# sayands/sgaligner

Hardware: AMD Instinct MI355X
Metric: subscan-pairs/sec (fwd+bwd) + node-match Hits@1 vs reference (higher is better)
Workload: dtype f32 (fp32 operands and fp32 accumulation throughout; the anchors x negatives loss sweeps multiply them as three exact bf16 planes, six bf16 MFMAs per product...

## Files before the change

include/sgaligner_hip.h:

```cpp
#ifndef SGALIGNER_HIP_H
#define SGALIGNER_HIP_H
#include <stddef.h>
#include <stdint.h>
#ifdef __cplusplus
extern "C" {
#endif

int sga_version(void);
const char* sga_last_error(void);
int sga_device_cus(void);

int sga_pointnet_fwd(const float* x, const float* w1, const float* b1, const float* w2, const float* b2,
                     const float* w3, const float* b3, float* y, int32_t* argmax, int T, int P, int C3,
                     void* stream);
size_t sga_pointnet_fwd_ws_bytes(int T, int C3);
int sga_pointnet_fwd_ws(const float* x, const float* w1, const float* b1, const float* w2, const float* b2,
                        const float* w3, const float* b3, float* y, int32_t* argmax, int T, int P, int C3,
                        void* workspace, size_t ws_bytes, int mode, void* stream);
size_t sga_pointnet_fwd_bn_ws_bytes(int T, int C3);
int sga_pointnet_fwd_bn(const float* x, const float* w1, const float* b1, const float* w2, const float* b2,
                        const float* w3, const float* b3, float* y, int32_t* argmax, int T, int P, int C3,
                        void* workspace, size_t ws_bytes, void* bn_workspace, size_t bn_ws_bytes, double* bn_sums, int mode, void* stream);
int sga_pointnet_bwd(const float* x, const int32_t* argmax, const float* y, const float* gy, const float* w1,
                     const float* b1, const float* w2, const float* b2, const float* w3, float* gw1, float* gb1,
                     float* gw2, float* gb2, float* gw3, float* gb3, int T, int P, int C3, int mode, void* stream);

int sga_gemm(int transA, int transB, int M, int N, int K, const void* A, long lda, int a_is_f64, const float* B,
             long ldb, float* C, long ldc, const float* bias, int accumulate, void* stream);
int sga_colsum(const float* X, long ld, int M, int N, float* out, int accumulate, void* stream);
int sga_gemm_bnstats(int M, int N, int K, const float* A, long lda, const float* B, long ldb, float* C, long ldc, const float* bias,
                     double* sums, void* stream);
int sga_cast_f64_f32(const double* in, float* out, size_t n, void* stream);
enum sga_gemm_route {
    SGA_GEMM_EMPTY = 0,
    SGA_GEMM_TN_NARROW,
    SGA_GEMM_TN_SPLIT,
    SGA_GEMM_TN_BIG,
    SGA_GEMM_NN,
    SGA_GEMM_NT_128,
    SGA_GEMM_NT_64,
    SGA_GEMM_NT3_128,
    SGA_GEMM_NT3_64,
    SGA_GEMM_SMALL_F32,
    SGA_GEMM_SMALL_F64,
    SGA_GEMM_GENERIC_F32,
    SGA_GEMM_GENERIC_F64,
    SGA_GEMM_REFUSED
};
int sga_gemm_plan(int transA, int transB, int M, int N, int K, long lda, long ldb, long ldc, long ldr, int a_is_f64, int a_aligned16,
                  int b_aligned16, int has_bias, int accumulate, int act, int has_resid, int has_colstats, int ncu, int* route, int* splits,
                  int* k_per_split);

int sga_fusion_fwd(const float* const* embs, int M, const float* weight, float* joint, int T, int D, void* stream);
size_t sga_fusion_bwd_workspace_bytes(int M);
int sga_fusion_bwd(const float* const* embs, int M, const float* weight, const float* gjoint, float* const* gembs,
                   float* gweight, int T, int D, void* workspace, size_t workspace_bytes, void* stream);
int sga_fusion_var_fwd(const float* const* embs, int M, const int32_t* widths, const float* weight, float* joint, int T, void* stream);
int sga_fusion_var_bwd(const float* const* embs, int M, const int32_t* widths, const float* weight, const float* gjoint,
                       float* const* gembs, float* gweight, int T, void* workspace, size_t workspace_bytes, void* stream);

int sga_gat_complete_flags(const int64_t* edges, const int32_t* node_off, const int32_t* edge_off, int G, uint8_t* flags, void* stream);
int sga_gat_attn_fwd(const float* H, const float* att_src, const float* att_dst, const float* bias,
                     const int64_t* edges, const int32_t* node_off, const int32_t* edge_off, int G, int nmax,
                     float* out, int32_t* status, const uint8_t* complete, void* stream);
int sga_gat_attn_bwd(const float* H, const float* dO, const float* att_src, const float* att_dst, const int64_t* edges,
                     const int32_t* node_off, const int32_t* edge_off, int G, int nmax, float* dH, float* d_att_src,
                     float* d_att_dst, const uint8_t* complete, void* stream);
int sga_gat_attn_fwd_hc(const float* H, int heads, int channels, const float* att_src, const float* att_dst, const float* bias,
                        const int64_t* edges, const int32_t* node_off, const int32_t* edge_off, int G, int nmax,
                        float* out, int32_t* status, const uint8_t* complete, void* stream);
int sga_gat_attn_bwd_hc(const float* H, const float* dO, int heads, int channels, const float* att_src, const float* att_dst,
                        const int64_t* edges, const int32_t* node_off, const int32_t* edge_off, int G, int nmax, float* dH,
                        float* d_att_src, float* d_att_dst, const uint8_t* complete, void* stream);
int sga_gat_lds_nodes(int channels, int bwd);
int sga_elu_fwd(const float* x, float* y, size_t n, void* stream);
int sga_elu_bwd(const float* x, const float* gy, float* gx, size_t n, void* stream);

int sga_gcn_aggregate(const float* H, int C, const float* bias, const int64_t* edges, const int32_t* node_off, const int32_t* edge_off,
                      int G, int nmax, int transpose, int relu, float* out, int32_t* status, void* stream);
int sga_relu_bwd(const float* y, const float* gy, float* gx, size_t n, void* stream);

int sga_nca_row_group(void);
int sga_nca_block_sums(const float* S, long lds, int h, int A, int row0, float alpha, float ep, double* rsum, float* diag, double* cpart,
                       void* stream);
int sga_nca_loss(const double* rsum, const double* cpart, int ngroups, const float* diag, int A, float alpha, float beta, double* csum,
                 float* invr, float* invc, double* loss, void* stream);
int sga_nca_coef(const float* S, long lds, float* G, long ldg, float* GT, long ldt, int h, int A, int row0, float alpha, float beta, float ep,
                 const float* invr, const float* invc, const double* gout, void* stream);

int sga_loss_gather(const float* E, int T, int D, const int32_t* idx, int R, float* Z, int Dp, float* nrm, void* stream);
int sga_loss_scatter(const float* dZ, const float* Z, const float* nrm, const int32_t* idx, int R, int D, int Dp,
                     float* dE, void* stream);
int sga_loss_slots(void);
int sga_loss_neg_sums(const float* Z, int Dp, int A, int J1, int J2, float tau0, float tau1, double* sums8, void* stream);
int sga_loss_neg_grad(const float* Z, int Dp, int A, int J1, int J2, float tau0, float tau1, const double* gs8,
                      float* dZ, void* stream);
int sga_loss_neg_sums_shard(const float* Z, int Dp, int A, int J1, int J2, float tau0, float tau1, double* sums8, int a_lo, int a_hi,
                            void* stream);
int sga_loss_neg_grad_shard(const float* Z, int Dp, int A, int J1, int J2, float tau0, float tau1, const double* gs8,
                            float* dZ, int a_lo, int a_hi, void* stream);
size_t sga_loss_anchor_f16_ws_bytes(int NT, int A, int ns);
int sga_loss_anchor_fwd_f16(const float* const* Z, const void* const* Zh, const int* Dp, int NT, int A, const double* sums,
                            float alpha, float tau_icl, float tau_ial, double* out, int a_lo, int a_hi, void* ws, size_t ws_bytes,
                            void* stream);
int sga_loss_anchor_bwd_f16(const float* const* Z, const void* const* Zh, const int* Dp, int NT, int A, const double* sums,
                            float alpha, float tau_icl, float tau_ial, const float* coef, float* const* M1,
                            double* gs, int a_lo, int a_hi, void* ws, size_t ws_bytes, void* stream);

int sga_loss_stash_grad(const float* M1, const float* Z, int A, int Dp, float* dZ, int a_lo, int a_hi, void* stream);
int sga_loss_multi_sums(const float* const* Z, int M, int D, const float* beta, int A, int J1, int J2, float tau0, float tau1,
                        double* sums, int a_lo, int a_hi, void* stream);
int sga_loss_multi_grad(const float* const* Z, int M, int D, const float* beta, int A, int J1, int J2, float tau0, float tau1,
                        const double* gs, float* const* dZ, double* gamma, int a_lo, int a_hi, void* stream);
size_t sga_loss_centre_bytes(void);
int sga_loss_centre_tables(const float* Z, int A, int J1, int J2, float* Zc, void* stat_ws, void* stream);
int sga_loss_multi_sums_centred(const float* const* Zc, int M, const float* beta, int A, int J1, int J2, float tau0, float tau1,
                                double* sums, int a_lo, int a_hi, void* stream);
int sga_loss_multi_grad_centred(const float* const* Zc, int M, const float* beta, int A, int J1, int J2, float tau0, float tau1,
                                const double* gs, float* const* dZ, double* gamma, int a_lo, int a_hi, void* stream);
int sga_loss_scatter_tangent_stat(const float* dZ, const float* Z, const float* nrm, const int32_t* idx, int R, int D,
                                  const void* stat_ws, float* dE, void* stream);
int sga_loss_anchor_multi_fwd(const float* const* Z, int M, const float* beta, int A, const double* sums, float alpha,
                              float tau_icl, float tau_ial, double* out, int a_lo, int a_hi, void* stream);
int sga_loss_anchor_multi_bwd(const float* const* Z, int M, const float* beta, int A, const double* sums, float alpha,
                              float tau_icl, float tau_ial, const float* coef, float* const* M1, double* gs, double* gamma,
                              int a_lo, int a_hi, double* out_terms, void* stream);
int sga_loss_anchor_multi_bwd_sym(const float* const* Z, int M, const float* beta, int A, const double* sums, float alpha,
                                  float tau_icl, float tau_ial, const float* coef, float* const* M1, float* const* M2, double* gs,
                                  double* gamma, int a_lo, int a_hi, double* out_terms, void* stream);
int sga_loss_stash_grad_sym(const float* M1, const float* M2, const float* Z, int A, int Dp, float* dZ, int a_lo, int a_hi,
                            void* stream);
int sga_loss_anchor_multi_bwd_symx(const float* const* Z, int M, const float* beta, int A, const double* sums, float alpha,
                                   float tau_icl, float tau_ial, const float* coef, float* const* M1, float* const* M2,
                                   double* gs, double* gamma, int a_lo, int a_hi, int j_lo, int j_hi, int mir, double* out_terms, void* stream);
int sga_loss_stash_grad_symx(const float* M1, const float* M2, const float* Z, int A, int Dp, float* dZ, int a_lo, int a_hi,
                             int j_lo, int j_hi, int mir, void* stream);

int sga_loss_check_norms(const float* nrm, int n, float* poison, void* stream);

size_t sga_loss_split3_bytes(int A, int J1, int J2);
int sga_loss_split3_tables(const float* Z, int A, int J1, int J2, void* Zb, float* Zc, void* stream);
int sga_loss_multi_sums_bf16x6(const void* const* Zb, int M, const float* beta, int A, int J1, int J2, float tau0, float tau1,
                               double* sums, int a_lo, int a_hi, int lite, void* stream);
int sga_loss_multi_grad_bf16x6(const void* const* Zb, int M, const float* beta, int A, int J1, int J2, float tau0, float tau1,
                               const double* gs, float* const* dZ, double* gamma, int a_lo, int a_hi, void* stream);
int sga_loss_scatter_tangent(const float* dZ, const float* Z, const float* nrm, const int32_t* idx, int A, int J1, int J2, int D,
                             const void* Zb, float* dE, void* stream);
int sga_loss_stash_grad_symx_bf16x6(const float* M1, const float* M2, const void* Zb, int A, int J1, int J2, float* dZ,
                                    int a_lo, int a_hi, int j_lo, int j_hi, int mir, void* stream);

int sga_group_loss_fwd(const float* const* Z, int M, const float* beta, int A, int J1, const int32_t* groups, int G,
                       const int64_t* s_off, int64_t s_total, float alpha, float tau_icl, float tau_ial, float* S,
                       double* sums, double* out, int use_valu, void* stream);
int sga_group_loss_bwd(const float* const* Z, int M, const float* beta, int A, int J1, const int32_t* groups, int G,
                       const int64_t* s_off, int64_t s_total, float alpha, float tau_icl, float tau_ial, float* S,
                       const double* sums, const float* coef, float* const* dZ, double* gamma, int use_valu, void* stream);

size_t sga_simrank_workspace_bytes(int T);
size_t sga_simrank_workspace_bytes_f16(int T, int D);
int sga_simrank(const float* E, int T, int D, const int32_t* pair_off, const int32_t* blk_pair, const int32_t* blk_row, int n_blocks, int B,
                int max_pair_objects, const int32_t* q_idx, const int32_t* q_tgt, int Q, int K, int32_t* rank,
                int32_t* topk_idx, float* topk_sim, int f16, void* workspace, size_t workspace_bytes, void* stream);
int sga_pair_metrics(const int32_t* rank, const int32_t* topk_idx, const float* topk_sim, int K, const int32_t* q_tgt,
                     const int32_t* pair_off, const int32_t* pair_q_off, int B, float* out, void* stream);

int sga_gemm_ex(int transA, int transB, int M, int N, int K, const float* A, long lda, const float* B, long ldb,
                float* C, long ldc, const float* bias, int act, const float* resid, long ldr, void* stream);
int sga_pct_attention(const float* Q, long ldq, const float* V, long ldv, int T, int N, float* stats, float* Xs,
                      long ldx, void* stream);
int sga_pct_attention_bwd(const float* Q, long ldq, const float* V, long ldv, const float* dXs, long ldd, int T, int N,
                          const float* stats, float* work, float* dQ, long ldo, float* dV, long ldw, void* stream);
int sga_segment_max(const float* Y, long ldy, int T, int N, int C, float* G, int32_t* argmax, void* stream);
int sga_segment_max_bwd(const float* dG, const int32_t* argmax, int T, int N, int C, float* dY, long ldd, void* stream);
int sga_pct_head_prep(const float* dG, const float* G, const float* gamma, const float* beta, const float* fin, int T, int C, long R,
                      int training, float slope, float* coef, float* ab, void* stream);
int sga_pct_head_dw(const float* WG, const float* W, const float* ab, const float* cs, const float* coef, const int32_t* amax,
                    const float* cat, long ldc, int T, int N, int C, int K, float* dW, float* Wb, float* a0, void* stream);
int sga_pct_head_scatter(const float* coef, const int32_t* amax, const float* W, int T, int N, int C, int K, float* dcat, long ldd,
                         void* stream);
int sga_segment_max_affine(const float* Y, long ldy, int T, int N, int C, const float* scale, const float* shift, float slope, float* G,
                           int32_t* argmax, void* stream);

int sga_bn_stats(const float* X, long ldx, int R, int C, double* sums, void* stream);
int sga_bn_finalize(const double* sums, int R, int C, const float* gamma, const float* beta, float* running_mean, float* running_var,
                    long long* num_batches_tracked, float momentum, float eps, int training, float* out, void* stream);
int sga_bn_bwd_finalize(const double* sums, int R, int C, float* out, void* stream);
int sga_bn_apply(const float* X, long ldx, int R, int C, const float* scale, const float* shift, int act,
                 const float* resid, long ldr, float* Y, long ldy, void* stream);
int sga_bn_bwd_stats(const float* X, long ldx, const float* dY, long ldd, int R, int C, const float* scale,
                     const float* shift, const float* mean, const float* rstd, int act, double* sums, void* stream);
int sga_bn_bwd_apply(const float* X, long ldx, const float* dY, long ldd, int R, int C, const float* scale,
                     const float* shift, const float* mean, const float* rstd, const float* mean_g,
                     const float* mean_gx, int act, float* dX, long ldo, void* stream);

size_t sga_fps_scratch_floats(int total_points);
int sga_fps(const float* pts, const int32_t* offsets, int n_obj, const int32_t* start, int npoint,
            const int32_t* work_small, int n_small, const int32_t* work_mid, int n_mid,
            const int32_t* work_large, int n_large, int32_t* out_idx, float* scratch, void* stream);

int sga_hull_candidates(const float* pts, const int32_t* offsets, int n_obj, unsigned char* keep, int32_t* n_planes, void* stream);
int sga_hull_max_candidates(void);
int sga_hull_vertices(const double* pts, const int32_t* offsets, int n_obj, unsigned char* is_vertex, int32_t* status, void* stream);

size_t sga_nn_workspace_bytes(int total_queries, int max_support, int chunk);
int sga_nn_search(const double* pts, const int32_t* offsets, int n_clouds, int total_points, const int32_t* pairs, int n_pairs,
                  const int32_t* out_offsets, int total_queries, int max_queries, int max_support, int chunk,
                  const int32_t* offsets_host, const int32_t* pairs_host, int squared, double* out_dist, int32_t* out_idx,
                  void* workspace, size_t workspace_bytes, void* stream);

size_t sga_ransac_workspace_bytes(int n_jobs, int total_hyp, int max_rows, int chunk);
int sga_ransac_rigid(const double* corr, const int32_t* offsets, int n_jobs, int total_rows, const int32_t* samples,
                     const int32_t* hyp_offsets, int total_hyp, int max_rows, int max_hyp, int chunk, const int32_t* offsets_host,
                     const int32_t* hyp_offsets_host, double threshold, int refine_rounds, double* transform, int32_t* inlier_count,
                     int32_t* best_hyp, int32_t* status, unsigned char* inlier_mask, int32_t* hyp_count, void* workspace,
                     size_t workspace_bytes, void* stream);

int sga_subscan_lds_slots(void);
int sga_frame_visibility(const float* pts, const int32_t* pt_off, const double* w2c, const int32_t* fr_off, const double* intr,
                         const int64_t* vis_off, int n_scans, int total_points, int total_frames, int64_t total_words, int max_points,
                         int max_frames, const int32_t* pt_off_host, const int32_t* fr_off_host, const int64_t* vis_off_host,
                         uint64_t* vis, void* stream);
int sga_subscan_walk(const uint64_t* vis, uint64_t* cum, const int32_t* pt_off, const int32_t* fr_off, const int64_t* vis_off,
                     const int32_t* max_pts, int n_scans, int total_points, int total_frames, int64_t total_words,
                     const int32_t* pt_off_host, const int32_t* fr_off_host, const int64_t* vis_off_host, int32_t* seg_end,
                     int32_t* seg_count, int32_t* frame_count, int32_t* n_seg, void* stream);
int sga_subscan_object_counts(const uint64_t* bits, const int32_t* pt_off, const int32_t* fr_off, const int64_t* vis_off, int n_scans,
                              int total_points, int total_frames, int64_t total_words, int max_points, const int32_t* rows, int n_rows,
                              const int32_t* slot, int n_slots, const int32_t* pt_off_host, const int32_t* fr_off_host,
                              const int64_t* vis_off_host, const int32_t* rows_host, int32_t* counts, void* stream);

int sga_scenegraph_lds_slots(void);
int sga_scenegraph_tile(void);
int sga_graph_max_nodes(void);
int sga_object_counts(const int32_t* slot, const int32_t* pt_off, const int32_t* slot_off, int n_scans, int total_points, int total_slots,
                      int max_points, const int32_t* pt_off_host, const int32_t* slot_off_host, int32_t* counts, void* stream);
size_t sga_object_partition_ws_bytes(int n_scans, int max_points, int max_slots);
int sga_object_partition(const float* pts, const int32_t* slot, const int32_t* pt_off, const int32_t* slot_off, const int32_t* dest_off,
                         int n_scans, int total_points, int total_slots, int max_points, int max_slots, int n_kept_points,
                         const int32_t* pt_off_host, const int32_t* slot_off_host, const int32_t* dest_off_host, const int32_t* counts_host,
                         int32_t* perm, float* pts_out, void* ws, size_t ws_bytes, void* stream);
int sga_graph_complete(const int32_t* node_off, const int32_t* pair_off, const int32_t* trip_off, const int32_t* edge_off, int n_graphs,
                       const int32_t* pairs, const int32_t* rels, int none_id, int V, const int32_t* node_off_host,
                       const int32_t* pair_off_host, const int32_t* trip_off_host, const int32_t* edge_off_host, const int32_t* pairs_host,
                       const int32_t* rels_host, int64_t* edges, int32_t* n_edges, int32_t* bow, void* stream);
int sga_bow_counts(const int32_t* rows, const int32_t* cols, int n, int T, int V, const int32_t* rows_host, const int32_t* cols_host,
                   int32_t* out, void* stream);

size_t sga_loss_neg_grad_wide_floats(int A, int J1, int J2);
int sga_loss_neg_grad_wide(const float* Z, int Dp, int A, int J1, int J2, float tau0, float tau1, const double* gs8, float* dZ,
                           float* stash, size_t stash_floats, void* stream);

long sga_wide16_ldt(int A, int J1, int J2);
int sga_wide16_prepare(const float* Z, int Dp, int A, int J1, int J2, void* Zh, void* ZhT, void* stream);
int sga_loss_neg_sums_f16(const void* Zh, int Dp, int A, int J1, int J2, float tau0, float tau1, double* sums8, int a_lo, int a_hi, void* stream);
size_t sga_loss_neg_grad_f16_bytes(int A, int J1, int J2);
int sga_loss_neg_grad_f16(const void* Zh, const void* ZhT, int Dp, int A, int J1, int J2, float tau0, float tau1, const double* gs8,
                          float* dZ, void* stash, size_t stash_bytes, int a_lo, int a_hi, void* stream);
size_t sga_loss_stash_grad_f16_bytes(int A, int ns);
int sga_loss_stash_grad_f16(const float* M1, const void* ZhT, int Dp, int A, int J1, int J2, float* dZ, int a_lo, int a_hi,
                            void* ws, size_t ws_bytes, void* stream);

int sga_loss_head_fwd(const void* sums, int sums_f64, const float* lv_ial, const float* lv_icl, int M, double inv_a2,
                      double z_ial, double alpha, double zoom, double* out, void* stream);
int sga_loss_head_bwd(const double* gout, const void* sums, int sums_f64, const float* lv_ial, const float* lv_icl, int M,
                      double inv_a2, double z_ial, double alpha, double zoom, void* dsums, float* dlv_ial, float* dlv_icl,
                      void* stream);

#ifdef __cplusplus
}
#endif
#endif
```

sgaligner_amd/_build.py:

```python
from __future__ import annotations

import concurrent.futures as cf
import glob
import os
import subprocess
import sys

CSRC = os.path.join(os.path.dirname(os.path.abspath(__file__)), 'csrc')
LIB = os.path.join(CSRC, 'libsga_hip.so')
HIPCC = os.environ.get('HIPCC', '/opt/rocm/bin/hipcc')
FLAGS = ['--offload-arch=gfx950', '-O3', '-std=c++17', '-fPIC', '-ffp-contract=fast', '-munsafe-fp-atomics',
         '-Wno-unused-result', '-Wno-unused-value', '-I', CSRC]


def _newer(src_list, target):
    if not os.path.exists(target):
        return True
    t = os.path.getmtime(target)
    return any(os.path.getmtime(s) > t for s in src_list)


FILE_FLAGS = {'contrastive.hip': ['-fno-slp-vectorize'],
              'loss_pertable.hip': ['-fno-slp-vectorize'],
              'loss_anchor.hip': ['-fno-slp-vectorize'],
              'sweep3.hip': ['-fno-slp-vectorize'],
              'pointnet.hip': ['-fno-slp-vectorize'],
              'nnsearch.hip': ['-ffp-contract=off'],
              'visibility.hip': ['-ffp-contract=off']}


def _compile(src, obj, extra):
    cmd = [HIPCC] + FLAGS + FILE_FLAGS.get(os.path.basename(src), []) + extra + ['-c', src, '-o', obj]
    r = subprocess.run(cmd, capture_output=True, text=True)
    if r.returncode != 0:
        raise RuntimeError(f'hipcc failed for {src}:\n{r.stdout}\n{r.stderr}')
    return src


def build_lib(verbose: bool = True, extra_flags=()) -> str:
    srcs = sorted(glob.glob(os.path.join(CSRC, '*.hip')))
    hdrs = sorted(glob.glob(os.path.join(CSRC, '*.h'))) + sorted(glob.glob(os.path.join(CSRC, '..', '..', 'include', '*.h')))
    jobs = []
    objs = []
    for s in srcs:
        o = s[:-4] + '.o'
        objs.append(o)
        if _newer([s] + hdrs, o):
            jobs.append((s, o))
    if jobs:
        with cf.ThreadPoolExecutor(max_workers=min(8, len(jobs))) as ex:
            for done in ex.map(lambda so: _compile(so[0], so[1], list(extra_flags)), jobs):
                if verbose:
                    print('[sga build] compiled', os.path.basename(done), flush=True)
    if jobs or _newer(objs, LIB):
        r = subprocess.run([HIPCC, '--offload-arch=gfx950', '-shared', '-fPIC', '-o', LIB] + objs,
                           capture_output=True, text=True)
        if r.returncode != 0:
            raise RuntimeError(f'link failed:\n{r.stdout}\n{r.stderr}')
        if verbose:
            print('[sga build] linked', LIB, flush=True)
    return LIB


if __name__ == '__main__':
    build_lib(extra_flags=sys.argv[1:])
```

sgaligner_amd/_lib.py:

```python
from __future__ import annotations

import ctypes
import os
from ctypes import c_char_p, c_double, c_float, c_int, c_int64, c_long, c_size_t, c_void_p

_HERE = os.path.dirname(os.path.abspath(__file__))
LIB_PATH = os.environ.get('SGA_LIB_PATH') or os.path.join(_HERE, 'csrc', 'libsga_hip.so')
_lib = None

P = c_void_p
I = c_int
F = c_float

SIGNATURES = {
    'sga_version': (I, []),
    'sga_last_error': (c_char_p, []),
    'sga_device_cus': (I, []),
    'sga_pointnet_fwd': (I, [P, P, P, P, P, P, P, P, P, I, I, I, P]),
    'sga_pointnet_fwd_ws_bytes': (c_size_t, [I, I]),
    'sga_loss_neg_grad_wide_floats': (c_size_t, [I, I, I]),
    'sga_loss_neg_grad_wide': (I, [P, I, I, I, I, c_float, c_float, P, P, P, c_size_t, P]),
    'sga_wide16_ldt': (c_long, [I, I, I]),
    'sga_wide16_prepare': (I, [P, I, I, I, I, P, P, P]),
    'sga_loss_neg_sums_f16': (I, [P, I, I, I, I, c_float, c_float, P, I, I, P]),
    'sga_loss_neg_grad_f16_bytes': (c_size_t, [I, I, I]),
    'sga_loss_neg_grad_f16': (I, [P, P, I, I, I, I, c_float, c_float, P, P, P, c_size_t, I, I, P]),
    'sga_loss_head_fwd': (I, [P, I, P, P, I, c_double, c_double, c_double, c_double, P, P]),
    'sga_loss_head_bwd': (I, [P, P, I, P, P, I, c_double, c_double, c_double, c_double, P, P, P, P]),
    'sga_pointnet_fwd_ws': (I, [P, P, P, P, P, P, P, P, P, I, I, I, P, c_size_t, I, P]),
    'sga_pointnet_fwd_bn_ws_bytes': (c_size_t, [I, I]),
    'sga_pointnet_fwd_bn': (I, [P, P, P, P, P, P, P, P, P, I, I, I, P, c_size_t, P, c_size_t, P, I, P]),
    'sga_pointnet_bwd': (I, [P] * 15 + [I, I, I, I, P]),
    'sga_gat_complete_flags': (I, [P, P, P, I, P, P]),
    'sga_gat_attn_fwd': (I, [P, P, P, P, P, P, P, I, I, P, P, P, P]),
    'sga_gat_attn_bwd': (I, [P, P, P, P, P, P, P, I, I, P, P, P, P, P]),
    'sga_gat_attn_fwd_hc': (I, [P, I, I, P, P, P, P, P, P, I, I, P, P, P, P]),
    'sga_gat_attn_bwd_hc': (I, [P, P, I, I, P, P, P, P, P, I, I, P, P, P, P, P]),
    'sga_gat_lds_nodes': (I, [I, I]),
    'sga_elu_fwd': (I, [P, P, c_size_t, P]),
    'sga_elu_bwd': (I, [P, P, P, c_size_t, P]),
    'sga_simrank_workspace_bytes': (c_size_t, [I]),
    'sga_simrank_workspace_bytes_f16': (c_size_t, [I, I]),
    'sga_simrank': (I, [P, I, I, P, P, P, I, I, I, P, P, I, I, P, P, P, I, P, c_size_t, P]),
    'sga_pair_metrics': (I, [P, P, P, I, P, P, P, I, P, P]),
    'sga_gemm_ex': (I, [I, I, I, I, I, P, c_long, P, c_long, P, c_long, P, I, P, c_long, P]),
    'sga_pct_attention': (I, [P, c_long, P, c_long, I, I, P, P, c_long, P]),
    'sga_pct_attention_bwd': (I, [P, c_long, P, c_long, P, c_long, I, I, P, P, P, c_long, P, c_long, P]),
    'sga_segment_max': (I, [P, c_long, I, I, I, P, P, P]),
    'sga_segment_max_bwd': (I, [P, P, I, I, I, P, c_long, P]),
    'sga_pct_head_prep': (I, [P, P, P, P, P, I, I, c_long, I, c_float, P, P, P]),
    'sga_pct_head_dw': (I, [P, P, P, P, P, P, P, c_long, I, I, I, I, P, P, P, P]),
    'sga_pct_head_scatter': (I, [P, P, P, I, I, I, I, P, c_long, P]),
    'sga_segment_max_affine': (I, [P, c_long, I, I, I, P, P, c_float, P, P, P]),
    'sga_bn_stats': (I, [P, c_long, I, I, P, P]),
    'sga_bn_finalize': (I, [P, I, I, P, P, P, P, P, c_float, c_float, I, P, P]),
    'sga_bn_bwd_finalize': (I, [P, I, I, P, P]),
    'sga_bn_apply': (I, [P, c_long, I, I, P, P, I, P, c_long, P, c_long, P]),
    'sga_bn_bwd_stats': (I, [P, c_long, P, c_long, I, I, P, P, P, P, I, P, P]),
    'sga_bn_bwd_apply': (I, [P, c_long, P, c_long, I, I, P, P, P, P, P, P, I, P, c_long, P]),
    'sga_fps_scratch_floats': (c_size_t, [I]),
    'sga_fps': (I, [P, P, I, P, I, P, I, P, I, P, I, P, P, P]),
    'sga_hull_candidates': (I, [P, P, I, P, P, P]),
    'sga_hull_max_candidates': (I, []),
    'sga_hull_vertices': (I, [P, P, I, P, P, P]),
    'sga_nn_workspace_bytes': (c_size_t, [I, I, I]),
    'sga_nn_search': (I, [P, P, I, I, P, I, P, I, I, I, I, P, P, I, P, P, P, c_size_t, P]),
    'sga_ransac_workspace_bytes': (c_size_t, [I, I, I, I]),
    'sga_ransac_rigid': (I, [P, P, I, I, P, P, I, I, I, I, P, P, c_double, I, P, P, P, P, P, P, P, c_size_t, P]),
    'sga_subscan_lds_slots': (I, []),
    'sga_frame_visibility': (I, [P, P, P, P, P, P, I, I, I, c_int64, I, I, P, P, P, P, P]),
    'sga_subscan_walk': (I, [P, P, P, P, P, P, I, I, I, c_int64, P, P, P, P, P, P, P, P]),
    'sga_subscan_object_counts': (I, [P, P, P, P, I, I, I, c_int64, I, P, I, P, I, P, P, P, P, P, P]),
    'sga_scenegraph_lds_slots': (I, []),
    'sga_scenegraph_tile': (I, []),
    'sga_graph_max_nodes': (I, []),
    'sga_object_counts': (I, [P, P, P, I, I, I, I, P, P, P, P]),
    'sga_object_partition_ws_bytes': (c_size_t, [I, I, I]),
    'sga_object_partition': (I, [P, P, P, P, P, I, I, I, I, I, I, P, P, P, P, P, P, P, c_size_t, P]),
    'sga_graph_complete': (I, [P, P, P, P, I, P, P, I, I, P, P, P, P, P, P, P, P, P, P]),
    'sga_bow_counts': (I, [P, P, I, I, I, P, P, P, P]),
    'sga_gemm': (I, [I, I, I, I, I, P, c_long, I, P, c_long, P, c_long, P, I, P]),
    'sga_colsum': (I, [P, c_long, I, I, P, I, P]),
    'sga_gemm_bnstats': (I, [I, I, I, P, c_long, P, c_long, P, c_long, P, P, P]),
    'sga_cast_f64_f32': (I, [P, P, c_size_t, P]),
    'sga_gemm_plan': (I, [I, I, I, I, I, c_long, c_long, c_long, c_long] + [I] * 9 + [P, P, P]),
    'sga_loss_gather': (I, [P, I, I, P, I, P, I, P, P]),
    'sga_loss_scatter': (I, [P, P, P, P, I, I, I, P, P]),
    'sga_loss_neg_sums': (I, [P, I, I, I, I, F, F, P, P]),
    'sga_loss_neg_grad': (I, [P, I, I, I, I, F, F, P, P, P]),
    'sga_loss_neg_sums_shard': (I, [P, I, I, I, I, F, F, P, I, I, P]),
    'sga_loss_neg_grad_shard': (I, [P, I, I, I, I, F, F, P, P, I, I, P]),
    'sga_loss_anchor_f16_ws_bytes': (c_size_t, [I, I, I]),
    'sga_loss_anchor_fwd_f16': (I, [P, P, P, I, I, P, F, F, F, P, I, I, P, c_size_t, P]),
    'sga_loss_anchor_bwd_f16': (I, [P, P, P, I, I, P, F, F, F, P, P, P, I, I, P, c_size_t, P]),
    'sga_loss_stash_grad_f16_bytes': (c_size_t, [I, I]),
    'sga_loss_stash_grad_f16': (I, [P, P, I, I, I, I, P, I, I, P, c_size_t, P]),
    'sga_loss_multi_sums': (I, [P, I, I, P, I, I, I, F, F, P, I, I, P]),
    'sga_loss_multi_grad': (I, [P, I, I, P, I, I, I, F, F, P, P, P, I, I, P]),
    'sga_loss_centre_bytes': (c_size_t, []),
    'sga_loss_centre_tables': (I, [P, I, I, I, P, P, P]),
    'sga_loss_multi_sums_centred': (I, [P, I, P, I, I, I, F, F, P, I, I, P]),
    'sga_loss_multi_grad_centred': (I, [P, I, P, I, I, I, F, F, P, P, P, I, I, P]),
    'sga_loss_scatter_tangent_stat': (I, [P, P, P, P, I, I, P, P, P]),
    'sga_loss_check_norms': (I, [P, I, P, P]),
    'sga_loss_slots': (I, []),
    'sga_loss_anchor_multi_fwd': (I, [P, I, P, I, P, F, F, F, P, I, I, P]),
    'sga_loss_anchor_multi_bwd': (I, [P, I, P, I, P, F, F, F, P, P, P, P, I, I, P, P]),
    'sga_loss_stash_grad': (I, [P, P, I, I, P, I, I, P]),
    'sga_loss_anchor_multi_bwd_sym': (I, [P, I, P, I, P, F, F, F, P, P, P, P, P, I, I, P, P]),
    'sga_loss_stash_grad_sym': (I, [P, P, P, I, I, P, I, I, P]),
    'sga_loss_anchor_multi_bwd_symx': (I, [P, I, P, I, P, F, F, F, P, P, P, P, P, I, I, I, I, I, P, P]),
    'sga_loss_stash_grad_symx': (I, [P, P, P, I, I, P, I, I, I, I, I, P]),
    'sga_loss_split3_bytes': (c_size_t, [I, I, I]),
    'sga_loss_split3_tables': (I, [P, I, I, I, P, P, P]),
    'sga_loss_scatter_tangent': (I, [P, P, P, P, I, I, I, I, P, P, P]),
    'sga_loss_stash_grad_symx_bf16x6': (I, [P, P, P, I, I, I, P, I, I, I, I, I, P]),
    'sga_loss_multi_sums_bf16x6': (I, [P, I, P, I, I, I, F, F, P, I, I, I, P]),
    'sga_loss_multi_grad_bf16x6': (I, [P, I, P, I, I, I, F, F, P, P, P, I, I, P]),
    'sga_group_loss_fwd': (I, [P, I, P, I, I, P, I, P, c_int64, F, F, F, P, P, P, I, P]),
    'sga_group_loss_bwd': (I, [P, I, P, I, I, P, I, P, c_int64, F, F, F, P, P, P, P, P, I, P]),
    'sga_fusion_fwd': (I, [P, I, P, P, I, I, P]),
    'sga_fusion_bwd_workspace_bytes': (c_size_t, [I]),
    'sga_fusion_bwd': (I, [P, I, P, P, P, P, I, I, P, c_size_t, P]),
    'sga_fusion_var_fwd': (I, [P, I, P, P, P, I, P]),
    'sga_fusion_var_bwd': (I, [P, I, P, P, P, P, P, I, P, c_size_t, P]),
    'sga_gcn_aggregate': (I, [P, I, P, P, P, P, I, I, I, I, P, P, P]),
    'sga_relu_bwd': (I, [P, P, P, c_size_t, P]),
    'sga_nca_row_group': (I, []),
    'sga_nca_block_sums': (I, [P, c_long, I, I, I, F, F, P, P, P, P]),
    'sga_nca_loss': (I, [P, P, I, P, I, F, F, P, P, P, P, P]),
    'sga_nca_coef': (I, [P, c_long, P, c_long, P, c_long, I, I, I, F, F, F, P, P, P, P]),
}

GEMM_ROUTES = ('EMPTY', 'TN_NARROW', 'TN_SPLIT', 'TN_BIG', 'NN', 'NT_128', 'NT_64', 'NT3_128', 'NT3_64', 'SMALL_F32', 'SMALL_F64',
               'GENERIC_F32', 'GENERIC_F64', 'REFUSED')


class SgaLibraryError(RuntimeError):
    pass


def lib():
    global _lib
    if _lib is None:
        if not os.path.exists(LIB_PATH):
            raise SgaLibraryError(
                f'HIP library not built: {LIB_PATH} is missing. Run `python -c "import __graft_entry__ as g; g.build()"` '
                f'(or `python -m sgaligner_amd._build`). sgaligner_amd has no CPU fallback.')
        import torch
        try:
            l = ctypes.CDLL(LIB_PATH)
        except OSError as e:
            raise SgaLibraryError(f'cannot load {LIB_PATH}: {e}') from e
        for name, (res, args) in SIGNATURES.items():
            try:
                fn = getattr(l, name)
            except AttributeError as e:
                raise SgaLibraryError(f'{LIB_PATH} does not export {name}; rebuild the library') from e
            fn.restype = res
            fn.argtypes = args
        _lib = l
    return _lib


def check(rc: int, what: str):
    if rc != 0:
        msg = lib().sga_last_error()
        raise RuntimeError(f'{what} failed (code {rc}): {msg.decode() if msg else "?"}')
```

sgaligner_amd/csrc/loss_anchor.hip:

```cpp
#include "mfma_tiles.h"
#include <type_traits>

#include "loss_math.h"

extern "C" int sga_gemm(int transA, int transB, int M, int N, int K, const void* A, long lda, int a_is_f64, const float* B,
                        long ldb, float* C, long ldc, const float* bias, int accumulate, void* stream);

namespace {

constexpr int CT_THREADS = 256;
struct AnchorMultiArgs {
    int M, A, i_lo, i_hi, nsplit;
    const float* Z[4];
    const float* beta;
    const double* sums;
    const float* inv;
    float alpha, kc, ki, itc, iti;
    double* out;
    const float* coef;
    float* M1[4];
    double* gs;
    double* gamma;
    int j_lo;
    float* M2[4];
    int j_hi, mir;
};

template <int M>
__global__ __launch_bounds__(CT_THREADS, M <= 3 ? 2 : 1) void anchor_multi_kernel(AnchorMultiArgs a) {
    constexpr int DP = 104, NQ = 13, NT = M + 1;
    extern __shared__ __attribute__((aligned(16))) float lds[];
    float* inv_s = lds + M * 2 * 32 * DP;
    const int tid = threadIdx.x, lane = tid & 63, wave = tid >> 6, h = lane >> 5, l31 = lane & 31;
    const int A = a.A, ns = a.i_hi - a.i_lo;
    const int ib = blockIdx.x / a.nsplit, split = blockIdx.x % a.nsplit;
    const int i0 = a.i_lo + ib * 32;
    const int my_i = i0 + l31;
    const bool iv = my_i < a.i_hi;

    for (int e = tid; e < M * 2 * 32 * (DP / 4); e += CT_THREADS) {
        const int c = (e % (DP / 4)) * 4, r = (e / (DP / 4)) % 32, side = (e / (DP / 4) / 32) % 2, m = e / (DP / 4) / 64;
        const int row = min(i0 + r, a.i_hi - 1) + side * A;
        *reinterpret_cast<f32x4*>(lds + ((m * 2 + side) * 32 + r) * DP + c) = *reinterpret_cast<const f32x4*>(a.Z[m] + (size_t)row * DP + c);
    }
    for (int e = tid; e < NT * 8; e += CT_THREADS) inv_s[e] = (float)(1.0 / (a.sums[e] + 1e-9));
    __syncthreads();
    float beta[M];
#pragma unroll
    for (int m = 0; m < M; ++m) beta[m] = a.beta[m];

    double acc_d[NT + 2 * M];
#pragma unroll
    for (int e = 0; e < NT + 2 * M; ++e) acc_d[e] = 0.0;

    const int ntile = (A + 31) / 32;
    for (int jt = split * 4 + wave; jt < ntile; jt += a.nsplit * 4) {
        const int j0 = jt * 32;
        float acc_out[NT + 2 * M];
#pragma unroll
        for (int e = 0; e < NT + 2 * M; ++e) acc_out[e] = 0.f;
        const int jrow = min(j0 + l31, A - 1);
        f32x16 P[M], Q[M];
        zero_acc<M>(P);
        zero_acc<M>(Q);
#pragma unroll
        for (int m = 0; m < M; ++m) {
            const float* gp = a.Z[m] + (size_t)(A + jrow) * DP + 4 * h;
            const float* gq = a.Z[m] + (size_t)jrow * DP + 4 * h;
            const float* bp = lds + ((m * 2 + 0) * 32 + l31) * DP + 4 * h;
            const float* bq = lds + ((m * 2 + 1) * 32 + l31) * DP + 4 * h;
            f32x4 apA = *reinterpret_cast<const f32x4*>(gp), aqA = *reinterpret_cast<const f32x4*>(gq), apB = apA, aqB = aqA;
#pragma unroll
            for (int q = 0; q < NQ; ++q) {
                if (q + 1 < NQ) {
                    if (q & 1) { apA = *reinterpret_cast<const f32x4*>(gp + 8 * (q + 1)); aqA = *reinterpret_cast<const f32x4*>(gq + 8 * (q + 1)); }
                    else { apB = *reinterpret_cast<const f32x4*>(gp + 8 * (q + 1)); aqB = *reinterpret_cast<const f32x4*>(gq + 8 * (q + 1)); }
                }
                const f32x4 b1 = *reinterpret_cast<const f32x4*>(bp + 8 * q);
                const f32x4 b2 = *reinterpret_cast<const f32x4*>(bq + 8 * q);
#pragma unroll
                for (int r = 0; r < 4; ++r) {
                    P[m] = __builtin_amdgcn_mfma_f32_32x32x2f32((q & 1) ? apB[r] : apA[r], b1[r], P[m], 0, 0, 0);
                    Q[m] = __builtin_amdgcn_mfma_f32_32x32x2f32((q & 1) ? aqB[r] : aqA[r], b2[r], Q[m], 0, 0, 0);
                }
                __builtin_amdgcn_sched_barrier(0);
            }
        }
        float xs[M][16], ys[M][16];
#pragma unroll
        for (int m = 0; m < M; ++m)
#pragma unroll
            for (int r = 0; r < 16; ++r) { xs[m][r] = P[m][r]; ys[m][r] = Q[m][r]; }
        const float* js = inv_s + M * 8;
#pragma unroll
        for (int r = 0; r < 16; ++r) {
            const int j = j0 + mfma32_row(r, h);
            const bool ok = iv && j < A;
            float xj = 0.f, yj = 0.f;
#pragma unroll
            for (int m = 0; m < M; ++m) { xj = fmaf(beta[m], xs[m][r], xj); yj = fmaf(beta[m], ys[m][r], yj); }
            {
                const float dji = fexp2(xj * a.ki);
                const float qma = g_val(dji, js[1], js[3]), qmb = g_val(dji, js[5], js[7]);
                const float lqma = flog(qma), lqmb = flog(qmb);
#pragma unroll
                for (int k = 0; k < NT; ++k) {
                    const float x = k < M ? xs[k < M ? k : 0][r] : xj, y = k < M ? ys[k < M ? k : 0][r] : yj;
                    const float* is = inv_s + k * 8;
                    const float qa = g_val(fexp2(x * a.kc), is[0], is[2]);
                    const float qb = g_val(fexp2(y * a.kc), is[4], is[6]);
                    const float term = -flog(a.alpha * qa + (1.f - a.alpha) * qb);
                    acc_out[k] += ok ? term : 0.f;
                    if (k < M) {
                        const float dm = fexp2(x * a.ki);
                        const float qoa = g_val(dm, is[1], is[3]), qob = g_val(dm, is[5], is[7]);
                        const float ta = __expf(qoa) * (qoa - lqma), tb = __expf(qob) * (qob - lqmb);
                        acc_out[NT + (k < M ? k : 0)] += ok ? ta : 0.f;
                        acc_out[NT + M + (k < M ? k : 0)] += ok ? tb : 0.f;
                    }
                }
            }
#pragma unroll
            for (int e = 0; e < NT + 2 * M; ++e) asm volatile("" : "+v"(acc_out[e]));
            __builtin_amdgcn_sched_barrier(0);
        }
#pragma unroll
        for (int e = 0; e < NT + 2 * M; ++e) acc_d[e] += (double)acc_out[e];
    }
    const int slot = my_slot();
#pragma unroll
    for (int e = 0; e < NT + 2 * M; ++e) {
        const double v = wave_sum_d(acc_d[e]);
        if (lane == 0 && v != 0.0) atomicAdd(a.out + (NT + 2 * M) * (1 + slot) + e, v);
    }
}

__global__ void inv_sums_kernel(const double* __restrict__ sums, float* __restrict__ inv, int n) {
    const int i = blockIdx.x * blockDim.x + threadIdx.x;
    if (i < n) inv[i] = (float)(1.0 / (sums[i] + 1e-9));
}

template <int M, bool TERMS = false, int RB = (M <= 3 ? 32 : 16), bool SYM = false>
__global__ __launch_bounds__(CT_THREADS, 2) void anchor_multi_bwd16_kernel(AnchorMultiArgs a) {
    static_assert(!SYM || TERMS, "symmetric mode: one-pass build");
    constexpr int DP = 104, NT = M + 1, NSUB = RB / 16, TW = 4 / NSUB;
    extern __shared__ __attribute__((aligned(16))) float lds[];
    const float* __restrict__ inv_s = a.inv;
    auto CF = [&](int e) { return a.coef[e]; };
    const int tid = threadIdx.x, lane = tid & 63, wave = tid >> 6, g = lane >> 4, l15 = lane & 15;
    const int A = a.A, ns = a.i_hi - a.i_lo;
    const int JH = SYM ? a.j_hi : A;
    const int ib = blockIdx.x / a.nsplit, split = blockIdx.x % a.nsplit;
    const int i0 = a.i_lo + ib * RB;
    const int ih = wave % NSUB, tw = wave / NSUB;
    const int my_i = i0 + ih * 16 + l15;
    const bool iv = my_i < a.i_hi;

    for (int e = tid; e < M * 2 * RB * (DP / 4); e += CT_THREADS) {
        const int c = (e % (DP / 4)) * 4, r = (e / (DP / 4)) % RB, side = (e / (DP / 4) / RB) % 2, m = e / (DP / 4) / (2 * RB);
        const int row = min(i0 + r, a.i_hi - 1) + side * A;
        *reinterpret_cast<f32x4*>(lds + ((m * 2 + side) * RB + r) * DP + c) = *reinterpret_cast<const f32x4*>(a.Z[m] + (size_t)row * DP + c);
    }
    __syncthreads();
    float beta[M];
#pragma unroll
    for (int m = 0; m < M; ++m) beta[m] = a.beta[m];

    float acc_gs[NT][8], acc_gam[M];
#pragma unroll
    for (int k = 0; k < NT; ++k)
#pragma unroll
        for (int e = 0; e < 8; ++e) acc_gs[k][e] = 0.f;
#pragma unroll
    for (int m = 0; m < M; ++m) acc_gam[m] = 0.f;
    float acc_out[TERMS ? NT + 2 * M : 1];
#pragma unroll
    for (int e = 0; e < (TERMS ? NT + 2 * M : 1); ++e) acc_out[e] = 0.f;
    int tiles_done = 0;
    const int slot = my_slot();
    auto flush = [&]() {
        if (TERMS) {
#pragma unroll
            for (int e = 0; e < NT + 2 * M; ++e) {
                const float v = wave_sum(acc_out[TERMS ? e : 0]);
                if (lane == 0 && v != 0.f) atomicAdd(a.out + (NT + 2 * M) * (1 + slot) + e, (double)v);
                acc_out[TERMS ? e : 0] = 0.f;
            }
        }
#pragma unroll
        for (int k = 0; k < NT; ++k)
#pragma unroll
            for (int e = 0; e < 8; ++e) {
                const float iv2 = inv_s[k * 8 + e];
                const float v = -iv2 * iv2 * wave_sum(acc_gs[k][e]);
                if (lane == 0 && v != 0.f) atomicAdd(a.gs + NT * 8 * (1 + slot) + k * 8 + e, (double)v);
                acc_gs[k][e] = 0.f;
            }
#pragma unroll
        for (int m = 0; m < M; ++m) {
            const float v = wave_sum(acc_gam[m]);
            if (lane == 0 && v != 0.f) atomicAdd(a.gamma + M * (1 + slot) + m, (double)v);
            acc_gam[m] = 0.f;
        }
    };
    const float* js = inv_s + M * 8;

    const int ntile = (JH + 15) / 16;
#pragma unroll 1
    for (int jt = (a.j_lo >> 4) + split * TW + tw; jt < ntile; jt += a.nsplit * TW) {
        const int j0 = jt * 16;
        const int jrow = min(j0 + l15, A - 1);
        int lofs = 0;
        asm volatile("" : "+v"(lofs));
        f32x4 P[M], Q[M];
        struct JOps { f32x4 p[6], q[6]; float pt[2], qt[2]; };
        auto jload = [&](int m, JOps& o) {
            const float* gp = a.Z[m] + (size_t)(A + jrow) * DP;
            const float* gq = a.Z[m] + (size_t)jrow * DP;
#pragma unroll
            for (int q = 0; q < 6; ++q) {
                o.p[q] = *reinterpret_cast<const f32x4*>(gp + 16 * q + 4 * g);
                o.q[q] = *reinterpret_cast<const f32x4*>(gq + 16 * q + 4 * g);
            }
#pragma unroll
            for (int t = 0; t < 2; ++t) { o.pt[t] = gp[96 + 4 * t + g]; o.qt[t] = gq[96 + 4 * t + g]; }
        };
        constexpr bool JDB = true;
        JOps jb[JDB ? 2 : 1];
        jload(0, jb[0]);
#pragma unroll
        for (int m = 0; m < M; ++m) {
            if (JDB) { if (m + 1 < M) jload(m + 1, jb[JDB ? (m + 1) & 1 : 0]); }
            else if (m > 0) jload(m, jb[0]);
            __builtin_amdgcn_sched_barrier(0);
            P[m] = f32x4{0.f, 0.f, 0.f, 0.f};
            Q[m] = P[m];
            const JOps& o = jb[JDB ? m & 1 : 0];
            const float* bp = lds + lofs + ((m * 2 + 0) * RB + ih * 16 + l15) * DP;
            const float* bq = lds + lofs + ((m * 2 + 1) * RB + ih * 16 + l15) * DP;
#pragma unroll
            for (int q = 0; q < 6; ++q) {
                const f32x4 b1 = *reinterpret_cast<const f32x4*>(bp + 16 * q + 4 * g);
                const f32x4 b2 = *reinterpret_cast<const f32x4*>(bq + 16 * q + 4 * g);
#pragma unroll
                for (int r = 0; r < 4; ++r) {
                    P[m] = __builtin_amdgcn_mfma_f32_16x16x4f32(o.p[q][r], b1[r], P[m], 0, 0, 0);
                    Q[m] = __builtin_amdgcn_mfma_f32_16x16x4f32(o.q[q][r], b2[r], Q[m], 0, 0, 0);
                }
            }
#pragma unroll
            for (int t = 0; t < 2; ++t) {
                const int kk = 96 + 4 * t + g;
                P[m] = __builtin_amdgcn_mfma_f32_16x16x4f32(o.pt[t], bp[kk], P[m], 0, 0, 0);
                Q[m] = __builtin_amdgcn_mfma_f32_16x16x4f32(o.qt[t], bq[kk], Q[m], 0, 0, 0);
            }
            __builtin_amdgcn_sched_barrier(0);
        }
        const float cJ = CF(M);
        auto epilogue = [&](auto masked_c) {
        constexpr bool MASKED = decltype(masked_c)::value;
#pragma unroll
        for (int r = 0; r < 4; ++r) {
            const int j = j0 + 4 * g + r;
            const bool ok = !MASKED || (iv && (j < JH));
            const float okf = (!MASKED || ok) ? 1.f : 0.f;
            float xj = 0.f, yj = 0.f;
#pragma unroll
            for (int m = 0; m < M; ++m) { xj = fmaf(beta[m], P[m][r], xj); yj = fmaf(beta[m], Q[m][r], yj); }
            float gJ, EA = 0.f, EB = 0.f;
            {
                const float dx = fexp2(xj * a.kc), dy = fexp2(yj * a.kc);
                const GP Ax = g_parts(dx, js[0], js[2]), Bx = g_parts(dx, js[4], js[6]);
                const float qAy = g_val(dy, js[0], js[2]), qBy = g_val(dy, js[4], js[6]);
                const float denA = a.alpha * Ax.q + (1.f - a.alpha) * qBy;
                const float wA = okf * (-cJ * a.alpha) * frcp(denA) * dx;
                const float wB = okf * (-cJ * (1.f - a.alpha)) * frcp(a.alpha * qAy + (1.f - a.alpha) * Bx.q) * dx;
                if (TERMS) acc_out[TERMS ? M : 0] = fmaf(okf, -flog(denA), acc_out[TERMS ? M : 0]);
                gJ = fmaf(wA, Ax.dd, wB * Bx.dd) * a.itc;
                acc_gs[M][0] = fmaf(wA, Ax.p, acc_gs[M][0]); acc_gs[M][2] = fmaf(wA, Ax.r, acc_gs[M][2]);
                acc_gs[M][4] = fmaf(wB, Bx.p, acc_gs[M][4]); acc_gs[M][6] = fmaf(wB, Bx.r, acc_gs[M][6]);
            }
            const float dji = fexp2(xj * a.ki);
            const GP MA = g_parts(dji, js[1], js[3]), MB = g_parts(dji, js[5], js[7]);
            const float lqma = flog(MA.q), lqmb = flog(MB.q);
            float gx[M];
#pragma unroll
            for (int m = 0; m < M; ++m) {
                const float* is = inv_s + m * 8;
                const float c = CF(m), ca = CF(NT + m), cb = CF(NT + M + m);
                const float x = P[m][r], y = Q[m][r];
                const float dx = fexp2(x * a.kc), dy = fexp2(y * a.kc);
                const GP Ax = g_parts(dx, is[0], is[2]), Bx = g_parts(dx, is[4], is[6]);
                const float qAy = g_val(dy, is[0], is[2]), qBy = g_val(dy, is[4], is[6]);
                const float denA = a.alpha * Ax.q + (1.f - a.alpha) * qBy;
                const float wA = okf * (-c * a.alpha) * frcp(denA) * dx;
                const float wB = okf * (-c * (1.f - a.alpha)) * frcp(a.alpha * qAy + (1.f - a.alpha) * Bx.q) * dx;
                if (TERMS) acc_out[TERMS ? m : 0] = fmaf(okf, -flog(denA), acc_out[TERMS ? m : 0]);
                float gxm = fmaf(wA, Ax.dd, wB * Bx.dd) * a.itc;
                acc_gs[m][0] = fmaf(wA, Ax.p, acc_gs[m][0]); acc_gs[m][2] = fmaf(wA, Ax.r, acc_gs[m][2]);
                acc_gs[m][4] = fmaf(wB, Bx.p, acc_gs[m][4]); acc_gs[m][6] = fmaf(wB, Bx.r, acc_gs[m][6]);
                const float dm = fexp2(x * a.ki);
                const GP OA = g_parts(dm, is[1], is[3]), OB = g_parts(dm, is[5], is[7]);
                const float xA = okf * __expf(OA.q), xB = okf * __expf(OB.q);
                const float eA = ca * xA, eB = cb * xB;
                if (TERMS) {
                    acc_out[TERMS ? NT + m : 0] = fmaf(xA, OA.q - lqma, acc_out[TERMS ? NT + m : 0]);
                    acc_out[TERMS ? NT + M + m : 0] = fmaf(xB, OB.q - lqmb, acc_out[TERMS ? NT + M + m : 0]);
                }
                const float tA = eA * (OA.q - lqma + 1.f) * dm, tB = eB * (OB.q - lqmb + 1.f) * dm;
                gxm = fmaf(fmaf(tA, OA.dd, tB * OB.dd), a.iti, gxm);
                acc_gs[m][1] = fmaf(tA, OA.p, acc_gs[m][1]); acc_gs[m][3] = fmaf(tA, OA.r, acc_gs[m][3]);
                acc_gs[m][5] = fmaf(tB, OB.p, acc_gs[m][5]); acc_gs[m][7] = fmaf(tB, OB.r, acc_gs[m][7]);
                EA += eA; EB += eB;
                gx[m] = gxm;
            }
            {
                const float uA = -EA * frcp(MA.q) * dji, uB = -EB * frcp(MB.q) * dji;
                gJ = fmaf(fmaf(uA, MA.dd, uB * MB.dd), a.iti, gJ);
                acc_gs[M][1] = fmaf(uA, MA.p, acc_gs[M][1]); acc_gs[M][3] = fmaf(uA, MA.r, acc_gs[M][3]);
                acc_gs[M][5] = fmaf(uB, MB.p, acc_gs[M][5]); acc_gs[M][7] = fmaf(uB, MB.r, acc_gs[M][7]);
            }
#pragma unroll
            for (int m = 0; m < M; ++m) {
                acc_gam[m] = fmaf(gJ, P[m][r], acc_gam[m]);
                if (ok) a.M1[m][(size_t)(j - a.j_lo) * ns + (my_i - a.i_lo)] = fmaf(beta[m], gJ, gx[m]);
            }
#pragma unroll
            for (int k = 0; k < NT; ++k)
#pragma unroll
                for (int e = 0; e < 8; ++e) asm volatile("" : "+v"(acc_gs[k][e]));
#pragma unroll
            for (int m = 0; m < M; ++m) asm volatile("" : "+v"(acc_gam[m]));
            if (TERMS) {
#pragma unroll
                for (int e = 0; e < NT + 2 * M; ++e) asm volatile("" : "+v"(acc_out[TERMS ? e : 0]));
            }
            __builtin_amdgcn_sched_barrier(0);
        }
        };
        auto epilogue_sym = [&](auto) {
#pragma unroll
        for (int r = 0; r < 4; ++r) {
            const int j = j0 + 4 * g + r;
            const bool ok = iv && (j < JH);
            const float okf = ok ? 1.f : 0.f;
            float xj = 0.f, yj = 0.f;
#pragma unroll
            for (int m = 0; m < M; ++m) { xj = fmaf(beta[m], P[m][r], xj); yj = fmaf(beta[m], Q[m][r], yj); }
            float gci[NT][2];
#pragma unroll
            for (int k = 0; k < NT; ++k) {
                const float* is = inv_s + k * 8;
                const float x = k < M ? P[k < M ? k : 0][r] : xj, y = k < M ? Q[k < M ? k : 0][r] : yj;
                const float c = CF(k);
                const float dx = fexp2(x * a.kc), dy = fexp2(y * a.kc);
                const GP Ax = g_parts(dx, is[0], is[2]), Bx = g_parts(dx, is[4], is[6]);
                const GP Ay = g_parts(dy, is[0], is[2]), By = g_parts(dy, is[4], is[6]);
                const float den1 = a.alpha * Ax.q + (1.f - a.alpha) * By.q;
                const float den2 = a.alpha * Ay.q + (1.f - a.alpha) * Bx.q;
                const float r1 = okf * -c * frcp(den1), r2 = okf * -c * frcp(den2);
                const float wAx = a.alpha * r1 * dx, wBx = (1.f - a.alpha) * r2 * dx;
                const float wAy = a.alpha * r2 * dy, wBy = (1.f - a.alpha) * r1 * dy;
                acc_out[TERMS ? k : 0] = fmaf(okf, -(flog(den1) + flog(den2)), acc_out[TERMS ? k : 0]);
                gci[k][0] = fmaf(wAx, Ax.dd, wBx * Bx.dd) * a.itc;
                gci[k][1] = fmaf(wAy, Ay.dd, wBy * By.dd) * a.itc;
                acc_gs[k][0] = fmaf(wAx, Ax.p, fmaf(wAy, Ay.p, acc_gs[k][0])); acc_gs[k][2] = fmaf(wAx, Ax.r, fmaf(wAy, Ay.r, acc_gs[k][2]));
                acc_gs[k][4] = fmaf(wBx, Bx.p, fmaf(wBy, By.p, acc_gs[k][4])); acc_gs[k][6] = fmaf(wBx, Bx.r, fmaf(wBy, By.r, acc_gs[k][6]));
#pragma unroll
                for (int e = 0; e < 8; e += 2) asm volatile("" : "+v"(acc_gs[k][e]));
                asm volatile("" : "+v"(acc_out[TERMS ? k : 0]));
                __builtin_amdgcn_sched_barrier(0);
            }
#pragma unroll
            for (int dir = 0; dir < 2; ++dir) {
                const float vj = dir ? yj : xj;
                const float dji = fexp2(vj * a.ki);
                const GP MA = g_parts(dji, js[1], js[3]), MB = g_parts(dji, js[5], js[7]);
                const float lqma = flog(MA.q), lqmb = flog(MB.q);
                float gx[M], EA = 0.f, EB = 0.f;
#pragma unroll
                for (int m = 0; m < M; ++m) {
                    const float* is = inv_s + m * 8;
                    const float ca = CF(NT + m), cb = CF(NT + M + m);
                    const float v = dir ? Q[m][r] : P[m][r];
                    const float dm = fexp2(v * a.ki);
                    const GP OA = g_parts(dm, is[1], is[3]), OB = g_parts(dm, is[5], is[7]);
                    const float xA = okf * __expf(OA.q), xB = okf * __expf(OB.q);
                    const float eA = ca * xA, eB = cb * xB;
                    acc_out[TERMS ? NT + m : 0] = fmaf(xA, OA.q - lqma, acc_out[TERMS ? NT + m : 0]);
                    acc_out[TERMS ? NT + M + m : 0] = fmaf(xB, OB.q - lqmb, acc_out[TERMS ? NT + M + m : 0]);
                    const float tA = eA * (OA.q - lqma + 1.f) * dm, tB = eB * (OB.q - lqmb + 1.f) * dm;
                    gx[m] = fmaf(fmaf(tA, OA.dd, tB * OB.dd), a.iti, gci[m][dir]);
                    acc_gs[m][1] = fmaf(tA, OA.p, acc_gs[m][1]); acc_gs[m][3] = fmaf(tA, OA.r, acc_gs[m][3]);
                    acc_gs[m][5] = fmaf(tB, OB.p, acc_gs[m][5]); acc_gs[m][7] = fmaf(tB, OB.r, acc_gs[m][7]);
                    EA += eA; EB += eB;
                }
                const float uA = -EA * frcp(MA.q) * dji, uB = -EB * frcp(MB.q) * dji;
                const float gJ = fmaf(fmaf(uA, MA.dd, uB * MB.dd), a.iti, gci[M][dir]);
                acc_gs[M][1] = fmaf(uA, MA.p, acc_gs[M][1]); acc_gs[M][3] = fmaf(uA, MA.r, acc_gs[M][3]);
                acc_gs[M][5] = fmaf(uB, MB.p, acc_gs[M][5]); acc_gs[M][7] = fmaf(uB, MB.r, acc_gs[M][7]);
                float* const* dst = dir ? a.M2 : a.M1;
                const size_t off = (size_t)(j - (dir ? a.mir : a.j_lo)) * ns + (my_i - a.i_lo);
#pragma unroll
                for (int m = 0; m < M; ++m) {
                    acc_gam[m] = fmaf(gJ, dir ? Q[m][r] : P[m][r], acc_gam[m]);
                    if (ok) dst[m][off] = fmaf(beta[m], gJ, gx[m]);
                }
#pragma unroll
                for (int k = 0; k < NT; ++k)
#pragma unroll
                    for (int e = 1; e < 8; e += 2) asm volatile("" : "+v"(acc_gs[k][e]));
#pragma unroll
                for (int m = 0; m < M; ++m) asm volatile("" : "+v"(acc_gam[m]));
#pragma unroll
                for (int e = NT; e < NT + 2 * M; ++e) asm volatile("" : "+v"(acc_out[TERMS ? e : 0]));
                __builtin_amdgcn_sched_barrier(0);
            }
        }
        };
        if constexpr (SYM) {
            if (j0 >= a.mir) epilogue_sym(0); else epilogue(std::true_type{});
        } else {
            if (j0 + 16 <= A && i0 + RB <= a.i_hi) epilogue(std::false_type{}); else epilogue(std::true_type{});
        }
        if ((++tiles_done & (SYM ? 15 : 31)) == 0) flush();
    }
    flush();
}

}

static int fill_anchor_multi(AnchorMultiArgs& a, const float* const* Z, int M, const float* beta, int A, const double* sums,
                             float alpha, float tau_icl, float tau_ial, int a_lo, int a_hi) {
    if (M < 2 || M > 4) { sga_set_error("sga_loss_anchor_multi: M=%d not in {2,3,4} (use the per-table kernels)", M); return SGA_ERR_ARG; }
    if (a_lo < 0 || a_hi > A || a_lo > a_hi) { sga_set_error("sga_loss_anchor_multi: anchor shard [%d,%d) outside [0,%d]", a_lo, a_hi, A); return SGA_ERR_ARG; }
    a.M = M; a.A = A; a.i_lo = a_lo; a.i_hi = a_hi; a.beta = beta; a.sums = sums; a.alpha = alpha;
    a.kc = LOG2E / tau_icl; a.ki = LOG2E / tau_ial; a.itc = 1.f / tau_icl; a.iti = 1.f / tau_ial;
    for (int m = 0; m < M; ++m) { if (!Z[m]) { sga_set_error("sga_loss_anchor_multi: null table"); return SGA_ERR_ARG; } a.Z[m] = Z[m]; }
    const int nib = (a_hi - a_lo + 31) / 32, ntile = (A + 31) / 32;
    int ns = (4 * sga_num_cus() + nib - 1) / (nib > 0 ? nib : 1);
    if (ns > (ntile + 3) / 4) ns = (ntile + 3) / 4;
    if (ns < 1) ns = 1;
    a.nsplit = ns;
    return SGA_OK;
}

template <int M>
static void launch_anchor_multi(const AnchorMultiArgs& a, hipStream_t s) {
    const size_t lds = (size_t)(M * 2 * 32 * 104 + (M + 1) * 8) * sizeof(float);
    auto k = anchor_multi_kernel<M>;
    hipFuncSetAttribute(reinterpret_cast<const void*>(k), hipFuncAttributeMaxDynamicSharedMemorySize, (int)lds);
    const int nib = (a.i_hi - a.i_lo + 31) / 32;
    hipLaunchKernelGGL(k, dim3(nib * a.nsplit), dim3(CT_THREADS), lds, s, a);
}

extern "C" int sga_loss_anchor_multi_fwd(const float* const* Z, int M, const float* beta, int A, const double* sums,
                                         float alpha, float tau_icl, float tau_ial, double* out, int a_lo, int a_hi,
                                         void* stream) {
    SGA_CHECK_ARG(Z && beta && sums && out && A >= 0, "sga_loss_anchor_multi_fwd: bad argument");
    hipStream_t s = static_cast<hipStream_t>(stream);
    const int n = (M + 1) + 2 * M;
    if (int rc0 = zero_slots(out, n, s, "sga_loss_anchor_multi_fwd")) return rc0;
    if (A == 0 || a_hi <= a_lo) return SGA_OK;
    AnchorMultiArgs a{};
    int rc = fill_anchor_multi(a, Z, M, beta, A, sums, alpha, tau_icl, tau_ial, a_lo, a_hi);
    if (rc) return rc;
    a.out = out;
    if (M == 2) launch_anchor_multi<2>(a, s); else if (M == 3) launch_anchor_multi<3>(a, s); else launch_anchor_multi<4>(a, s);
    fold_slots(out, n, s);
    SGA_CHECK_LAUNCH("sga_loss_anchor_multi_fwd");
    return SGA_OK;
}

static void launch_anchor_multi_bwd(AnchorMultiArgs& a, int j_lo, int j_hi, int mir, bool sym, hipStream_t s) {
    const int M = a.M;
    a.j_lo = j_lo; a.j_hi = j_hi; a.mir = mir;
    float* inv = reinterpret_cast<float*>(a.gs + (size_t)(1 + SGA_SLOTS) * (M + 1) * 8);
    hipLaunchKernelGGL(inv_sums_kernel, dim3(1), dim3(64), 0, s, a.sums, inv, (M + 1) * 8);
    a.inv = inv;
    const int RB = M <= 3 ? 32 : 16, TW = M <= 3 ? 2 : 4;
    const size_t lds = (size_t)(M * 2 * RB * 104 + (M + 1) * 8) * sizeof(float);
    const int nib = (a.i_hi - a.i_lo + RB - 1) / RB, ntile16 = (j_hi - j_lo + 15) / 16;
    int nsp = (6 * sga_num_cus() + nib - 1) / nib;
    if (nsp > (ntile16 + TW - 1) / TW) nsp = (ntile16 + TW - 1) / TW;
    if (nsp < 1) nsp = 1;
    a.nsplit = nsp;
    auto go = [&](auto k) {
        hipFuncSetAttribute(reinterpret_cast<const void*>(k), hipFuncAttributeMaxDynamicSharedMemorySize, (int)lds);
        hipLaunchKernelGGL(k, dim3(nib * nsp), dim3(CT_THREADS), lds, s, a);
    };
    if (sym) { if (M == 2) go(anchor_multi_bwd16_kernel<2, true, 32, true>); else if (M == 3) go(anchor_multi_bwd16_kernel<3, true, 32, true>); else go(anchor_multi_bwd16_kernel<4, true, 16, true>); }
    else if (a.out) { if (M == 2) go(anchor_multi_bwd16_kernel<2, true>); else if (M == 3) go(anchor_multi_bwd16_kernel<3, true>); else go(anchor_multi_bwd16_kernel<4, true>); }
    else { if (M == 2) go(anchor_multi_bwd16_kernel<2, false>); else if (M == 3) go(anchor_multi_bwd16_kernel<3, false>); else go(anchor_multi_bwd16_kernel<4, false>); }
    if (a.out) fold_slots(a.out, (M + 1) + 2 * M, s);
    fold_slots(a.gs, (M + 1) * 8, s);
    fold_slots(a.gamma, M, s);
}

extern "C" int sga_loss_anchor_multi_bwd(const float* const* Z, int M, const float* beta, int A, const double* sums,
                                         float alpha, float tau_icl, float tau_ial, const float* coef, float* const* M1,
                                         double* gs, double* gamma, int a_lo, int a_hi, double* out_terms, void* stream) {
    SGA_CHECK_ARG(Z && beta && sums && coef && M1 && gs && gamma && A >= 0, "sga_loss_anchor_multi_bwd: bad argument");
    hipStream_t s = static_cast<hipStream_t>(stream);
    if (int rc0 = zero_slots(gs, (M + 1) * 8, s, "sga_loss_anchor_multi_bwd")) return rc0;
    if (int rc1 = zero_slots(gamma, M, s, "sga_loss_anchor_multi_bwd")) return rc1;
    if (out_terms) { if (int rc2 = zero_slots(out_terms, (M + 1) + 2 * M, s, "sga_loss_anchor_multi_bwd")) return rc2; }
    if (A == 0 || a_hi <= a_lo) return SGA_OK;
    AnchorMultiArgs a{};
    int rc = fill_anchor_multi(a, Z, M, beta, A, sums, alpha, tau_icl, tau_ial, a_lo, a_hi);
    if (rc) return rc;
    a.coef = coef; a.gs = gs; a.gamma = gamma; a.out = out_terms;
    for (int m = 0; m < M; ++m) { SGA_CHECK_ARG(M1[m], "sga_loss_anchor_multi_bwd: null stash"); a.M1[m] = M1[m]; }
    launch_anchor_multi_bwd(a, 0, A, A, false, s);
    SGA_CHECK_LAUNCH("sga_loss_anchor_multi_bwd");
    return SGA_OK;
}

extern "C" int sga_loss_anchor_multi_bwd_symx(const float* const* Z, int M, const float* beta, int A, const double* sums, float alpha,
                                              float tau_icl, float tau_ial, const float* coef, float* const* M1, float* const* M2,
                                              double* gs, double* gamma, int a_lo, int a_hi, int j_lo, int j_hi, int mir, double* out_terms,
                                              void* stream) {
    SGA_CHECK_ARG(Z && beta && sums && coef && M1 && M2 && gs && gamma && out_terms && A >= 0, "sga_loss_anchor_multi_bwd_symx: bad argument");
    SGA_CHECK_ARG(M >= 2 && M <= 4, "sga_loss_anchor_multi_bwd_symx: M=%d (2, 3 or 4)", M);
    SGA_CHECK_ARG(a_lo % 32 == 0 && (a_hi % 32 == 0 || a_hi == A), "sga_loss_anchor_multi_bwd_symx: block [%d,%d) not on 32-row boundaries", a_lo, a_hi);
    SGA_CHECK_ARG(j_lo >= 0 && j_lo % 16 == 0 && j_hi <= A && j_lo <= j_hi && (j_hi % 16 == 0 || j_hi == A) && mir >= j_lo && (mir % 16 == 0 || mir >= j_hi),
                  "sga_loss_anchor_multi_bwd_symx: columns [%d,%d) / mirror start %d not on 16-column boundaries", j_lo, j_hi, mir);
    SGA_CHECK_ARG(mir <= j_lo || (j_lo >= a_lo && (mir < j_hi ? mir : j_hi) <= a_hi), "sga_loss_anchor_multi_bwd_symx: ordered columns [%d,%d) outside the block's square [%d,%d)",
                  j_lo, mir, a_lo, a_hi);
    hipStream_t s = static_cast<hipStream_t>(stream);
    if (int rc0 = zero_slots(gs, (M + 1) * 8, s, "sga_loss_anchor_multi_bwd_symx")) return rc0;
    if (int rc1 = zero_slots(gamma, M, s, "sga_loss_anchor_multi_bwd_symx")) return rc1;
    if (int rc2 = zero_slots(out_terms, (M + 1) + 2 * M, s, "sga_loss_anchor_multi_bwd_symx")) return rc2;
    if (A == 0 || a_hi <= a_lo || j_hi <= j_lo) return SGA_OK;
    AnchorMultiArgs a{};
    int rc = fill_anchor_multi(a, Z, M, beta, A, sums, alpha, tau_icl, tau_ial, a_lo, a_hi);
    if (rc) return rc;
    a.coef = coef; a.gs = gs; a.gamma = gamma; a.out = out_terms;
    for (int m = 0; m < M; ++m) {
        SGA_CHECK_ARG(M1[m] && (M2[m] || mir >= j_hi), "sga_loss_anchor_multi_bwd_symx: null stash");
        a.M1[m] = M1[m]; a.M2[m] = M2[m];
    }
    launch_anchor_multi_bwd(a, j_lo, j_hi, mir, true, s);
    SGA_CHECK_LAUNCH("sga_loss_anchor_multi_bwd_symx");
    return SGA_OK;
}

extern "C" int sga_loss_anchor_multi_bwd_sym(const float* const* Z, int M, const float* beta, int A, const double* sums, float alpha,
                                             float tau_icl, float tau_ial, const float* coef, float* const* M1, float* const* M2,
                                             double* gs, double* gamma, int a_lo, int a_hi, double* out_terms, void* stream) {
    return sga_loss_anchor_multi_bwd_symx(Z, M, beta, A, sums, alpha, tau_icl, tau_ial, coef, M1, M2, gs, gamma, a_lo, a_hi, a_lo, A, a_hi, out_terms, stream);
}

extern "C" int sga_loss_stash_grad_symx(const float* M1, const float* M2, const float* Z, int A, int Dp, float* dZ, int a_lo, int a_hi,
                                        int j_lo, int j_hi, int mir, void* stream) {
    SGA_CHECK_ARG(M1 && Z && dZ && A >= 0 && Dp >= 8 && Dp % 8 == 0 && a_lo >= 0 && a_hi <= A && a_lo <= a_hi && j_lo >= 0 && j_lo <= j_hi && j_hi <= A &&
                  mir >= j_lo && (M2 || mir >= j_hi), "sga_loss_stash_grad_symx: bad argument");
    const int ns = a_hi - a_lo, c1 = j_hi - j_lo, c2 = mir < j_hi ? j_hi - mir : 0;
    if (A == 0 || ns == 0 || c1 == 0) return SGA_OK;
    const float* X1 = Z;
    const float* X2 = Z + (size_t)A * Dp;
    float* d1 = dZ;
    float* d2 = dZ + (size_t)A * Dp;
    int rc = sga_gemm(1, 0, ns, Dp, c1, M1, ns, 0, X2 + (size_t)j_lo * Dp, Dp, d1 + (size_t)a_lo * Dp, Dp, nullptr, 1, stream);
    if (!rc) rc = sga_gemm(0, 0, c1, Dp, ns, M1, ns, 0, X1 + (size_t)a_lo * Dp, Dp, d2 + (size_t)j_lo * Dp, Dp, nullptr, 1, stream);
    if (!rc && c2 > 0) rc = sga_gemm(0, 0, c2, Dp, ns, M2, ns, 0, X2 + (size_t)a_lo * Dp, Dp, d1 + (size_t)mir * Dp, Dp, nullptr, 1, stream);
    if (!rc && c2 > 0) rc = sga_gemm(1, 0, ns, Dp, c2, M2, ns, 0, X1 + (size_t)mir * Dp, Dp, d2 + (size_t)a_lo * Dp, Dp, nullptr, 1, stream);
    return rc;
}

extern "C" int sga_loss_stash_grad_sym(const float* M1, const float* M2, const float* Z, int A, int Dp, float* dZ, int a_lo, int a_hi,
                                       void* stream) {
    return sga_loss_stash_grad_symx(M1, M2, Z, A, Dp, dZ, a_lo, a_hi, a_lo, A, a_hi, stream);
}
```

sgaligner_amd/csrc/sweep3.hip:

```cpp
#include <type_traits>

#include "loss_math.h"

namespace {

typedef __bf16 bf16x8 __attribute__((ext_vector_type(8)));
typedef __bf16 bf16x2 __attribute__((ext_vector_type(2)));
typedef float f32x2 __attribute__((ext_vector_type(2)));
typedef unsigned int u32x4 __attribute__((ext_vector_type(4)));
typedef unsigned int u32x2 __attribute__((ext_vector_type(2)));
typedef short s16x4 __attribute__((ext_vector_type(4)));

constexpr int S3_DP = 104;
constexpr int S3_PLANE = 3 * 2 * 1024;
constexpr int S3_TAIL = 3 * S3_PLANE;
constexpr int S3_BLOCK = S3_TAIL + 2048;
constexpr int S3_NCH = S3_BLOCK / 1024;
constexpr int S3_ROWSLOTS = 3 * 12 + 4;

__device__ __forceinline__ void split3_pair(float v0, float v1, unsigned& h, unsigned& m, unsigned& l) {
    const bf16x2 H = __builtin_convertvector(f32x2{v0, v1}, bf16x2);
    const unsigned hu = __builtin_bit_cast(unsigned, H);
#ifdef S3_SPLIT_DOT2
    unsigned c0 = 0x0000BF80u, c1 = 0xBF800000u;
    asm("" : "+s"(c0), "+s"(c1));
    const bf16x2 n0 = __builtin_bit_cast(bf16x2, c0), n1 = __builtin_bit_cast(bf16x2, c1);
    const float r0 = __builtin_amdgcn_fdot2_f32_bf16(H, n0, v0, false);
    const float r1 = __builtin_amdgcn_fdot2_f32_bf16(H, n1, v1, false);
#else
    const float r0 = v0 - __builtin_bit_cast(float, hu << 16);
    const float r1 = v1 - __builtin_bit_cast(float, hu & 0xffff0000u);
#endif
    const bf16x2 Mi = __builtin_convertvector(f32x2{r0, r1}, bf16x2);
    const unsigned mu = __builtin_bit_cast(unsigned, Mi);
#ifdef S3_SPLIT_DOT2
    const float s0 = __builtin_amdgcn_fdot2_f32_bf16(Mi, n0, r0, false);
    const float s1 = __builtin_amdgcn_fdot2_f32_bf16(Mi, n1, r1, false);
#else
    const float s0 = r0 - __builtin_bit_cast(float, mu << 16);
    const float s1 = r1 - __builtin_bit_cast(float, mu & 0xffff0000u);
#endif
    const bf16x2 Lo = __builtin_convertvector(f32x2{s0, s1}, bf16x2);
    h = hu; m = mu; l = __builtin_bit_cast(unsigned, Lo);
}
__device__ __forceinline__ f32x4 mfma_b(u32x4 a, u32x4 b, f32x4 c) {
    return __builtin_amdgcn_mfma_f32_16x16x32_bf16(__builtin_bit_cast(bf16x8, a), __builtin_bit_cast(bf16x8, b), c, 0, 0, 0);
}
__device__ __forceinline__ u32x2 tr_read16(const unsigned char* p) {
    return __builtin_bit_cast(u32x2, __builtin_amdgcn_ds_read_tr16_b64_v4i16((__attribute__((address_space(3))) s16x4*)(p)));
}
__device__ __forceinline__ unsigned long long sreg64(unsigned long long v) {
    const unsigned lo = __builtin_amdgcn_readfirstlane((unsigned)v), hi = __builtin_amdgcn_readfirstlane((unsigned)(v >> 32));
    return ((unsigned long long)hi << 32) | lo;
}
template <int X, int END, int NR, bool VALU_ALL> __device__ __forceinline__ void sgb_seq() {
    if constexpr (X < END) {
        __builtin_amdgcn_sched_group_barrier(0x008, 1, 0);
        if constexpr (X < NR) __builtin_amdgcn_sched_group_barrier(0x100, 1, 0);
        if constexpr (VALU_ALL || X < 2) __builtin_amdgcn_sched_group_barrier(0x002, 2, 0);
        sgb_seq<X + 1, END, NR, VALU_ALL>();
    }
}
__host__ __device__ constexpr int s3_slot(int g, int i) { return 16 * g + (i ^ (12 * (g & 1))); }

struct TLayout { int nbA, nb1, nb2; };
__host__ __device__ inline TLayout make_tlayout(int A, int J1, int J2) { return TLayout{(A + 31) / 32, (J1 + 31) / 32, (J2 + 31) / 32}; }

constexpr int S3_STAT_BYTES = 2048;
constexpr int S3_DREAL = 100;

constexpr int S3_CS_BLOCKS = 256;
__global__ __launch_bounds__(128) void split3_colsum_kernel(const float* __restrict__ Z, int R, double* __restrict__ part) {
    const int c = threadIdx.x;
    const int per = (R + gridDim.x - 1) / gridDim.x, r0 = blockIdx.x * per, r1 = min(R, r0 + per);
    if (c >= S3_DP) return;
    double acc = 0.0;
    for (int r = r0; r < r1; ++r) acc += (double)Z[(size_t)r * S3_DP + c];
    part[(size_t)blockIdx.x * S3_DP + c] = acc;
}
__global__ __launch_bounds__(128) void split3_stats_kernel(const double* __restrict__ part, int nblocks, int R, float* __restrict__ stat) {
    __shared__ double sq[128];
    const int c = threadIdx.x;
    double cs = 0.0;
    if (c < S3_DP) for (int b = 0; b < nblocks; ++b) cs += part[(size_t)b * S3_DP + c];
    float zb = (c < S3_DREAL && R > 0) ? (float)(cs / (double)R) : 0.f;
    sq[c] = (double)zb * (double)zb;
    __syncthreads();
    __shared__ double tot;
    if (c == 0) {
        double t = 0.0;
        for (int i = 0; i < 128; ++i) t += sq[i];
        tot = t;
    }
    __syncthreads();
    const bool centre = tot >= 0.25;
    if (!centre) zb = 0.f;
    if (c < S3_DP) stat[c] = zb;
    if (c == 0) { stat[S3_DP] = centre ? (float)(0.5 * tot) : 0.f; stat[S3_DP + 1] = centre ? 1.f : 0.f; }
}

__global__ __launch_bounds__(256) void split3_tables_kernel(const float* __restrict__ Z, int A, int J1, int J2, unsigned char* __restrict__ Zb,
                                                            const float* __restrict__ stat, float* __restrict__ Zc) {
    __shared__ float tile[32 * S3_DP];
    __shared__ float zbar[S3_DP];
    const TLayout L = make_tlayout(A, J1, J2);
    int b = blockIdx.x, old0, len;
    if (b < L.nbA) { old0 = 0; len = A; }
    else if (b < 2 * L.nbA) { b -= L.nbA; old0 = A; len = A; }
    else if (b < 2 * L.nbA + L.nb1) { b -= 2 * L.nbA; old0 = 2 * A; len = J1; }
    else { b -= 2 * L.nbA + L.nb1; old0 = 2 * A + J1; len = J2; }
    const int nvalid = min(32, len - 32 * b);
    const float* src = Z + (size_t)(old0 + 32 * b) * S3_DP;
    if (threadIdx.x < S3_DP) zbar[threadIdx.x] = stat[threadIdx.x];
    __syncthreads();
    for (int e = threadIdx.x; e < 32 * S3_DP; e += 256) {
        const int r = e / S3_DP, c = e - r * S3_DP;
        tile[e] = (r < nvalid && c < S3_DREAL) ? src[e] - zbar[c] : 0.f;
        if (Zc && old0 < 2 * A && r < nvalid) Zc[(size_t)(old0 + 32 * b) * S3_DP + e] = c == S3_DREAL + 1 ? 1.f : tile[e];
    }
    __syncthreads();
    if (threadIdx.x < 32) {
        const int r = threadIdx.x;
        if (r < nvalid) {
            double a = 0.0;
            for (int c = 0; c < S3_DREAL; ++c) a += (double)zbar[c] * (double)tile[r * S3_DP + c];
            tile[r * S3_DP + S3_DREAL] = (float)(a + (double)stat[S3_DP]);
            tile[r * S3_DP + S3_DREAL + 1] = 1.f;
        }
    }
    __syncthreads();
    unsigned* out = reinterpret_cast<unsigned*>(Zb + (size_t)blockIdx.x * S3_BLOCK);
    for (int e = threadIdx.x; e < 3 * 2 * 64 * 4; e += 256) {
        const int p = e & 3, st = (e >> 2) & 63, jh = (e >> 8) & 1, q = e >> 9;
        const int g = st >> 4, i = (st & 15) ^ (12 * (g & 1));
        const int row = 8 * (i >> 2) + 4 * jh + (i & 3), col = 32 * q + 8 * g + 2 * p;
        unsigned h, m, l;
        split3_pair(tile[row * S3_DP + col], tile[row * S3_DP + col + 1], h, m, l);
        out[e] = h; out[S3_PLANE / 4 + e] = m; out[2 * S3_PLANE / 4 + e] = l;
    }
    for (int e = threadIdx.x; e < 2 * 64 * 4; e += 256) {
        const int p = e & 3, st = (e >> 2) & 63, jh = (e >> 8) & 1;
        const int g = st >> 4, i = (st & 15) ^ (12 * (g & 1));
        const int row = 8 * (i >> 2) + 4 * jh + (i & 3), col = 96 + 2 * p;
        unsigned h, m, l;
        split3_pair(tile[row * S3_DP + col], tile[row * S3_DP + col + 1], h, m, l);
        out[S3_TAIL / 4 + e] = g < 2 ? h : (g == 2 ? m : l);
    }
}


__global__ __launch_bounds__(256) void centre_tables_kernel(const float* __restrict__ Z, int R, const float* __restrict__ stat, float* __restrict__ Zc) {
    const int lane = threadIdx.x & 63, wpb = blockDim.x >> 6;
    for (int r = blockIdx.x * wpb + (threadIdx.x >> 6); r < R; r += gridDim.x * wpb) {
        const float* z = Z + (size_t)r * S3_DP;
        float* o = Zc + (size_t)r * S3_DP;
        double acc = 0.0;
        float v[2];
#pragma unroll
        for (int t = 0; t < 2; ++t) {
            const int d = lane + 64 * t;
            const float zb = d < S3_DREAL ? stat[d] : 0.f;
            v[t] = d < S3_DREAL ? z[d] - zb : 0.f;
            acc += (double)zb * (double)v[t];
        }
        acc = wave_sum_d(acc);
        o[lane] = v[0];
        const int d1 = lane + 64;
        if (d1 < S3_DP) o[d1] = d1 < S3_DREAL ? v[1] : (d1 == S3_DREAL ? (float)(acc + (double)stat[S3_DP]) : (d1 == S3_DREAL + 1 ? 1.f : 0.f));
    }
}

#ifdef S3_DBG_TIMING
__device__ unsigned long long g_s3_dbg[16];
#define S3_T(i) { const unsigned long long t_ = __builtin_readcyclecounter(); tacc[i] += t_ - tprev; tprev = t_; }
#else
#define S3_T(i)
#endif
struct TSeg { int blk0, jt_lo, jt_hi, old0, lo, hi, fam; };
struct TGroup { int own0, nown, own_old0, own_blk0, blk0, nsplit, nseg; TSeg seg[2]; };
struct TArgs {
    int M; const unsigned char* Zb[4]; int perm[4]; int ngroups; TGroup grp[4];
    float k0, k1, it0, it1, ka;
    const float* beta;
    double* sums;
    const double* gs;
    float* dZ[4];
    double* gamma;
};

#ifndef S3_PAIR
#define S3_PAIR 1
#endif
template <int M, int PER> struct S3PairGaps {
    int slot[M][40];
    constexpr S3PairGaps() : slot{} {
        for (int p = 0; p < M; ++p) {
            int n = 0;
            for (int P = 0; P < 40; ++P) {
                const bool copy = p < M - 1 && P % (20 / PER) == 1 && P / (20 / PER) < 2 * PER;
                slot[p][P] = (P >= 3 && !copy) ? n++ : -1;
            }
        }
    }
};

template <int M, bool GRAD, int WV, int MG, bool GAM, bool LITE, bool FOLD>
__device__ __forceinline__ void sweep3_body(const TArgs& a, const int g) {
    static_assert(!LITE || !GRAD, "LITE: the forward sums only");
    static_assert(!FOLD || (GRAD && WV == 4), "FOLD: the one-wave-per-SIMD gradient sweep only");
    constexpr int NCT = 7;
    constexpr int WAVES = WV, THREADS = WAVES * 64;
    constexpr int OWN = WV * 16;
    constexpr int NCH = LITE ? S3_NCH - S3_PLANE / 1024 : S3_NCH;
    constexpr int KMAX = (NCH + WAVES - 1) / WAVES;
    constexpr int BUF = M * S3_BLOCK;
    constexpr bool PIPE = WV == 4;
#ifndef S3_OWN_IN_S
#define S3_OWN_IN_S 1
#endif
    constexpr bool OWN_IN_S = GRAD && PIPE && S3_OWN_IN_S;
#ifndef S3_SPREAD
#define S3_SPREAD 1
#endif
    constexpr bool SPREAD = OWN_IN_S && S3_SPREAD && !FOLD;
    constexpr bool PAIR_FITS = !(!GRAD && WV == 8 && M == 3 && !LITE);
    constexpr bool PAIR_DEFAULT = !(GRAD && M == 2) && !(!GRAD && M == 4 && !LITE);
    constexpr bool PAIR = PAIR_FITS && (S3_PAIR == 2 || (S3_PAIR == 1 && PAIR_DEFAULT));
    extern __shared__ __attribute__((aligned(16))) unsigned char lds3[];

    const int tid = threadIdx.x, lane = tid & 63, wave = tid >> 6, g4 = lane >> 4, l15 = lane & 15;
    const TGroup& grp = a.grp[g];
    const int wg_in_grp = (int)blockIdx.x - grp.blk0;
    const int nsplit = grp.nsplit, n_ob = (grp.nown + OWN - 1) / OWN, n_units = n_ob * nsplit;
    const int unit = (wg_in_grp & 7) * ((n_units + 7) >> 3) + (wg_in_grp >> 3);
    if ((wg_in_grp >> 3) >= ((n_units + 7) >> 3) || unit >= n_units) return;
    const int split = unit / n_ob;
    const int own0 = grp.own0 + (unit - split * n_ob) * OWN;
    const int own_end = grp.own0 + grp.nown;
    const int wrow0 = own0 + wave * 16;
#ifdef S3_DBG_TIMING
    unsigned long long tacc[8] = {0, 0, 0, 0, 0, 0, 0, 0}, tprev = __builtin_readcyclecounter();
#endif

    u32x4 opl[M][3][3], otl[M][2];
    float beta[M];
    const bool iv = wrow0 + l15 < own_end;
    {
        const int my_i = wrow0 + l15;
        const int rel = (iv ? my_i : own0) - grp.own_old0;
        const int o = rel & 31, oi = 4 * (o >> 3) + (o & 3), ojh = (o >> 2) & 1;
        const size_t off = (size_t)(grp.own_blk0 + (rel >> 5)) * S3_BLOCK;
#pragma unroll
        for (int m = 0; m < M; ++m) {
            const unsigned char* base = a.Zb[m] + off;
#pragma unroll
            for (int p = 0; p < 3; ++p)
#pragma unroll
                for (int q = 0; q < 3; ++q) {
                    const int so = ((q * 2 + ojh) * 64 + s3_slot(g4, oi)) * 16;
                    opl[m][p][q] = iv ? *reinterpret_cast<const u32x4*>(base + p * S3_PLANE + so) : u32x4{0, 0, 0, 0};
                }
            u32x4 th = iv ? *reinterpret_cast<const u32x4*>(base + S3_TAIL + (ojh * 64 + s3_slot(0, oi)) * 16) : u32x4{0, 0, 0, 0};
            u32x4 tm = iv ? *reinterpret_cast<const u32x4*>(base + S3_TAIL + (ojh * 64 + s3_slot(2, oi)) * 16) : u32x4{0, 0, 0, 0};
            u32x4 tl = iv ? *reinterpret_cast<const u32x4*>(base + S3_TAIL + (ojh * 64 + s3_slot(3, oi)) * 16) : u32x4{0, 0, 0, 0};
            const float ksc = a.k1;
            auto rescale = [&](u32x4& ph, u32x4& pm, u32x4& pl) {
#pragma unroll
                for (int d = 0; d < 4; ++d) {
                    const float x0 = (__builtin_bit_cast(float, ph[d] << 16) + __builtin_bit_cast(float, pm[d] << 16)) + __builtin_bit_cast(float, pl[d] << 16);
                    const float x1 = (__builtin_bit_cast(float, ph[d] & 0xffff0000u) + __builtin_bit_cast(float, pm[d] & 0xffff0000u)) + __builtin_bit_cast(float, pl[d] & 0xffff0000u);
                    unsigned nh, nm, nl;
                    split3_pair(x0 * ksc, x1 * ksc, nh, nm, nl);
                    ph[d] = nh; pm[d] = nm; pl[d] = nl;
                }
            };
#pragma unroll
            for (int q = 0; q < 3; ++q) rescale(opl[m][0][q], opl[m][1][q], opl[m][2][q]);
            rescale(th, tm, tl);
            otl[m][0] = g4 == 1 ? tm : th;
            otl[m][1] = g4 == 0 ? tl : (g4 == 2 ? tm : u32x4{0, 0, 0, 0});
#pragma unroll
            for (int t = 0; t < 2; ++t)
                otl[m][t][2] = (otl[m][t][2] >> 16) | (otl[m][t][2] << 16);
        }
    }
#pragma unroll
    for (int m = 0; m < M; ++m) beta[m] = a.beta[a.perm[m]];

    constexpr int NSM = GRAD ? (FOLD ? 1 : MG) : 1;
    f32x4 gacc[GRAD ? MG : 1][NCT], gsm[NSM][NCT];
#pragma unroll
    for (int m = 0; m < (GRAD ? MG : 1); ++m)
#pragma unroll
        for (int ct = 0; ct < NCT; ++ct) gacc[m][ct] = f32x4{0.f, 0.f, 0.f, 0.f};
#pragma unroll
    for (int m = 0; m < NSM; ++m)
#pragma unroll
        for (int ct = 0; ct < NCT; ++ct) gsm[m][ct] = f32x4{0.f, 0.f, 0.f, 0.f};
    float gam[M];
#pragma unroll
    for (int m = 0; m < M; ++m) gam[m] = 0.f;

    const int wave_u = __builtin_amdgcn_readfirstlane(wave);
    const unsigned l16 = (threadIdx.x & 63u) * 16u;
    __amdgpu_buffer_rsrc_t rs[M];
    typedef __attribute__((address_space(3))) unsigned char* lds_ptr;
    constexpr bool LAST_ODD = KMAX * WAVES > NCH || (LITE && KMAX * WAVES > 2 * (S3_PLANE / 1024));
    unsigned crot[M], clast[M], trot[M], brot[M];
    unsigned tile_off = 0, buf_off = 0;
#pragma unroll
    for (int m = 0; m < M; ++m) {
        const int rot = (wave_u + m) & (WAVES - 1);
        int c = rot + (KMAX - 1) * WAVES;
        c = c >= NCH ? c - WAVES : c;
        if (LITE) c = c >= 2 * (S3_PLANE / 1024) ? c + S3_PLANE / 1024 : c;
        crot[m] = (unsigned)rot * 1024u; clast[m] = (unsigned)c * 1024u;
        trot[m] = 0; brot[m] = 0;
    }
    auto set_seg = [&](const TSeg& sgm) {
#pragma unroll
        for (int m = 0; m < M; ++m)
            rs[m] = __builtin_amdgcn_make_buffer_rsrc(const_cast<unsigned char*>(a.Zb[m]) + (size_t)sgm.blk0 * S3_BLOCK, (short)0,
                                                      (int)((unsigned)sgm.jt_hi * (unsigned)S3_BLOCK), 0x00020000);
    };
    auto set_tile = [&](int jt, unsigned char* buf) {
        tile_off = (unsigned)jt * (unsigned)S3_BLOCK;
        buf_off = (unsigned)(buf - lds3);
#pragma unroll
        for (int m = 0; m < M; ++m) {
            trot[m] = tile_off + crot[m]; brot[m] = buf_off + (unsigned)(m * S3_BLOCK) + crot[m];
            asm("" : "+s"(trot[m]), "+s"(brot[m]));
        }
    };
    auto issue_slots = [&](int f_lo, int f_hi) {
#ifdef S3_DBG_NODMA
        return;
#endif
#ifdef S3_DBG_DMA_WAVES
        unsigned dma_mask = S3_DBG_DMA_WAVES;
        asm volatile("" : "+s"(dma_mask));
        if (!((dma_mask >> wave_u) & 1u)) return;
#endif
#pragma unroll
        for (int f = f_lo; f < f_hi; ++f) {
            if (f >= M * KMAX) break;
            const int m = f / KMAX, k = f % KMAX;
            unsigned so, lo;
            if (LAST_ODD && k == KMAX - 1) { so = tile_off + clast[m]; lo = buf_off + (unsigned)(m * S3_BLOCK) + clast[m]; }
            else { so = trot[m] + (unsigned)(k * WAVES * 1024); lo = brot[m] + (unsigned)(k * WAVES * 1024); }
            __builtin_amdgcn_raw_ptr_buffer_load_lds(rs[m], (lds_ptr)lds3 + lo, 16, l16, so, 0, 0);
        }
    };
    auto issue = [&](int jt, unsigned char* buf) { set_tile(jt, buf); issue_slots(0, M * KMAX); };

    const int aoff = s3_slot(g4, l15) * 16;
    const int tr_io = 4 * g4 + (l15 >> 2), tr_cs = l15 & 3;
    const int tr_main = s3_slot(tr_cs >> 1, tr_io) * 16 + (tr_cs & 1) * 8;
    const int tr_tail = S3_TAIL + tr_io * 16 + (tr_cs & 1) * 8;
    const int tr_tail_l = S3_TAIL + (48 + (tr_io ^ 12)) * 16 + (tr_cs & 1) * 8;

#pragma unroll 1
    for (int sg = 0; sg < 2; ++sg) {
        if (sg >= grp.nseg) break;
        const TSeg seg = grp.seg[sg];
        set_seg(seg);
        float c0[M + 1], c1[M + 1];
#pragma unroll
        for (int m = 0; m <= M; ++m) {
            const int mo = m < M ? a.perm[m] : M;
            c0[m] = GRAD ? (float)(a.gs[mo * 8 + seg.fam * 2 + 0] * (double)a.it0) : 0.f;
            c1[m] = GRAD ? (float)(a.gs[mo * 8 + seg.fam * 2 + 1] * (double)a.it1) : 0.f;
        }
        const float ka = a.ka;
        double dsum[M + 1][2];
#pragma unroll
        for (int m = 0; m <= M; ++m) { dsum[m][0] = 0.0; dsum[m][1] = 0.0; }
        float pl0[LITE ? M + 1 : 1], pl1[LITE ? M + 1 : 1];
#pragma unroll
        for (int m = 0; m < (LITE ? M + 1 : 1); ++m) { pl0[m] = 0.f; pl1[m] = 0.f; }

        __syncthreads();
        if (seg.jt_lo + split < seg.jt_hi) issue(seg.jt_lo + split, lds3);
        int it = 0;
#pragma unroll 1
        for (int jt = seg.jt_lo + split; jt < seg.jt_hi; jt += nsplit, ++it) {
            unsigned char* buf = lds3 + (it & 1) * BUF;
            const int j0 = seg.old0 + 32 * jt;
            S3_T(5)
            __syncthreads();
            S3_T(0)
            const int next_jt = jt + nsplit < seg.jt_hi ? jt + nsplit : jt;
            unsigned char* next_buf = lds3 + ((it + 1) & 1) * BUF;
            set_tile(next_jt, next_buf);
            S3_T(1)
            if (GRAD) {
                const int vlo = max(seg.lo - j0, 0), vhi = min(seg.hi - j0, 32);
                if (vlo > 0 || vhi < 32) {
                    for (int x = tid; x < M * 32 * S3_ROWSLOTS; x += THREADS) {
                        const int pc = x % S3_ROWSLOTS, w = (x / S3_ROWSLOTS) % 32, m = x / (S3_ROWSLOTS * 32);
                        if (w >= vlo && w < vhi) continue;
                        const int wjh = (w >> 2) & 1, wi = 4 * (w >> 3) + (w & 3);
                        unsigned char* base = buf + m * S3_BLOCK;
                        if (pc < 36) {
                            const int pl = pc / 12, q = (pc % 12) >> 2, gq = pc & 3;
                            *reinterpret_cast<u32x4*>(base + pl * S3_PLANE + ((q * 2 + wjh) * 64 + s3_slot(gq, wi)) * 16) = u32x4{0, 0, 0, 0};
                        } else {
                            const int gq = pc - 36;
                            *reinterpret_cast<u32x4*>(base + S3_TAIL + (wjh * 64 + s3_slot(gq, wi)) * 16) = u32x4{0, 0, 0, 0};
                        }
                    }
                    __syncthreads();
                }
            }

            f32x4 sacc[M][2];
            float own[M][2][4];
            float cj[2][4];
            auto substep_wait = [&](int ss) {
                if (ss > 0) { __builtin_amdgcn_s_waitcnt(0xc07f); __builtin_amdgcn_sched_barrier(0); }
            };
            constexpr int NSET = (PIPE || PAIR) ? 2 : 1;
            u32x4 at[NSET], ap[NSET][3][3];
            auto ld_one = [&](int ss, int idx) {
                const int e = ss % NSET;
                const unsigned char* ar = buf + (SPREAD ? ss % M : ss >> 1) * S3_BLOCK + (SPREAD ? ss / M : ss & 1) * 1024 + aoff;
                if (idx < 1) at[e] = *reinterpret_cast<const u32x4*>(ar + S3_TAIL);
                else ap[e][2 - (idx - 1) / 3][(idx - 1) % 3] = *reinterpret_cast<const u32x4*>(ar + (2 - (idx - 1) / 3) * S3_PLANE + ((idx - 1) % 3) * 2048);
            };
            auto ld_set = [&](int ss) {
#pragma unroll
                for (int idx = 0; idx < 10; ++idx) if (!(LITE && idx >= 1 && idx <= 3)) ld_one(ss, idx);
            };
            if (PIPE) {
                ld_set(0);
                if (PAIR) ld_set(1);
                __builtin_amdgcn_s_waitcnt(0xc07f);
                __builtin_amdgcn_sched_barrier(0);
            }
            auto lgkm_wait = [&](int n) {
                if (n == 0) __builtin_amdgcn_s_waitcnt(0xc07f);
                else if (n == 6) __builtin_amdgcn_s_waitcnt(0xc67f);
                else if (n == 8) __builtin_amdgcn_s_waitcnt(0xc87f);
                else __builtin_amdgcn_s_waitcnt(0xce7f);
                __builtin_amdgcn_sched_barrier(0);
            };
            if constexpr (SPREAD && PAIR) {
                constexpr int NDS = 2 * M - 2, PER = (M * KMAX + NDS - 1) / NDS, CS = 20 / PER;
                static_assert(2 * PER * CS <= 40 && (M - 1) * 2 * PER >= M * KMAX, "paired S stream: the copies' gaps");
                constexpr int PA[6] = {2, 1, 1, 0, 0, 0}, PB[6] = {0, 1, 0, 2, 1, 0};
                constexpr S3PairGaps<M, PER> GAPS{};
                f32x4 accq[2][2];
                float ot0 = 0.f, ot1 = 0.f, sjt = 0.f, ce0 = 0.f, ce1 = 0.f;
                auto own_step = [&](int ss, int r, int k) {
                    const int mm = ss % M, hh = ss / M;
                    if (mm >= MG) return;
                    const float sv = sacc[mm][hh][r];
                    if (k == 0) ot0 = fexp2(sv * ka);
                    else if (k == 1) ot1 = fexp2(sv);
                    else own[mm][hh][r] = fmaf(c0[mm], ot0, c1[mm] * ot1);
                };
                auto cj_step = [&](int hh, int r, int k) {
                    if (k == 0) {
                        sjt = 0.f;
#pragma unroll
                        for (int mm = 0; mm < M; ++mm) sjt = fmaf(beta[mm], sacc[mm][hh][r], sjt);
                    } else if (k == 1) ce0 = fexp2(sjt * ka);
                    else if (k == 2) ce1 = fexp2(sjt);
                    else cj[hh][r] = c0[M] * ce0 + c1[M] * ce1;
                };
                auto read_s = [&](int ss, const f32x4& acc) {
#pragma unroll
                    for (int r = 0; r < 4; ++r) {
                        float v = acc[r];
                        asm volatile("" : "+v"(v));
                        sacc[ss % M][ss / M][r] = v;
                    }
                };
#pragma unroll
                for (int p = 0; p < M; ++p) {
                    const int pp = p & 1;
                    const bool nxt = p + 1 < M;
                    accq[pp][0] = f32x4{0.f, 0.f, 0.f, 0.f}; accq[pp][1] = f32x4{0.f, 0.f, 0.f, 0.f};
                    if (p > 0) lgkm_wait(6);
#pragma unroll
                    for (int P = 0; P < 40; ++P) {
                        const int x = P >> 1, s = P & 1, m = (2 * p + s) % M;
                        if (x == 0) accq[pp][s] = mfma_b(at[s], otl[m][1], accq[pp][s]);
                        else if (x == 1) accq[pp][s] = mfma_b(at[s], otl[m][0], accq[pp][s]);
                        else accq[pp][s] = mfma_b(ap[s][PA[(x - 2) / 3]][(x - 2) % 3], opl[m][PB[(x - 2) / 3]][(x - 2) % 3], accq[pp][s]);
                        __builtin_amdgcn_sched_barrier(0);
                        if (nxt) {
                            const int sn = 2 * p + 2 + s;
                            if (P >= 2 && P < 4) ld_one(sn, 0);
                            else if (P >= 4 && P < 10) ld_one(sn, 1 + (P - 4) / 2);
                            else if (P >= 16 && P < 22) ld_one(sn, 4 + (P - 16) / 2);
                            else if (P >= 34) ld_one(sn, 7 + (P - 34) / 2);
                        }
                        if (p < M - 1 && (P % CS) == 1 && P / CS < 2 * PER) issue_slots(p * 2 * PER + P / CS, p * 2 * PER + P / CS + 1);
                        if (p > 0) {
                            if (P == 0) read_s(2 * p - 2, accq[pp ^ 1][0]);
                            if (P == 2) read_s(2 * p - 1, accq[pp ^ 1][1]);
                            const int fs = GAPS.slot[p][P];
                            if (fs >= 0) {
                                const int t = nxt ? fs : (fs % 3 < 2 ? 2 * (fs / 3) + fs % 3 : -1);
                                const int qq = (!nxt && fs % 3 == 2) ? fs / 3 : -1;
                                if (t >= 0 && t < 24) own_step(2 * p - 2 + ((t / 3) & 1), t / 6, t % 3);
                                if (qq >= 0 && qq < 12) {
                                    const int r = qq / 3, k = qq % 3;
                                    if (k == 0) { if (r > 0) cj_step(0, r - 1, 3); cj_step(0, r, 0); }
                                    else cj_step(0, r, k);
                                }
                            }
                            if (P == 21) lgkm_wait(nxt ? 14 : 0);
                        }
                        __builtin_amdgcn_sched_barrier(0);
                    }
                }
                read_s(2 * M - 2, accq[(M - 1) & 1][0]);
                read_s(2 * M - 1, accq[(M - 1) & 1][1]);
                cj_step(0, 3, 3);
            } else if constexpr (SPREAD) {
                constexpr int NDS = 2 * M - 2, PER = (M * KMAX + NDS - 1) / NDS;
                constexpr int PA[6] = {2, 1, 1, 0, 0, 0}, PB[6] = {0, 1, 0, 2, 1, 0};
                f32x4 accp[2][2];
                float ot0 = 0.f, ot1 = 0.f, sjt = 0.f, ce0 = 0.f, ce1 = 0.f;
                auto own_step = [&](int mm, int hh, int r, int k) {
                    const float sv = sacc[mm][hh][r];
                    if (k == 0) ot0 = fexp2(sv * ka);
                    else if (k == 1) ot1 = fexp2(sv);
                    else own[mm][hh][r] = fmaf(c0[mm], ot0, c1[mm] * ot1);
                };
                auto cj_step = [&](int hh, int r, int k) {
                    if (k == 0) {
                        sjt = 0.f;
#pragma unroll
                        for (int mm = 0; mm < M; ++mm) sjt = fmaf(beta[mm], sacc[mm][hh][r], sjt);
                    } else if (k == 1) ce0 = fexp2(sjt * ka);
                    else if (k == 2) ce1 = fexp2(sjt);
                    else cj[hh][r] = c0[M] * ce0 + c1[M] * ce1;
                };
#pragma unroll
                for (int ss = 0; ss < 2 * M; ++ss) {
                    const int m = ss % M, jh = ss / M, e = ss % NSET, pa = ss & 1;
                    const int pm = ss > 0 ? (ss - 1) % M : 0, pjh = ss > 0 ? (ss - 1) / M : 0;
                    accp[pa][0] = f32x4{0.f, 0.f, 0.f, 0.f}; accp[pa][1] = f32x4{0.f, 0.f, 0.f, 0.f};
                    substep_wait(ss);
#pragma unroll
                    for (int x = 0; x < 20; ++x) {
                        if (x == 0) accp[pa][0] = mfma_b(at[e], otl[m][1], accp[pa][0]);
                        else if (x == 1) accp[pa][1] = mfma_b(at[e], otl[m][0], accp[pa][1]);
                        else accp[pa][x & 1] = mfma_b(ap[e][PA[(x - 2) / 3]][(x - 2) % 3], opl[m][PB[(x - 2) / 3]][(x - 2) % 3], accp[pa][x & 1]);
                        __builtin_amdgcn_sched_barrier(0);
                        if (ss + 1 < 2 * M && x < 10) ld_one(ss + 1, x);
                        if (ss < NDS && (x % 3) == 1 && (x / 3) < PER) issue_slots(ss * PER + (x / 3), ss * PER + (x / 3) + 1);
                        if (ss > 0) {
                            if (x == 0) { sacc[pm][pjh][0] = accp[pa ^ 1][0][0] + accp[pa ^ 1][1][0]; sacc[pm][pjh][1] = accp[pa ^ 1][0][1] + accp[pa ^ 1][1][1]; }
                            if (x == 2) { sacc[pm][pjh][2] = accp[pa ^ 1][0][2] + accp[pa ^ 1][1][2]; sacc[pm][pjh][3] = accp[pa ^ 1][0][3] + accp[pa ^ 1][1][3]; }
                            if (pm < MG) {
                                constexpr int G0[4] = {3, 8, 12, 16}, G1[4] = {5, 9, 14, 17}, G2[4] = {6, 11, 15, 18};
#pragma unroll
                                for (int r = 0; r < 4; ++r) {
                                    if (x == G0[r]) own_step(pm, pjh, r, 0);
                                    if (x == G1[r]) own_step(pm, pjh, r, 1);
                                    if (x == G2[r]) own_step(pm, pjh, r, 2);
                                }
                            }
                        }
                        if (ss >= NDS) {
                            const int q = (x == 19 ? 5 : (x % 3) == 1 && x <= 13 ? x / 3 : -1);
                            if (q >= 0) {
                                const int qq = (ss - NDS) * 6 + q, r = qq / 3, k = qq % 3;
                                if (k == 0) { if (r > 0) cj_step(0, r - 1, 3); cj_step(0, r, 0); }
                                else cj_step(0, r, k);
                            }
                        }
                        __builtin_amdgcn_sched_barrier(0);
                    }
                }
#pragma unroll
                for (int r = 0; r < 4; ++r) sacc[M - 1][1][r] = accp[(2 * M - 1) & 1][0][r] + accp[(2 * M - 1) & 1][1][r];
                cj_step(0, 3, 3);
            } else if constexpr (PAIR) {
                constexpr int NDS = GRAD ? (2 * M - 2) : 2 * M, PER = (M * KMAX + NDS - 1) / NDS, CS = 20 / PER;
                static_assert(!PIPE || (2 * PER * CS <= 40 && (NDS / 2) * 2 * PER >= M * KMAX), "paired S stream: the copies' gaps");
                constexpr int PA[6] = {2, 1, 1, 0, 0, 0}, PB[6] = {0, 1, 0, 2, 1, 0};
#pragma unroll
// ... 750 lines not shown
```

sgaligner_amd/loss_ops.py:

```python
from __future__ import annotations

import ctypes as _ct

import numpy as _np
import torch

from . import _lib
from . import ops as _o
from .ops import (_SmallCache, _ev_start, _ev_stop, _fingerprint, _h2d, _p, _ptr_array, _req, _stream, get_mfma_mode, DEFERRED_CHECKS, IndexSets,
                  _POINTNET_MODE, _stash_bytes, cast_f32, colsum, gemm)

def _anchor_chunks(a_lo, a_hi, A, n_tables):
    ns = a_hi - a_lo
    if ns <= 0 or A <= 0:
        return []
    rows = max(32, (_stash_bytes() // (4 * A * max(1, n_tables))) // 32 * 32)
    return [(c, min(c + rows, a_hi)) for c in range(a_lo, a_hi, rows)]


def _sym_chunks(A, n_tables):
    return [(lo, hi) for lo, hi, _, _, _ in _sym_jobs([0, A], 0, n_tables)]


def _sym_jobs(cuts, rank, n_tables):
# ... 119 lines not shown
        coef = gout.contiguous().float()
        A = s.A
        slots = 1 + L.sga_loss_slots()
        dparr = (_ct.c_int * nt)(*dps)
        dzs = [torch.zeros((s.R, dp), device=dev, dtype=torch.float32) for dp in dps]
        gs = torch.zeros((nt, 8), device=dev, dtype=torch.float64)
        a_lo, a_hi = ctx.shard
        all16 = nt > 0 and all(dp > 128 for dp in dps)
        chunks = _anchor_chunks(a_lo, a_hi, A, 3 * nt if all16 else nt)
        if chunks:
            cmax = max(hi - lo for lo, hi in chunks)
            m1 = [torch.empty((A * cmax,), device=dev, dtype=torch.float32) for _ in range(nt)]
            gsc = torch.empty((slots, nt, 8), device=dev, dtype=torch.float64)
            ws = ws16 = None
            evb = _ev_start() if all(zh is not None for zh in zhs) else None
            if all16:
                ws = torch.empty((int(L.sga_loss_anchor_f16_ws_bytes(nt, A, cmax)),), device=dev, dtype=torch.uint8)
                if any(zh is not None for zh in zhs):
                    ws16 = torch.empty((int(L.sga_loss_stash_grad_f16_bytes(A, cmax)),), device=dev, dtype=torch.uint8)
            for lo, hi in chunks:
                _lib.check(L.sga_loss_anchor_bwd_f16(_ptr_array(zs), _ptr_array(zhs), dparr, nt, A, _p(sums), ctx.alpha, TAU_ICL, TAU_IAL, _p(coef),
                                                     _ptr_array(m1), _p(gsc), lo, hi, _p(ws) if all16 else None, ws.numel() if all16 else 0, st),
                           'sga_loss_anchor_bwd_f16')
                gs += gsc[0]
                for k in range(nt):
                    if zhs[k] is not None and lo % 8 == 0:
                        _lib.check(L.sga_loss_stash_grad_f16(_p(m1[k]), _p(zts[k]), dps[k], A, s.J1, s.J2, _p(dzs[k]), lo, hi, _p(ws16) if ws16 is not None else None,
                                                             ws16.numel() if ws16 is not None else 0, st), 'sga_loss_stash_grad_f16')
                    else:
                        _lib.check(L.sga_loss_stash_grad(_p(m1[k]), _p(zs[k]), A, dps[k], _p(dzs[k]), lo, hi, st), 'sga_loss_stash_grad')
            del m1, ws, ws16
            _ev_stop(evb, 'wide16_aa_bwd', (A, sum(dps)))
        gs = _allreduce_sum(gs, ctx.reduce)
        grads = []
        for k in range(nt):
            z, dp, dz = zs[k], dps[k], dzs[k]
            ev = _ev_start() if dp <= 128 else None
            if zhs[k] is not None:
                need = int(L.sga_loss_neg_grad_f16_bytes(A, s.J1, s.J2))
                have = max(min(need, _stash_bytes()), int(L.sga_loss_neg_grad_f16_bytes(min(A, 128), s.J1, s.J2)))
                stash = torch.empty((have,), device=dev, dtype=torch.uint8)
                ev16 = _ev_start()
                _lib.check(L.sga_loss_neg_grad_f16(_p(zhs[k]), _p(zts[k]), dp, A, s.J1, s.J2, TAU_ICL, TAU_IAL, gs[k].data_ptr(), _p(dz),
                                                   _p(stash), have, a_lo, a_hi, st), 'sga_loss_neg_grad_f16')
                _ev_stop(ev16, 'wide16_grad', (A, s.J1, s.J2, dp))
                del stash
            elif dp > 128 and _o.WIDE_STASH and a_lo == 0 and a_hi == A:
                need = int(L.sga_loss_neg_grad_wide_floats(A, s.J1, s.J2))
                have = max(min(need, _stash_bytes() // 4), 2 * (s.J1 + s.J2) * min(A, 32))
                stash = torch.empty((have,), device=dev, dtype=torch.float32)
                _lib.check(L.sga_loss_neg_grad_wide(_p(z), dp, A, s.J1, s.J2, TAU_ICL, TAU_IAL, gs[k].data_ptr(), _p(dz), _p(stash), have, st),
                           'sga_loss_neg_grad_wide')
                del stash
            else:
                _lib.check(L.sga_loss_neg_grad_shard(_p(z), dp, A, s.J1, s.J2, TAU_ICL, TAU_IAL, gs[k].data_ptr(), _p(dz), a_lo, a_hi, st),
                           'sga_loss_neg_grad')
            _ev_stop(ev, 'sweep_kernel<4,4,grad>', (A, s.J1, s.J2, dp))
            t, d = ctx.shapes[k]
            de = torch.zeros((t, d), device=dev, dtype=torch.float32)
            _lib.check(L.sga_loss_scatter(_p(dz), _p(z), _p(nrms[k]), _p(s.idx), s.R, d, dp, _p(de), st), 'sga_loss_scatter')
            grads.append(de)
            dzs[k] = None
        return (None, None, None, None, *grads)


def contrastive_terms(tables, data_dict, alpha=ALPHA, shard=None, reduce=None):
    s = IndexSets.of(data_dict, tables[0].device, int(tables[0].shape[0]))
    return ContrastiveTermsFn.apply(s, alpha, shard, reduce, *tables), s


class LossHeadFn(torch.autograd.Function):

    @staticmethod
    def forward(ctx, sums, lv_ial, lv_icl, n_anchors, z_ial, alpha_ial, zoom):
        M = int(lv_ial.numel())
        if sums.dtype not in (torch.float32, torch.float64) or sums.numel() != 3 * M + 1 or lv_icl.numel() != M:
            raise RuntimeError('sgaligner_amd: LossHeadFn takes the 3M+1 loss terms (float32/float64) and two [M] log_vars vectors')
        sums = sums.contiguous()
        la, lc = _req(lv_ial.detach(), 'log_vars (ial)'), _req(lv_icl.detach(), 'log_vars (icl)')
        out = torch.empty((4,), device=sums.device, dtype=torch.float64)
        inv_aa = 1.0 / float(n_anchors * n_anchors) if n_anchors else float('nan')
        ctx.consts = (M, inv_aa, float(z_ial), float(alpha_ial), float(zoom))
        ctx.f64 = int(sums.dtype == torch.float64)
        _lib.check(_lib.lib().sga_loss_head_fwd(_p(sums), ctx.f64, _p(la), _p(lc), *ctx.consts, _p(out), _stream()), 'sga_loss_head_fwd')
        ctx.save_for_backward(sums, la, lc)
        return out

    @staticmethod
    def coef_hint(lv_ial, lv_icl, n_anchors, z_ial, alpha_ial, zoom):
        M = int(lv_ial.numel())
        la, lc = _req(lv_ial.detach(), 'log_vars (ial)'), _req(lv_icl.detach(), 'log_vars (icl)')
        dev = la.device
        key = (str(dev), M)
        cst = LossHeadFn._hint_const.get(key)
        if cst is None:
            cst = LossHeadFn._hint_const[key] = (torch.tensor([1.0, 0.0, 0.0, 0.0], device=dev, dtype=torch.float64),
                                                 torch.zeros((3 * M + 1,), device=dev, dtype=torch.float32))
        inv_aa = 1.0 / float(n_anchors * n_anchors) if n_anchors else float('nan')
        d = torch.empty((3 * M + 1,), device=dev, dtype=torch.float32)
        junk = torch.empty((2, M), device=dev, dtype=torch.float32)
        _lib.check(_lib.lib().sga_loss_head_bwd(_p(cst[0]), _p(cst[1]), 0, _p(la), _p(lc), M, inv_aa, float(z_ial), float(alpha_ial), float(zoom),
                                                _p(d), _p(junk[0]), _p(junk[1]), _stream()), 'sga_loss_head_bwd')
        return d

    _hint_const = {}

    @staticmethod
    def backward(ctx, gout):
        sums, la, lc = ctx.saved_tensors
        M = ctx.consts[0]
        gout = gout.to(torch.float64).contiguous()
        dsums = torch.empty_like(sums)
        dla, dlc = torch.empty_like(la), torch.empty_like(lc)
        _lib.check(_lib.lib().sga_loss_head_bwd(_p(gout), _p(sums), ctx.f64, _p(la), _p(lc), *ctx.consts, _p(dsums), _p(dla), _p(dlc),
                                                _stream()), 'sga_loss_head_bwd')
        return dsums, dla, dlc, None, None, None, None


class LossGroups:

    def __init__(self, data_dict, b, device):
        ca = _np.asarray(data_dict['e1i_count']).reshape(-1).astype(_np.int64)
        c1 = _np.asarray(data_dict['e1j_count']).reshape(-1).astype(_np.int64)
        c2 = _np.asarray(data_dict['e2j_count']).reshape(-1).astype(_np.int64)
        if not (len(ca) == len(c1) == len(c2)):
            raise RuntimeError('sgaligner_amd: e1i_count / e1j_count / e2j_count disagree')
        if int(b) < 1:
            raise RuntimeError(f'sgaligner_amd: loss_group must be a positive number of pairs (got {b})')
        B = len(ca)
        cuts = list(range(0, B, int(b))) + [B]
        oa, o1, o2 = (_np.concatenate([[0], _np.cumsum(c)]) for c in (ca, c1, c2))
        g = _np.zeros((len(cuts) - 1, 8), dtype=_np.int32)
        for k, (lo, hi) in enumerate(zip(cuts[:-1], cuts[1:])):
            g[k, :6] = (oa[lo], oa[hi] - oa[lo], o1[lo], o1[hi] - o1[lo], o2[lo], o2[hi] - o2[lo])
        size = 2 * g[:, 1].astype(_np.int64) * (g[:, 1].astype(_np.int64) + g[:, 3] + g[:, 5])
        soff = _np.concatenate([[0], _np.cumsum(size)]).astype(_np.int64)
        self.G, self.b = int(g.shape[0]), int(b)
        self.host = g
        self.s_total = int(soff[-1])
        self.groups = torch.from_numpy(g).to(device)
        self.soff = torch.from_numpy(soff).to(device)
        self.na = torch.from_numpy(g[:, 1].astype(_np.float32)).to(device)
        self.totals = (int(oa[-1]), int(o1[-1]), int(o2[-1]))

    _cache = _SmallCache()

    @staticmethod
    def of(data_dict, b, device):
        device = torch.device(device)
        key = _fingerprint([_np.asarray(data_dict[k]) for k in ('e1i_count', 'e1j_count', 'e2j_count')], (str(device), int(b)))
        return LossGroups._cache.get(key, lambda: LossGroups(data_dict, b, device))


class GroupedContrastiveFn(torch.autograd.Function):

    @staticmethod
    def forward(ctx, index_sets, groups, alpha, beta, *tables):
        L = _lib.lib()
        M = len(tables)
        nt = M + 1 if M > 1 else 1
        no = nt + (2 * M if M > 1 else 0)
        tables = [_req(t.contiguous(), f'table[{i}]') for i, t in enumerate(tables)]
        dev = tables[0].device
        s, gr = index_sets, groups
        if (s.A, s.J1, s.J2) != gr.totals:
            raise RuntimeError('sgaligner_amd: per-pair counts (e1i_count/e1j_count/e2j_count) do not add up to the index sets')
        st = _stream()
        dp = 104
        T = tables[0].shape[0]
        zs, nrms = [], []
        poison = torch.zeros((1,), device=dev, dtype=torch.float32)
        for e in tables:
            d = e.shape[1]
            if d > dp:
                raise RuntimeError('sgaligner_amd: loss_group needs emb_dim <= 104')
            z = torch.empty((max(s.R, 1), dp), device=dev, dtype=torch.float32)
            nrm = torch.empty((max(s.R, 1),), device=dev, dtype=torch.float32)
            _lib.check(L.sga_loss_gather(_p(e), T, d, _p(s.idx), s.R, _p(z), dp, _p(nrm), st), 'sga_loss_gather')
            _lib.check(L.sga_loss_check_norms(_p(nrm), s.R, _p(poison), st), 'sga_loss_check_norms')
            zs.append(z); nrms.append(nrm)
        if beta is not None:
            beta = _req(beta.contiguous(), 'beta')
        S = torch.empty((M * max(gr.s_total, 1),), device=dev, dtype=torch.float32)
        sums = torch.empty((max(gr.G, 1), nt, 8), device=dev, dtype=torch.float64)
        out = torch.zeros((max(gr.G, 1), no), device=dev, dtype=torch.float64)
        _lib.check(L.sga_group_loss_fwd(_ptr_array(zs), M, _p(beta), s.A, s.J1, _p(gr.groups), gr.G, _p(gr.soff), gr.s_total,
                                        float(alpha), TAU_ICL, TAU_IAL, _p(S), _p(sums), _p(out), int(_o.GROUP_LOSS_VALU), st), 'sga_group_loss_fwd')
        ctx.s, ctx.gr, ctx.alpha, ctx.M = s, gr, float(alpha), M
        ctx.shapes = [tuple(t.shape) for t in tables]
        ctx.has_beta = beta is not None
        ctx.save_for_backward(S, sums, *( [beta] if beta is not None else []), *zs, *nrms)
        return out[:gr.G].float() + poison

    @staticmethod
    def backward(ctx, gout):
        L = _lib.lib()
        s, gr, M = ctx.s, ctx.gr, ctx.M
        saved = list(ctx.saved_tensors)
        S, sums = saved[0], saved[1]
        beta = saved[2] if ctx.has_beta else None
        rest = saved[3:] if ctx.has_beta else saved[2:]
        zs, nrms = rest[:M], rest[M:]
        dev = S.device
        st = _stream()
        dp = 104
        coef = gout.contiguous().float()
        C = S.clone()
        dzs = [torch.zeros((max(s.R, 1), dp), device=dev, dtype=torch.float32) for _ in range(M)]
        gamma = torch.zeros((max(gr.G, 1), M), device=dev, dtype=torch.float64)
        _lib.check(L.sga_group_loss_bwd(_ptr_array(zs), M, _p(beta), s.A, s.J1, _p(gr.groups), gr.G, _p(gr.soff), gr.s_total,
                                        ctx.alpha, TAU_ICL, TAU_IAL, _p(C), _p(sums), _p(coef), _ptr_array(dzs), _p(gamma), int(_o.GROUP_LOSS_VALU), st),
                   'sga_group_loss_bwd')
        grads = []
        for k in range(M):
            t, d = ctx.shapes[k]
            de = torch.zeros((t, d), device=dev, dtype=torch.float32)
            _lib.check(L.sga_loss_scatter(_p(dzs[k]), _p(zs[k]), _p(nrms[k]), _p(s.idx), s.R, d, dp, _p(de), st), 'sga_loss_scatter')
            grads.append(de)
        gbeta = gamma[:gr.G].sum(0).float() if ctx.has_beta else None
        return (None, None, None, gbeta, *grads)


def grouped_contrastive_terms(tables, fusion_weight, data_dict, b, alpha=ALPHA):
    dev = tables[0].device
    s = IndexSets.of(data_dict, dev, int(tables[0].shape[0]))
    gr = LossGroups.of(data_dict, b, dev)
    beta = None
    if len(tables) > 1:
        w = torch.softmax(fusion_weight.reshape(-1), dim=0)
        beta = (w * w) / (w * w).sum()
    return GroupedContrastiveFn.apply(s, gr, alpha, beta, *tables), gr


def group_data_dicts(data_dict, b):
    ca, c1, c2 = (_np.asarray(data_dict[k]).reshape(-1) for k in ('e1i_count', 'e1j_count', 'e2j_count'))
    oa, o1, o2 = (_np.concatenate([[0], _np.cumsum(c)]) for c in (ca, c1, c2))
    B = len(ca)
    out = []
    for lo in range(0, B, int(b)):
        hi = min(B, lo + int(b))
        out.append({'e1i': _np.asarray(data_dict['e1i'])[oa[lo]:oa[hi]], 'e2i': _np.asarray(data_dict['e2i'])[oa[lo]:oa[hi]],
                    'e1j': _np.asarray(data_dict['e1j'])[o1[lo]:o1[hi]], 'e2j': _np.asarray(data_dict['e2j'])[o2[lo]:o2[hi]]})
    return out


def _sums_lite(ns, J1, J2):
    if _o.BF16X6_SUMS_LITE is not None:
        return bool(_o.BF16X6_SUMS_LITE)
    return ns * min(J1, J2) >= _o.BF16X6_SUMS_LITE_MIN_TERMS


def _allreduce_sum(t, group_reduce):
    if group_reduce is not None:
        group_reduce(t)
    return t


def _call(name, *args):
    _lib.check(getattr(_lib.lib(), name)(*args, _stream()), name)


class PlainTier:
    images, FILL = (), None
    sweep_on, stash_on = 'zs', 'zs'
    SUMS, GRAD = ('sga_loss_multi_sums', 'loss_multi_sums'), ('sga_loss_multi_grad', 'loss_multi_grad')

    def __init__(self, s, zs, dmax, saved=None):
        self.s, self.zs, self.dmax, self.M, self.geom = s, list(zs), dmax, len(zs), (s.A, s.J1, s.J2)
        if saved is None:
            self.alloc()
        else:
            for i, name in enumerate(self.images):
                setattr(self, name, list(saved[i * self.M:(i + 1) * self.M]))

    def saved(self):
        return [t for name in self.images for t in getattr(self, name)]

    def alloc(self):
        """The image buffers, their slack rows zeroed."""

    def prepare(self):
        for k, z in enumerate(self.zs if self.FILL else ()):
            _call(self.FILL, _p(z), *self.geom, *(_p(getattr(self, name)[k]) for name in self.images))

    def _sweep(self, entry, event, beta, io, a_lo, a_hi, *tail):
        width = (self.dmax,) if self.sweep_on == 'zs' else ()
        ev = _ev_start()
        _call(entry, _ptr_array(getattr(self, self.sweep_on)), self.M, *width, _p(beta), *self.geom, TAU_ICL, TAU_IAL, *io, a_lo, a_hi, *tail)
        _ev_stop(ev, event, (a_hi - a_lo, *self.geom, self.M, *map(bool, tail)))

    def sums(self, beta, sums, a_lo, a_hi):
        self._sweep(*self.SUMS, beta, (_p(sums),), a_lo, a_hi)

    def grad(self, beta, gs, dzs, gam_neg, a_lo, a_hi):
        self._sweep(*self.GRAD, beta, (_p(gs), _ptr_array(dzs), _p(gam_neg)), a_lo, a_hi)

    def stash(self, k, m1, m2, dz, job, sym):
        b = _p(getattr(self, self.stash_on)[k])
        if sym:
            _call('sga_loss_stash_grad_symx', _p(m1), _p(m2), b, self.s.A, 104, _p(dz), *job)
        else:
            _call('sga_loss_stash_grad', _p(m1), b, self.s.A, 104, _p(dz), *job[:2])

    def scatter(self, k, dz, nrm, d, de):
        _call('sga_loss_scatter', _p(dz), _p(self.zs[k]), _p(nrm), _p(self.s.idx), self.s.R, d, 104, _p(de))


class CentredTier(PlainTier):
    images, FILL, sweep_on, stash_on = ('zc', 'stat'), 'sga_loss_centre_tables', 'zc', 'zc'
    SUMS, GRAD = ('sga_loss_multi_sums_centred', 'loss_multi_sums'), ('sga_loss_multi_grad_centred', 'loss_multi_grad')

    def alloc(self):
        dev, nst = self.zs[0].device, int(_lib.lib().sga_loss_centre_bytes())
        self.stat = [torch.empty((nst,), device=dev, dtype=torch.uint8) for _ in self.zs]
        self.zc = [torch.empty((self.s.R + 32, 104), device=dev, dtype=torch.float32) for _ in self.zs]
        for zc in self.zc:
            zc[self.s.R:].zero_()

    def scatter(self, k, dz, nrm, d, de):
        _call('sga_loss_scatter_tangent_stat', _p(dz), _p(self.zs[k]), _p(nrm), _p(self.s.idx), self.s.R, d, _p(self.stat[k]), _p(de))


class PlanesTier(PlainTier):
    images, FILL, sweep_on, stash_on = ('planes', 'zc'), 'sga_loss_split3_tables', 'planes', 'zc'
    SUMS, GRAD = ('sga_loss_multi_sums_bf16x6', 'loss_multi_sums_bf16x6'), ('sga_loss_multi_grad_bf16x6', 'loss_multi_grad_bf16x6')

    def alloc(self):
        dev, nb = self.zs[0].device, _lib.lib().sga_loss_split3_bytes(*self.geom)
        self.planes = [torch.empty((nb,), device=dev, dtype=torch.uint8) for _ in self.zs]
        self.zc = [torch.empty((2 * self.s.A + 32, 104), device=dev, dtype=torch.float32) for _ in self.zs]
        for zc in self.zc:
            zc[2 * self.s.A:].zero_()

    def sums(self, beta, sums, a_lo, a_hi):
        self._sweep(*self.SUMS, beta, (_p(sums),), a_lo, a_hi, 1 if _sums_lite(a_hi - a_lo, *self.geom[1:]) else 0)

    def stash(self, k, m1, m2, dz, job, sym):
        if not _o.BF16X6_STASH:
            return super().stash(k, m1, m2, dz, job, sym)
        _call('sga_loss_stash_grad_symx_bf16x6', _p(m1), _p(m2), _p(self.planes[k]), *self.geom, _p(dz), *job)

    def scatter(self, k, dz, nrm, d, de):
        _call('sga_loss_scatter_tangent', _p(dz), _p(self.zs[k]), _p(nrm), _p(self.s.idx), *self.geom, d, _p(self.planes[k]), _p(de))


TIERS = {'plain': PlainTier, 'centred': CentredTier, 'planes': PlanesTier}


def _aa_walk(s, tier, beta, sums, alpha, coef, dzs, walk, sym, out=None):
    L = _lib.lib()
    M, A, nt = tier.M, s.A, tier.M + 1
    dev = sums.device
    slots = 1 + L.sga_loss_slots()
    n_terms = nt + 2 * M if out is not None else 0
    zz = torch.zeros((n_terms + nt * 8 + M,), device=dev, dtype=torch.float64)
    terms, gs, gam = zz[:n_terms], zz[n_terms:n_terms + nt * 8].view(nt, 8), zz[n_terms + nt * 8:]
    if not walk:
        return terms, gs, gam
    jobs = walk if sym else [(lo, hi, 0, A, A) for lo, hi in walk]
    gsc = torch.empty((slots + 1, nt, 8), device=dev, dtype=torch.float64)
    gam2 = torch.empty((slots, M), device=dev, dtype=torch.float64)
    fl = max(((jh - jl) + max(0, jh - mir)) * (hi - lo) for lo, hi, jl, jh, mir in jobs)
    buf = [torch.empty((fl,), device=dev, dtype=torch.float32) for _ in range(M)]
    zarr = _ptr_array(tier.zs)
    for lo, hi, jl, jh, mir in jobs:
        n1 = (jh - jl) * (hi - lo)
        m1, m2 = [b[:n1] for b in buf], [b[n1:] for b in buf]
        has2 = mir < jh
        if sym:
            _call('sga_loss_anchor_multi_bwd_symx', zarr, M, _p(beta), A, _p(sums), alpha, TAU_ICL, TAU_IAL, _p(coef), _ptr_array(m1),
                  _ptr_array(m2) if has2 else (_ct.c_void_p * M)(), _p(gsc), _p(gam2), lo, hi, jl, jh, mir, _p(out))
        else:
            _call('sga_loss_anchor_multi_bwd', zarr, M, _p(beta), A, _p(sums), alpha, TAU_ICL, TAU_IAL, _p(coef), _ptr_array(m1), _p(gsc), _p(gam2),
                  lo, hi, _p(out))
        if out is not None:
            terms += out[:n_terms]
        gs += gsc[0]
        gam += gam2[0]
        for k in range(M):
            tier.stash(k, m1[k], m2[k] if has2 else None, dzs[k], (lo, hi, jl, jh, mir), sym)
    return terms, gs, gam


class FusedContrastiveFn(torch.autograd.Function):

    @staticmethod
    def forward(ctx, index_sets, alpha, shard, reduce, coef_hint, beta, *tables):
        L = _lib.lib()
        M = len(tables)
        nt = M + 1
        tables = [_req(t.contiguous(), f'table[{i}]') for i, t in enumerate(tables)]
        beta = _req(beta.contiguous(), 'beta')
        dev = tables[0].device
        s = index_sets
        a_lo, a_hi = (0, s.A) if shard is None else (int(shard[0]), int(shard[1]))
        T = tables[0].shape[0]
        st = _stream()
        dp = 104
        dmax = max(e.shape[1] for e in tables)
        zs, nrms = [], []
        poison = torch.zeros((1,), device=dev, dtype=torch.float32)
        for k, e in enumerate(tables):
            d = e.shape[1]
            if d > dp:
                raise RuntimeError('sgaligner_amd: the fused loss path needs emb_dim <= 104')
            z = torch.empty((s.R + 32, dp), device=dev, dtype=torch.float32)
            z[s.R:].zero_()
            nrm = torch.empty((s.R,), device=dev, dtype=torch.float32)
            _lib.check(L.sga_loss_gather(_p(e), T, d, _p(s.idx), s.R, _p(z), dp, _p(nrm), st), 'sga_loss_gather')
            _lib.check(L.sga_loss_check_norms(_p(nrm), s.R, _p(poison), st), 'sga_loss_check_norms')
            zs.append(z); nrms.append(nrm)
        slots = 1 + L.sga_loss_slots()
        sums = torch.empty((slots, nt, 8), device=dev, dtype=torch.float64)
        tier = TIERS['plain' if dmax > 100 else 'centred' if get_mfma_mode() == 'f32' else 'planes'](s, zs, dmax)
        tier.prepare()
        tier.sums(beta, sums, a_lo, a_hi)
        sums = _allreduce_sum(sums[0].contiguous(), reduce)
        out = torch.empty((slots * (nt + 2 * M),), device=dev, dtype=torch.float64)
        onepass = coef_hint is not None and _o.FUSED_AA_ONEPASS and s.A >= _o.ONEPASS_MIN_ANCHORS
        extra = []
        if onepass:
            coef = _req(coef_hint.contiguous(), 'coef_hint')
            dz_all = torch.zeros((M, s.R, dp), device=dev, dtype=torch.float32)
            cuts, crank = (shard[2], shard[3]) if (shard is not None and len(shard) >= 4) else (([0, s.A], 0) if (a_lo == 0 and a_hi == s.A) else (None, 0))
            sym = _o.AA_SYMMETRIC and cuts is not None and all(c % 32 == 0 for c in cuts[:-1]) and cuts[-1] == s.A \
                and cuts[crank] == a_lo and cuts[crank + 1] == a_hi
            walk = _sym_jobs(list(cuts), crank, M) if sym else []
            if sym and len(cuts) == 2 and len(walk) < 2:
                sym = False
            if not sym:
                walk = _anchor_chunks(a_lo, a_hi, s.A, M)
            terms, gs_aa, gam_aa = _aa_walk(s, tier, beta, sums, float(alpha), coef, dz_all, walk, sym, out=out)
            out = _allreduce_sum(terms.clone(), reduce)
            extra = [dz_all, gs_aa.clone(), gam_aa.clone(), coef]
        else:
            _call('sga_loss_anchor_multi_fwd', _ptr_array(zs), M, _p(beta), s.A, _p(sums), float(alpha), TAU_ICL, TAU_IAL, _p(out), a_lo, a_hi)
            out = _allreduce_sum(out[:nt + 2 * M].contiguous(), reduce)
        ctx.s, ctx.alpha, ctx.M, ctx.shard, ctx.reduce = s, float(alpha), M, (a_lo, a_hi), reduce
        ctx.shapes = [tuple(t.shape) for t in tables]
        ctx.tier, ctx.dmax, ctx.onepass = type(tier), dmax, onepass
        ctx.save_for_backward(sums, beta, *zs, *nrms, *tier.saved(), *extra)
        return out.float() + poison

    @staticmethod
    def backward(ctx, gout):
        L = _lib.lib()
        s, M = ctx.s, ctx.M
        a_lo, a_hi = ctx.shard
        sums, beta, *rest = ctx.saved_tensors
        zs, nrms = rest[:M], rest[M:2 * M]
        tier = ctx.tier(s, zs, ctx.dmax, saved=rest[2 * M:])
        dev = sums.device
        dp = 104
        A = s.A
        coef = gout.contiguous().float()
        slots = 1 + L.sga_loss_slots()
        gam_neg = torch.empty((slots, M), device=dev, dtype=torch.float64)
        if ctx.onepass:
            dz_aa, gs_aa, gam_aa, hint = rest[-4:]
            hh = torch.dot(hint, hint)
            u = torch.dot(coef, hint) / hh
            mismatch = (coef - u * hint).abs().max() > 1e-4 * hh.sqrt()
            u = torch.where(mismatch, torch.full_like(u, float('nan')), u)
            if _o.VALIDATE:
                bad = mismatch.to(torch.int32).reshape(1)
                DEFERRED_CHECKS.submit_fn(bad, lambda v: None if v[0] == 0 else (
                    'sgaligner_amd: the gradient that reached the loss terms is not a multiple of the one OverallLoss announced at forward time '
                    "(backward through something other than loss_dict['loss'] up to a factor); set sgaligner_amd.ops.FUSED_AA_ONEPASS = False"))
            dz_all = dz_aa * u.float()
            dzs = [dz_all[k] for k in range(M)]
            gs = _allreduce_sum(gs_aa * u, ctx.reduce)
            gam_anc = gam_aa * u
        else:
            dz_all = torch.zeros((M, s.R, dp), device=dev, dtype=torch.float32)
            dzs = [dz_all[k] for k in range(M)]
            _, gs, gam_anc = _aa_walk(s, tier, beta, sums, ctx.alpha, coef, dzs, _anchor_chunks(a_lo, a_hi, A, M), False)
            gs = _allreduce_sum(gs, ctx.reduce)
        tier.grad(beta, gs, dzs, gam_neg, a_lo, a_hi)
        grads = []
        same = all(sh == ctx.shapes[0] for sh in ctx.shapes)
        de_all = torch.zeros((M,) + tuple(ctx.shapes[0]), device=dev, dtype=torch.float32) if same else None
        for k in range(M):
            t, d = ctx.shapes[k]
            de = de_all[k] if same else torch.zeros((t, d), device=dev, dtype=torch.float32)
            tier.scatter(k, dzs[k], nrms[k], d, de)
            grads.append(de)
        gbeta = (gam_neg[0] + gam_anc).float()
        return (None, None, None, None, None, gbeta, *grads)


def fused_contrastive_terms(tables, fusion_weight, data_dict, alpha=ALPHA, shard=None, reduce=None, coef_hint=None):
    s = IndexSets.of(data_dict, tables[0].device, int(tables[0].shape[0]))
    w = torch.softmax(fusion_weight.reshape(-1), dim=0)
    beta = (w * w) / (w * w).sum()
    if coef_hint is not None and not (torch.is_grad_enabled() and (beta.requires_grad or any(t.requires_grad for t in tables))):
        coef_hint = None
    return FusedContrastiveFn.apply(s, alpha, shard, reduce, coef_hint, beta, *tables), s
```

sgaligner_amd/ops.py:

```python
from __future__ import annotations

import torch

from . import _lib


_raw_stream = getattr(torch._C, '_cuda_getCurrentRawStream', None)


def _stream():
    if _raw_stream is not None:
        return _raw_stream(torch.cuda.current_device())
    return torch.cuda.current_stream().cuda_stream


def _req(t: torch.Tensor, name: str, dtype=torch.float32):
    if not isinstance(t, torch.Tensor) or not t.is_cuda:
        raise RuntimeError(f'sgaligner_amd: `{name}` must be a HIP device tensor (got '
                           f'{t.device if isinstance(t, torch.Tensor) else type(t)}); there is no CPU path')
    if t.dtype != dtype:
        raise RuntimeError(f'sgaligner_amd: `{name}` must be {dtype} (got {t.dtype})')
    if not t.is_contiguous():
        raise RuntimeError(f'sgaligner_amd: `{name}` must be contiguous')
    if t.data_ptr() % 16:
# ... 72 lines not shown
        raise RuntimeError(f'sgaligner_amd: unsupported feature dtype {x.dtype}')
    x = x.contiguous()
    out = torch.empty(x.shape, device=x.device, dtype=torch.float32)
    _lib.check(_lib.lib().sga_cast_f64_f32(_p(x), _p(out), x.numel(), _stream()), 'sga_cast_f64_f32')
    return out


class LinearFn(torch.autograd.Function):

    @staticmethod
    def forward(ctx, x, weight, bias):
        if not x.is_cuda:
            raise RuntimeError('sgaligner_amd.LinearFn: HIP device tensor required; there is no CPU path')
        if x.dtype not in (torch.float32, torch.float64):
            raise RuntimeError(f'sgaligner_amd.LinearFn: features must be float32 or float64 (the collated bag-of-words '
                               f'tables), got {x.dtype}')
        x = x.contiguous()
        _req(weight, 'weight'); _req(bias, 'bias')
        t, k = x.shape
        if x.dim() != 2 or k != weight.shape[1]:
            raise RuntimeError(f'sgaligner_amd.LinearFn: x is {tuple(x.shape)} but weight is {tuple(weight.shape)}')
        y = gemm(x, weight, False, True, t, weight.shape[0], k, bias=bias)
        ctx.save_for_backward(x, weight)
        return y

    @staticmethod
    def backward(ctx, gy):
        x, weight = ctx.saved_tensors
        gy = gy.contiguous()
        t, k = x.shape
        n = weight.shape[0]
        gx = gw = gb = None
        if ctx.needs_input_grad[0]:
            gx = gemm(gy, weight.t().contiguous(), False, True, t, k, n)
        if ctx.needs_input_grad[1]:
            if k % 4 and t >= 4096:
                kp = (k + 3) // 4 * 4
                xp = torch.zeros((t, kp), device=x.device, dtype=torch.float32)
                xp[:, :k] = x
                gw = gemm(gy, xp, True, False, n, kp, t)[:, :k].contiguous()
            else:
                gw = gemm(gy, cast_f32(x), True, False, n, k, t)
        if ctx.needs_input_grad[2]:
            gb = colsum(gy)
        return gx, gw, gb


def linear(x, weight, bias):
    return LinearFn.apply(x, weight, bias)


import ctypes as _ct


def _ptr_array(tensors):
    arr = (_ct.c_void_p * len(tensors))(*[(t.data_ptr() if t is not None else None) for t in tensors])
    return arr


def _ev_start():
    if KERNEL_EVENTS is None:
        return None
    ev = (torch.cuda.Event(enable_timing=True), torch.cuda.Event(enable_timing=True))
    ev[0].record()
    return ev


def _ev_stop(ev, key, shape):
    if ev is not None:
        ev[1].record()
        KERNEL_EVENTS.setdefault(key, []).append(ev + (shape,))


class FusionFn(torch.autograd.Function):

    @staticmethod
    def forward(ctx, weight, *embs):
        m = len(embs)
        embs = [_req(e.contiguous(), f'embs[{i}]') for i, e in enumerate(embs)]
        w = _req(weight.contiguous(), 'fusion.weight')
        t, d = embs[0].shape
        for e in embs:
            if tuple(e.shape) != (t, d):
                raise RuntimeError('sgaligner_amd.FusionFn: all modality tables must share one shape')
        joint = torch.empty((t, m * d), device=w.device, dtype=torch.float32)
        arr = _ptr_array(embs)
        ev = _ev_start()
        _lib.check(_lib.lib().sga_fusion_fwd(arr, m, _p(w), _p(joint), t, d, _stream()), 'sga_fusion_fwd')
        _ev_stop(ev, 'fusion_fwd', (t, d, m))
        ctx.save_for_backward(w, *embs)
        return joint

    @staticmethod
    def backward(ctx, gj):
        w, *embs = ctx.saved_tensors
        m = len(embs)
        t, d = embs[0].shape
        gj = gj.contiguous()
        gembs = [torch.empty_like(e) for e in embs]
        gw = torch.empty_like(w)
        nb = _lib.lib().sga_fusion_bwd_workspace_bytes(m)
        ws = torch.empty((nb,), device=w.device, dtype=torch.uint8)
        ev = _ev_start()
        _lib.check(_lib.lib().sga_fusion_bwd(_ptr_array(embs), m, _p(w), _p(gj), _ptr_array(gembs), _p(gw), t, d,
                                             _p(ws), nb, _stream()), 'sga_fusion_bwd')
        _ev_stop(ev, 'fusion_bwd', (t, d, m))
        return (gw, *gembs)


class FusionVarFn(torch.autograd.Function):

    @staticmethod
    def forward(ctx, weight, *embs):
        m = len(embs)
        embs = [_req(e.contiguous(), f'embs[{i}]') for i, e in enumerate(embs)]
        w = _req(weight.contiguous(), 'fusion.weight')
        t = embs[0].shape[0]
        for e in embs:
            if e.dim() != 2 or e.shape[0] != t:
                raise RuntimeError('sgaligner_amd.FusionVarFn: all modality tables must have the same number of rows')
        widths = (_ct.c_int32 * m)(*[int(e.shape[1]) for e in embs])
        joint = torch.empty((t, sum(widths)), device=w.device, dtype=torch.float32)
        ev = _ev_start()
        _lib.check(_lib.lib().sga_fusion_var_fwd(_ptr_array(embs), m, widths, _p(w), _p(joint), t, _stream()), 'sga_fusion_var_fwd')
        _ev_stop(ev, 'fusion_var_fwd', (t, tuple(widths), m))
        ctx.save_for_backward(w, *embs)
        return joint

    @staticmethod
    def backward(ctx, gj):
        w, *embs = ctx.saved_tensors
        m = len(embs)
        t = embs[0].shape[0]
        gj = gj.contiguous()
        widths = (_ct.c_int32 * m)(*[int(e.shape[1]) for e in embs])
        gembs = [torch.empty_like(e) for e in embs]
        gw = torch.empty_like(w)
        nb = _lib.lib().sga_fusion_bwd_workspace_bytes(m)
        ws = torch.empty((nb,), device=w.device, dtype=torch.uint8)
        ev = _ev_start()
        _lib.check(_lib.lib().sga_fusion_var_bwd(_ptr_array(embs), m, widths, _p(w), _p(gj), _ptr_array(gembs), _p(gw), t,
                                                 _p(ws), nb, _stream()), 'sga_fusion_var_bwd')
        _ev_stop(ev, 'fusion_var_bwd', (t, tuple(widths), m))
        return (gw, *gembs)


def fusion(weight, embs):
    if len({int(e.shape[-1]) for e in embs}) > 1:
        return FusionVarFn.apply(weight, *embs)
    return FusionFn.apply(weight, *embs)


import hashlib as _hashlib
import os as _os
from collections import OrderedDict as _OrderedDict

import numpy as _np


def _fingerprint(arrays, extra=()):
    h = _hashlib.blake2b(digest_size=16)
    shapes = []
    for a in arrays:
        a = _np.ascontiguousarray(a)
        shapes.append((a.shape, a.dtype.str))
        h.update(a.reshape(-1).view(_np.uint8))
    return (h.digest(), tuple(shapes), tuple(extra))


class _SmallCache:

    def __init__(self, n=4):
        self.n, self.d = n, _OrderedDict()

    def get(self, key, make):
        v = self.d.get(key)
        if v is None:
            v = make()
            self.d[key] = v
            while len(self.d) > self.n:
                self.d.popitem(last=False)
        else:
            self.d.move_to_end(key)
        return v

    def clear(self):
        self.d.clear()


_H2D_RING = {'n': 0, 'bufs': [None] * 8, 'evs': [None] * 8}


def _h2d(host_array, device):
    arr = _np.ascontiguousarray(host_array)
    t = torch.from_numpy(arr)
    device = torch.device(device)
    if device.type != 'cuda':
        return t.to(device)
    slot = _H2D_RING['n'] % len(_H2D_RING['bufs'])
    _H2D_RING['n'] += 1
    buf, ev = _H2D_RING['bufs'][slot], _H2D_RING['evs'][slot]
    if ev is not None:
        ev.synchronize()
    nbytes = arr.nbytes
    if buf is None or buf.numel() < nbytes:
        buf = torch.empty((max(nbytes * 2, 4096),), dtype=torch.uint8).pin_memory()
        _H2D_RING['bufs'][slot] = buf
    if nbytes:
        _np.copyto(buf.numpy()[:nbytes], arr.reshape(-1).view(_np.uint8))
    out = buf[:nbytes].view(t.dtype).view(t.shape).to(device, non_blocking=True)
    ev = torch.cuda.Event()
    ev.record()
    _H2D_RING['evs'][slot] = ev
    return out


VALIDATE = _os.environ.get('SGA_VALIDATE', '1') != '0'


class _DeferredChecks:

    def __init__(self):
        self.pending = []
        self.free = []

    def submit_fn(self, dev_tensor, verdict):
        n = int(dev_tensor.numel())
        host = self.free.pop() if self.free else torch.empty((2,), dtype=torch.int64).pin_memory()
        view = host[:n] if dev_tensor.dtype == torch.int64 else host.view(torch.int32)[:n]
        view.copy_(dev_tensor.reshape(-1), non_blocking=True)
        ev = torch.cuda.Event()
        ev.record()
        self.pending.append((ev, host, view, verdict))

    def submit(self, minmax_dev, upper, what):
        upper = int(upper)
        self.submit_fn(minmax_dev, lambda v: (what % (v[0], v[1], upper)) if (v[0] < 0 or v[1] >= upper) else None)

    def poll(self, wait=False):
        keep = []
        err = None
        for ev, host, view, verdict in self.pending:
            if wait:
                ev.synchronize()
            if wait or ev.query():
                msg = verdict([int(x) for x in view])
                self.free.append(host)
                if msg is not None and err is None:
                    err = msg
            else:
                keep.append((ev, host, view, verdict))
        self.pending = keep
        if err is not None:
            raise RuntimeError(err)

    def flush(self):
        self.poll(wait=True)


DEFERRED_CHECKS = _DeferredChecks()


class IndexSets:

    def __init__(self, data_dict, device, n_rows=None):
        arrs = [_np.ascontiguousarray(_np.asarray(data_dict[k]).astype(_np.int32)) for k in ('e1i', 'e2i', 'e1j', 'e2j')]
        if arrs[0].shape != arrs[1].shape:
            raise RuntimeError('sgaligner_amd: e1i and e2i must have the same length')
        self.A, self.J1, self.J2 = int(arrs[0].shape[0]), int(arrs[2].shape[0]), int(arrs[3].shape[0])
        self.R = 2 * self.A + self.J1 + self.J2
        host = _np.concatenate(arrs)
        if VALIDATE and host.size:
            lo, hi = int(host.min()), int(host.max())
            if lo < 0 or (n_rows is not None and hi >= n_rows):
                raise RuntimeError(f'sgaligner_amd: e1i/e2i/e1j/e2j hold object indices in [{lo}, {hi}] but the embedding '
                                   f'tables have {n_rows} rows')
        self.idx = _h2d(host, device)

    _cache = _SmallCache()

    @staticmethod
    def from_device(idx, A, J1, J2):
        s = IndexSets.__new__(IndexSets)
        s.A, s.J1, s.J2 = int(A), int(J1), int(J2)
        s.R = 2 * s.A + s.J1 + s.J2
        if idx.dtype != torch.int32 or idx.numel() != s.R:
            raise RuntimeError('sgaligner_amd: packed index array must be int32 of length 2A+J1+J2')
        s.idx = idx.contiguous()
        return s

    @staticmethod
    def of(data_dict, device, n_rows=None):
        pre = data_dict.get('_sga_index_sets') if isinstance(data_dict, dict) else None
        if pre is not None:
            return pre
        device = torch.device(device)
        key = _fingerprint([_np.asarray(data_dict[k]) for k in ('e1i', 'e2i', 'e1j', 'e2j')], (str(device), n_rows))
        return IndexSets._cache.get(key, lambda: IndexSets(data_dict, device, n_rows))


FUSED_AA_ONEPASS = True
AA_SYMMETRIC = True
ONEPASS_MIN_ANCHORS = 256
WIDE_STASH = True
KERNEL_EVENTS = None

def _default_stash_bytes():
    env = _os.environ.get('SGA_STASH_BYTES')
    if env:
        return int(env)
    try:
        if torch.cuda.is_available() and torch.cuda.get_device_properties(torch.cuda.current_device()).total_memory >= (128 << 30):
            return 16 << 30
    except Exception:
        pass
    return 4 << 30


STASH_BYTES = None
_stash_default = []


def _stash_bytes():
    if STASH_BYTES is not None:
        return int(STASH_BYTES)
    if not _stash_default:
        _stash_default.append(_default_stash_bytes())
    return _stash_default[0]


POINTNET_SPLIT_MAX_OBJECTS = 1023
BF16X6_SUMS_LITE = {'1': True, '0': False}.get(_os.environ.get('SGA_BF16X6_SUMS_LITE', ''), None)
BF16X6_SUMS_LITE_MIN_TERMS = 1 << 24
BF16X6_STASH = _os.environ.get('SGA_BF16X6_STASH', '1') != '0'
GAT_COMPLETE_FAST_PATH = _os.environ.get('SGA_GAT_COMPLETE', '1') != '0'
SIMRANK_F16 = False


_REEXPORT = {
    'pointnet_ops': ('pointnet_bn_fusable', 'pointnet_forward', 'PointNetFn', 'pointnet'),
    'loss_ops': ('_anchor_chunks', '_sym_chunks', '_sym_jobs', 'SWEEP_GRAD_INFO', 'SWEEP_SUMS_INFO', 'TAU_ICL', 'TAU_IAL', 'ALPHA', 'ContrastiveTermsFn',
                 'contrastive_terms', 'LossHeadFn', 'LossGroups', 'GroupedContrastiveFn', 'grouped_contrastive_terms', 'group_data_dicts',
                 '_allreduce_sum', 'FusedContrastiveFn', 'fused_contrastive_terms'),
    'gat_ops': ('GraphBatch', '_attn_fwd', '_attn_bwd', '_elu', 'MultiGATFn', 'multi_gat', 'gat_lds_nodes', '_attn_fwd_hc', '_attn_bwd_hc',
                'GATLayerFn', 'EluFn', 'multi_gat_layers'),
    'gcn_ops': ('gcn_aggregate', 'MultiGCNFn', 'multi_gcn'),
    'nca_ops': ('NCAFn', 'nca_loss'),
    'rank_ops': ('PairLayout', 'QueryBlocks', 'simrank', 'pair_metrics'),
}
_WHERE = {name: mod for mod, names in _REEXPORT.items() for name in names}


def __getattr__(name):
    mod = _WHERE.get(name)
    if mod is None:
        raise AttributeError(f"module 'sgaligner_amd.ops' has no attribute {name!r}")
    import importlib
    value = getattr(importlib.import_module('.' + mod, __package__), name)
    globals()[name] = value
    return value
```

Baseline: 990.2.

## Add bf16x6 split-plane anchor-anchor backward kernel with shared epilogue

Adds a new anchor-anchor backward kernel that reads the precomputed three-plane bf16 tables and forms the anchor-by-anchor similarities with bf16 MFMAs, six per product, instead of the fp32 path. The epilogue and the split-plane layout helpers move into shared headers so both kernels use them. The Python tier class sends aligned jobs to the new kernel when at least 1024 anchors and at most three tables are present, and falls back otherwise. The aim is to speed up the anchor similarity matmul by reusing the split planes already built for the sweeps, at the cost of extra code paths and alignment conditions.

```diff
diff --git a/include/sgaligner_hip.h b/include/sgaligner_hip.h
--- a/include/sgaligner_hip.h
+++ b/include/sgaligner_hip.h
@@ -148,6 +148,10 @@
                              const void* Zb, float* dE, void* stream);
 int sga_loss_stash_grad_symx_bf16x6(const float* M1, const float* M2, const void* Zb, int A, int J1, int J2, float* dZ,
                                     int a_lo, int a_hi, int j_lo, int j_hi, int mir, void* stream);
+int sga_loss_anchor_multi_bwd_symx_bf16x6(const void* const* Zb, int M, const float* beta, int A, int J1, int J2, const double* sums,
+                                          float alpha, float tau_icl, float tau_ial, const float* coef, float* const* M1, float* const* M2,
+                                          double* gs, double* gamma, int a_lo, int a_hi, int j_lo, int j_hi, int mir, double* out_terms,
+                                          void* stream);
 
 int sga_group_loss_fwd(const float* const* Z, int M, const float* beta, int A, int J1, const int32_t* groups, int G,
                        const int64_t* s_off, int64_t s_total, float alpha, float tau_icl, float tau_ial, float* S,
diff --git a/sgaligner_amd/_build.py b/sgaligner_amd/_build.py
--- a/sgaligner_amd/_build.py
+++ b/sgaligner_amd/_build.py
@@ -24,6 +24,7 @@
               'loss_pertable.hip': ['-fno-slp-vectorize'],
               'loss_anchor.hip': ['-fno-slp-vectorize'],
               'sweep3.hip': ['-fno-slp-vectorize'],
+              'anchor3.hip': ['-fno-slp-vectorize'],
               'pointnet.hip': ['-fno-slp-vectorize'],
               'nnsearch.hip': ['-ffp-contract=off'],
               'visibility.hip': ['-ffp-contract=off']}
diff --git a/sgaligner_amd/_lib.py b/sgaligner_amd/_lib.py
--- a/sgaligner_amd/_lib.py
+++ b/sgaligner_amd/_lib.py
@@ -115,6 +115,7 @@
     'sga_loss_split3_tables': (I, [P, I, I, I, P, P, P]),
     'sga_loss_scatter_tangent': (I, [P, P, P, P, I, I, I, I, P, P, P]),
     'sga_loss_stash_grad_symx_bf16x6': (I, [P, P, P, I, I, I, P, I, I, I, I, I, P]),
+    'sga_loss_anchor_multi_bwd_symx_bf16x6': (I, [P, I, P, I, I, I, P, F, F, F, P, P, P, P, P, I, I, I, I, I, P, P]),
     'sga_loss_multi_sums_bf16x6': (I, [P, I, P, I, I, I, F, F, P, I, I, I, P]),
     'sga_loss_multi_grad_bf16x6': (I, [P, I, P, I, I, I, F, F, P, P, P, I, I, P]),
     'sga_group_loss_fwd': (I, [P, I, P, I, I, P, I, P, c_int64, F, F, F, P, P, P, I, P]),
diff --git a/sgaligner_amd/csrc/aa_epilogue.h b/sgaligner_amd/csrc/aa_epilogue.h
--- /dev/null
+++ b/sgaligner_amd/csrc/aa_epilogue.h
@@ -0,0 +1,233 @@
+#pragma once
+#include "loss_math.h"
+
+namespace {
+
+struct AnchorMultiArgs {
+    int M, A, i_lo, i_hi, nsplit;
+    const float* Z[4];
+    const float* beta;
+    const double* sums;
+    const float* inv;
+    float alpha, kc, ki, itc, iti;
+    double* out;
+    const float* coef;
+    float* M1[4];
+    double* gs;
+    double* gamma;
+    int j_lo;
+    float* M2[4];
+    int j_hi, mir;
+};
+
+__global__ void inv_sums_kernel(const double* __restrict__ sums, float* __restrict__ inv, int n) {
+    const int i = blockIdx.x * blockDim.x + threadIdx.x;
+    if (i < n) inv[i] = (float)(1.0 / (sums[i] + 1e-9));
+}
+
+template <int M, bool TERMS>
+__device__ __forceinline__ void aa_flush(const AnchorMultiArgs& a, const float* inv_s, const int lane, const int slot,
+                                         float (&acc_gs)[M + 1][8], float (&acc_gam)[M], float (&acc_out)[TERMS ? 3 * M + 1 : 1]) {
+    constexpr int NT = M + 1;
+    if (TERMS) {
+#pragma unroll
+        for (int e = 0; e < NT + 2 * M; ++e) {
+            const float v = wave_sum(acc_out[TERMS ? e : 0]);
+            if (lane == 0 && v != 0.f) atomicAdd(a.out + (NT + 2 * M) * (1 + slot) + e, (double)v);
+            acc_out[TERMS ? e : 0] = 0.f;
+        }
+    }
+#pragma unroll
+    for (int k = 0; k < NT; ++k)
+#pragma unroll
+        for (int e = 0; e < 8; ++e) {
+            const float iv2 = inv_s[k * 8 + e];
+            const float v = -iv2 * iv2 * wave_sum(acc_gs[k][e]);
+            if (lane == 0 && v != 0.f) atomicAdd(a.gs + NT * 8 * (1 + slot) + k * 8 + e, (double)v);
+            acc_gs[k][e] = 0.f;
+        }
+#pragma unroll
+    for (int m = 0; m < M; ++m) {
+        const float v = wave_sum(acc_gam[m]);
+        if (lane == 0 && v != 0.f) atomicAdd(a.gamma + M * (1 + slot) + m, (double)v);
+        acc_gam[m] = 0.f;
+    }
+}
+
+template <int M, bool TERMS, bool MASKED>
+__device__ __forceinline__ void aa_epilogue(const AnchorMultiArgs& a, const float* inv_s, const float (&beta)[M], const f32x4 (&P)[M],
+                                            const f32x4 (&Q)[M], float (&acc_gs)[M + 1][8], float (&acc_gam)[M], float (&acc_out)[TERMS ? 3 * M + 1 : 1],
+                                            const int jg, const int JH, const bool iv, const int my_i, const int ns) {
+    constexpr int NT = M + 1;
+    auto CF = [&](int e) { return a.coef[e]; };
+    const float* js = inv_s + M * 8;
+    const float cJ = CF(M);
+#pragma unroll
+    for (int r = 0; r < 4; ++r) {
+        const int j = jg + r;
+        const bool ok = !MASKED || (iv && (j < JH));
+        const float okf = (!MASKED || ok) ? 1.f : 0.f;
+        float xj = 0.f, yj = 0.f;
+#pragma unroll
+        for (int m = 0; m < M; ++m) { xj = fmaf(beta[m], P[m][r], xj); yj = fmaf(beta[m], Q[m][r], yj); }
+        float gJ, EA = 0.f, EB = 0.f;
+        {
+            const float dx = fexp2(xj * a.kc), dy = fexp2(yj * a.kc);
+            const GP Ax = g_parts(dx, js[0], js[2]), Bx = g_parts(dx, js[4], js[6]);
+            const float qAy = g_val(dy, js[0], js[2]), qBy = g_val(dy, js[4], js[6]);
+            const float denA = a.alpha * Ax.q + (1.f - a.alpha) * qBy;
+            const float wA = okf * (-cJ * a.alpha) * frcp(denA) * dx;
+            const float wB = okf * (-cJ * (1.f - a.alpha)) * frcp(a.alpha * qAy + (1.f - a.alpha) * Bx.q) * dx;
+            if (TERMS) acc_out[TERMS ? M : 0] = fmaf(okf, -flog(denA), acc_out[TERMS ? M : 0]);
+            gJ = fmaf(wA, Ax.dd, wB * Bx.dd) * a.itc;
+            acc_gs[M][0] = fmaf(wA, Ax.p, acc_gs[M][0]); acc_gs[M][2] = fmaf(wA, Ax.r, acc_gs[M][2]);
+            acc_gs[M][4] = fmaf(wB, Bx.p, acc_gs[M][4]); acc_gs[M][6] = fmaf(wB, Bx.r, acc_gs[M][6]);
+        }
+        const float dji = fexp2(xj * a.ki);
+        const GP MA = g_parts(dji, js[1], js[3]), MB = g_parts(dji, js[5], js[7]);
+        const float lqma = flog(MA.q), lqmb = flog(MB.q);
+        float gx[M];
+#pragma unroll
+        for (int m = 0; m < M; ++m) {
+            const float* is = inv_s + m * 8;
+            const float c = CF(m), ca = CF(NT + m), cb = CF(NT + M + m);
+            const float x = P[m][r], y = Q[m][r];
+            const float dx = fexp2(x * a.kc), dy = fexp2(y * a.kc);
+            const GP Ax = g_parts(dx, is[0], is[2]), Bx = g_parts(dx, is[4], is[6]);
+            const float qAy = g_val(dy, is[0], is[2]), qBy = g_val(dy, is[4], is[6]);
+            const float denA = a.alpha * Ax.q + (1.f - a.alpha) * qBy;
+            const float wA = okf * (-c * a.alpha) * frcp(denA) * dx;
+            const float wB = okf * (-c * (1.f - a.alpha)) * frcp(a.alpha * qAy + (1.f - a.alpha) * Bx.q) * dx;
+            if (TERMS) acc_out[TERMS ? m : 0] = fmaf(okf, -flog(denA), acc_out[TERMS ? m : 0]);
+            float gxm = fmaf(wA, Ax.dd, wB * Bx.dd) * a.itc;
+            acc_gs[m][0] = fmaf(wA, Ax.p, acc_gs[m][0]); acc_gs[m][2] = fmaf(wA, Ax.r, acc_gs[m][2]);
+            acc_gs[m][4] = fmaf(wB, Bx.p, acc_gs[m][4]); acc_gs[m][6] = fmaf(wB, Bx.r, acc_gs[m][6]);
+            const float dm = fexp2(x * a.ki);
+            const GP OA = g_parts(dm, is[1], is[3]), OB = g_parts(dm, is[5], is[7]);
+            const float xA = okf * __expf(OA.q), xB = okf * __expf(OB.q);
+            const float eA = ca * xA, eB = cb * xB;
+            if (TERMS) {
+                acc_out[TERMS ? NT + m : 0] = fmaf(xA, OA.q - lqma, acc_out[TERMS ? NT + m : 0]);
+                acc_out[TERMS ? NT + M + m : 0] = fmaf(xB, OB.q - lqmb, acc_out[TERMS ? NT + M + m : 0]);
+            }
+            const float tA = eA * (OA.q - lqma + 1.f) * dm, tB = eB * (OB.q - lqmb + 1.f) * dm;
+            gxm = fmaf(fmaf(tA, OA.dd, tB * OB.dd), a.iti, gxm);
+            acc_gs[m][1] = fmaf(tA, OA.p, acc_gs[m][1]); acc_gs[m][3] = fmaf(tA, OA.r, acc_gs[m][3]);
+            acc_gs[m][5] = fmaf(tB, OB.p, acc_gs[m][5]); acc_gs[m][7] = fmaf(tB, OB.r, acc_gs[m][7]);
+            EA += eA; EB += eB;
+            gx[m] = gxm;
+        }
+        {
+            const float uA = -EA * frcp(MA.q) * dji, uB = -EB * frcp(MB.q) * dji;
+            gJ = fmaf(fmaf(uA, MA.dd, uB * MB.dd), a.iti, gJ);
+            acc_gs[M][1] = fmaf(uA, MA.p, acc_gs[M][1]); acc_gs[M][3] = fmaf(uA, MA.r, acc_gs[M][3]);
+            acc_gs[M][5] = fmaf(uB, MB.p, acc_gs[M][5]); acc_gs[M][7] = fmaf(uB, MB.r, acc_gs[M][7]);
+        }
+#pragma unroll
+        for (int m = 0; m < M; ++m) {
+            acc_gam[m] = fmaf(gJ, P[m][r], acc_gam[m]);
+            if (ok) a.M1[m][(size_t)(j - a.j_lo) * ns + (my_i - a.i_lo)] = fmaf(beta[m], gJ, gx[m]);
+        }
+#pragma unroll
+        for (int k = 0; k < NT; ++k)
+#pragma unroll
+            for (int e = 0; e < 8; ++e) asm volatile("" : "+v"(acc_gs[k][e]));
+#pragma unroll
+        for (int m = 0; m < M; ++m) asm volatile("" : "+v"(acc_gam[m]));
+        if (TERMS) {
+#pragma unroll
+            for (int e = 0; e < NT + 2 * M; ++e) asm volatile("" : "+v"(acc_out[TERMS ? e : 0]));
+        }
+        __builtin_amdgcn_sched_barrier(0);
+    }
+}
+
+template <int M>
+__device__ __forceinline__ void aa_epilogue_sym(const AnchorMultiArgs& a, const float* inv_s, const float (&beta)[M], const f32x4 (&P)[M],
+                                                const f32x4 (&Q)[M], float (&acc_gs)[M + 1][8], float (&acc_gam)[M], float (&acc_out)[3 * M + 1],
+                                                const int jg, const int JH, const bool iv, const int my_i, const int ns) {
+    constexpr int NT = M + 1;
+    constexpr bool TERMS = true;
+    auto CF = [&](int e) { return a.coef[e]; };
+    const float* js = inv_s + M * 8;
+#pragma unroll
+    for (int r = 0; r < 4; ++r) {
+        const int j = jg + r;
+        const bool ok = iv && (j < JH);
+        const float okf = ok ? 1.f : 0.f;
+        float xj = 0.f, yj = 0.f;
+#pragma unroll
+        for (int m = 0; m < M; ++m) { xj = fmaf(beta[m], P[m][r], xj); yj = fmaf(beta[m], Q[m][r], yj); }
+        float gci[NT][2];
+#pragma unroll
+        for (int k = 0; k < NT; ++k) {
+            const float* is = inv_s + k * 8;
+            const float x = k < M ? P[k < M ? k : 0][r] : xj, y = k < M ? Q[k < M ? k : 0][r] : yj;
+            const float c = CF(k);
+            const float dx = fexp2(x * a.kc), dy = fexp2(y * a.kc);
+            const GP Ax = g_parts(dx, is[0], is[2]), Bx = g_parts(dx, is[4], is[6]);
+            const GP Ay = g_parts(dy, is[0], is[2]), By = g_parts(dy, is[4], is[6]);
+            const float den1 = a.alpha * Ax.q + (1.f - a.alpha) * By.q;
+            const float den2 = a.alpha * Ay.q + (1.f - a.alpha) * Bx.q;
+            const float r1 = okf * -c * frcp(den1), r2 = okf * -c * frcp(den2);
+            const float wAx = a.alpha * r1 * dx, wBx = (1.f - a.alpha) * r2 * dx;
+            const float wAy = a.alpha * r2 * dy, wBy = (1.f - a.alpha) * r1 * dy;
+            acc_out[TERMS ? k : 0] = fmaf(okf, -(flog(den1) + flog(den2)), acc_out[TERMS ? k : 0]);
+            gci[k][0] = fmaf(wAx, Ax.dd, wBx * Bx.dd) * a.itc;
+            gci[k][1] = fmaf(wAy, Ay.dd, wBy * By.dd) * a.itc;
+            acc_gs[k][0] = fmaf(wAx, Ax.p, fmaf(wAy, Ay.p, acc_gs[k][0])); acc_gs[k][2] = fmaf(wAx, Ax.r, fmaf(wAy, Ay.r, acc_gs[k][2]));
+            acc_gs[k][4] = fmaf(wBx, Bx.p, fmaf(wBy, By.p, acc_gs[k][4])); acc_gs[k][6] = fmaf(wBx, Bx.r, fmaf(wBy, By.r, acc_gs[k][6]));
+#pragma unroll
+            for (int e = 0; e < 8; e += 2) asm volatile("" : "+v"(acc_gs[k][e]));
+            asm volatile("" : "+v"(acc_out[TERMS ? k : 0]));
+            __builtin_amdgcn_sched_barrier(0);
+        }
+#pragma unroll
+        for (int dir = 0; dir < 2; ++dir) {
+            const float vj = dir ? yj : xj;
+            const float dji = fexp2(vj * a.ki);
+            const GP MA = g_parts(dji, js[1], js[3]), MB = g_parts(dji, js[5], js[7]);
+            const float lqma = flog(MA.q), lqmb = flog(MB.q);
+            float gx[M], EA = 0.f, EB = 0.f;
+#pragma unroll
+            for (int m = 0; m < M; ++m) {
+                const float* is = inv_s + m * 8;
+                const float ca = CF(NT + m), cb = CF(NT + M + m);
+                const float v = dir ? Q[m][r] : P[m][r];
+                const float dm = fexp2(v * a.ki);
+                const GP OA = g_parts(dm, is[1], is[3]), OB = g_parts(dm, is[5], is[7]);
+                const float xA = okf * __expf(OA.q), xB = okf * __expf(OB.q);
+                const float eA = ca * xA, eB = cb * xB;
+                acc_out[TERMS ? NT + m : 0] = fmaf(xA, OA.q - lqma, acc_out[TERMS ? NT + m : 0]);
+                acc_out[TERMS ? NT + M + m : 0] = fmaf(xB, OB.q - lqmb, acc_out[TERMS ? NT + M + m : 0]);
+                const float tA = eA * (OA.q - lqma + 1.f) * dm, tB = eB * (OB.q - lqmb + 1.f) * dm;
+                gx[m] = fmaf(fmaf(tA, OA.dd, tB * OB.dd), a.iti, gci[m][dir]);
+                acc_gs[m][1] = fmaf(tA, OA.p, acc_gs[m][1]); acc_gs[m][3] = fmaf(tA, OA.r, acc_gs[m][3]);
+                acc_gs[m][5] = fmaf(tB, OB.p, acc_gs[m][5]); acc_gs[m][7] = fmaf(tB, OB.r, acc_gs[m][7]);
+                EA += eA; EB += eB;
+            }
+            const float uA = -EA * frcp(MA.q) * dji, uB = -EB * frcp(MB.q) * dji;
+            const float gJ = fmaf(fmaf(uA, MA.dd, uB * MB.dd), a.iti, gci[M][dir]);
+            acc_gs[M][1] = fmaf(uA, MA.p, acc_gs[M][1]); acc_gs[M][3] = fmaf(uA, MA.r, acc_gs[M][3]);
+            acc_gs[M][5] = fmaf(uB, MB.p, acc_gs[M][5]); acc_gs[M][7] = fmaf(uB, MB.r, acc_gs[M][7]);
+            float* const* dst = dir ? a.M2 : a.M1;
+            const size_t off = (size_t)(j - (dir ? a.mir : a.j_lo)) * ns + (my_i - a.i_lo);
+#pragma unroll
+            for (int m = 0; m < M; ++m) {
+                acc_gam[m] = fmaf(gJ, dir ? Q[m][r] : P[m][r], acc_gam[m]);
+                if (ok) dst[m][off] = fmaf(beta[m], gJ, gx[m]);
+            }
+#pragma unroll
+            for (int k = 0; k < NT; ++k)
+#pragma unroll
+                for (int e = 1; e < 8; e += 2) asm volatile("" : "+v"(acc_gs[k][e]));
+#pragma unroll
+            for (int m = 0; m < M; ++m) asm volatile("" : "+v"(acc_gam[m]));
+#pragma unroll
+            for (int e = NT; e < NT + 2 * M; ++e) asm volatile("" : "+v"(acc_out[TERMS ? e : 0]));
+            __builtin_amdgcn_sched_barrier(0);
+        }
+    }
+}
+
+}
diff --git a/sgaligner_amd/csrc/anchor3.hip b/sgaligner_amd/csrc/anchor3.hip
--- /dev/null
+++ b/sgaligner_amd/csrc/anchor3.hip
@@ -0,0 +1,184 @@
+#include "mfma_tiles.h"
+#include <type_traits>
+
+#include "s3_layout.h"
+#include "aa_epilogue.h"
+
+namespace {
+
+constexpr int A3_THREADS = 512;
+constexpr int A3_TW = 4;
+constexpr int A3_NOP = 11;
+
+struct Anchor3Args {
+    AnchorMultiArgs a;
+    const unsigned char* Zb[4];
+    int nbA;
+};
+
+__device__ __forceinline__ u32x4 a3_ld(const unsigned char* p) { return *reinterpret_cast<const u32x4*>(p); }
+
+template <int M, bool TERMS, bool SYM>
+__global__ __launch_bounds__(A3_THREADS) void anchor3_bwd_kernel(Anchor3Args A3) {
+    static_assert(!SYM || TERMS, "symmetric mode: one-pass build");
+    static_assert(M == 2 || M == 3, "two or three tables");
+    const AnchorMultiArgs& a = A3.a;
+    extern __shared__ __attribute__((aligned(16))) u32x4 own3[];
+    const float* __restrict__ inv_s = a.inv;
+    const int tid = threadIdx.x, lane = tid & 63, wave = tid >> 6, g = lane >> 4, l15 = lane & 15;
+    const int A = a.A, ns = a.i_hi - a.i_lo;
+    const int JH = SYM ? a.j_hi : A;
+    const int ib = blockIdx.x / a.nsplit, split = blockIdx.x % a.nsplit;
+    const int i0 = a.i_lo + ib * 32;
+    const int ih = wave & 1, tw = wave >> 1;
+    const int my_i = i0 + ih * 16 + l15;
+    const bool iv = my_i < a.i_hi;
+
+    if (tid < 256) {
+        const int ln = tid & 63, hh = (tid >> 6) & 1, side = tid >> 7;
+        const int gg = ln >> 4, o = hh * 16 + (ln & 15);
+        const int ojh = (o >> 2) & 1, oi = 4 * (o >> 3) + (o & 3);
+        const int so = (ojh * 64 + s3_slot(gg, oi)) * 16;
+#pragma unroll
+        for (int m = 0; m < M; ++m) {
+            const unsigned char* base = A3.Zb[m] + (size_t)(side * A3.nbA + (i0 >> 5)) * S3_BLOCK;
+            u32x4* dst = own3 + (((m * 2 + side) * 2 + hh) * A3_NOP) * 64 + ln;
+            const unsigned char* tb = base + S3_TAIL + ojh * 1024;
+            const u32x4 th = a3_ld(tb + s3_slot(0, oi) * 16), tm = a3_ld(tb + s3_slot(2, oi) * 16), tl = a3_ld(tb + s3_slot(3, oi) * 16);
+            u32x4 ot[2];
+            s3_own_tails(th, tm, tl, gg, ot);
+            dst[0] = ot[1];
+            dst[64] = ot[0];
+#pragma unroll
+            for (int p = 0; p < 3; ++p)
+#pragma unroll
+                for (int q = 0; q < 3; ++q) dst[(2 + p * 3 + q) * 64] = a3_ld(base + p * S3_PLANE + q * 2048 + so);
+        }
+    }
+    __syncthreads();
+    float beta[M];
+#pragma unroll
+    for (int m = 0; m < M; ++m) beta[m] = a.beta[m];
+
+    constexpr int NT = M + 1;
+    float acc_gs[NT][8], acc_gam[M];
+#pragma unroll
+    for (int k = 0; k < NT; ++k)
+#pragma unroll
+        for (int e = 0; e < 8; ++e) acc_gs[k][e] = 0.f;
+#pragma unroll
+    for (int m = 0; m < M; ++m) acc_gam[m] = 0.f;
+    float acc_out[TERMS ? NT + 2 * M : 1];
+#pragma unroll
+    for (int e = 0; e < (TERMS ? NT + 2 * M : 1); ++e) acc_out[e] = 0.f;
+    int tiles_done = 0;
+    const int slot = my_slot();
+
+    const int aoff = s3_slot(g, l15) * 16;
+    const int jt_end = 2 * ((JH + 31) >> 5);
+#pragma unroll 1
+    for (int jt = (a.j_lo >> 4) + split * A3_TW + tw; jt < jt_end; jt += a.nsplit * A3_TW) {
+        const int jb = jt >> 1, jh = jt & 1, j0 = 32 * jb;
+        int lofs = 0;
+        asm volatile("" : "+v"(lofs));
+        f32x4 P[M], Q[M];
+        struct JF { u32x4 t, p[3][3]; };
+        auto jload = [&](int ss, JF& o) {
+            const unsigned char* ar = A3.Zb[ss >> 1] + (size_t)(((ss & 1) ? 0 : A3.nbA) + jb) * S3_BLOCK + jh * 1024 + aoff;
+            o.t = a3_ld(ar + S3_TAIL);
+#pragma unroll
+            for (int p = 0; p < 3; ++p)
+#pragma unroll
+                for (int q = 0; q < 3; ++q) o.p[p][q] = a3_ld(ar + p * S3_PLANE + q * 2048);
+        };
+        JF jf[2];
+        jload(0, jf[0]);
+#pragma unroll
+        for (int ss = 0; ss < 2 * M; ++ss) {
+            if (ss + 1 < 2 * M) jload(ss + 1, jf[(ss + 1) & 1]);
+            __builtin_amdgcn_sched_barrier(0);
+            const JF& o = jf[ss & 1];
+            const u32x4* bo = own3 + lofs + ((ss * 2 + ih) * A3_NOP) * 64 + lane;
+            u32x4 ow[A3_NOP];
+#pragma unroll
+            for (int k = 0; k < A3_NOP; ++k) ow[k] = bo[k * 64];
+            constexpr int PA[6] = {2, 1, 1, 0, 0, 0}, PB[6] = {0, 1, 0, 2, 1, 0};
+            f32x4 acc = f32x4{0.f, 0.f, 0.f, 0.f};
+            acc = mfma_b(o.t, ow[0], acc);
+            acc = mfma_b(o.t, ow[1], acc);
+#pragma unroll
+            for (int x = 0; x < 6; ++x)
+#pragma unroll
+                for (int q = 0; q < 3; ++q) acc = mfma_b(o.p[PA[x]][q], ow[2 + PB[x] * 3 + q], acc);
+            if (ss & 1) Q[ss >> 1] = acc; else P[ss >> 1] = acc;
+            __builtin_amdgcn_sched_barrier(0);
+        }
+        const int jg = j0 + 8 * g + 4 * jh;
+        if constexpr (SYM) {
+            if (j0 >= a.mir) aa_epilogue_sym<M>(a, inv_s, beta, P, Q, acc_gs, acc_gam, acc_out, jg, JH, iv, my_i, ns);
+            else aa_epilogue<M, TERMS, true>(a, inv_s, beta, P, Q, acc_gs, acc_gam, acc_out, jg, JH, iv, my_i, ns);
+        } else {
+            if (j0 + 32 <= A && i0 + 32 <= a.i_hi) aa_epilogue<M, TERMS, false>(a, inv_s, beta, P, Q, acc_gs, acc_gam, acc_out, jg, JH, iv, my_i, ns);
+            else aa_epilogue<M, TERMS, true>(a, inv_s, beta, P, Q, acc_gs, acc_gam, acc_out, jg, JH, iv, my_i, ns);
+        }
+        if ((++tiles_done & (SYM ? 15 : 31)) == 0) aa_flush<M, TERMS>(a, inv_s, lane, slot, acc_gs, acc_gam, acc_out);
+    }
+    aa_flush<M, TERMS>(a, inv_s, lane, slot, acc_gs, acc_gam, acc_out);
+}
+
+}
+
+extern "C" int sga_loss_anchor_multi_bwd_symx_bf16x6(const void* const* Zb, int M, const float* beta, int A, int J1, int J2, const double* sums,
+                                                     float alpha, float tau_icl, float tau_ial, const float* coef, float* const* M1, float* const* M2,
+                                                     double* gs, double* gamma, int a_lo, int a_hi, int j_lo, int j_hi, int mir, double* out_terms,
+                                                     void* stream) {
+    SGA_CHECK_ARG(Zb && beta && sums && coef && M1 && gs && gamma && A >= 0 && J1 >= 0 && J2 >= 0, "sga_loss_anchor_multi_bwd_symx_bf16x6: bad argument");
+    SGA_CHECK_ARG(M == 2 || M == 3, "sga_loss_anchor_multi_bwd_symx_bf16x6: M=%d (2 or 3; four tables take sga_loss_anchor_multi_bwd_symx)", M);
+    SGA_CHECK_ARG(a_lo >= 0 && a_lo <= a_hi && a_hi <= A && a_lo % 32 == 0 && (a_hi % 32 == 0 || a_hi == A),
+                  "sga_loss_anchor_multi_bwd_symx_bf16x6: block [%d,%d) not on 32-row boundaries of [0,%d]", a_lo, a_hi, A);
+    SGA_CHECK_ARG(j_lo >= 0 && j_lo % 32 == 0 && j_hi <= A && j_lo <= j_hi && (j_hi % 32 == 0 || j_hi == A) && mir >= j_lo && (mir % 32 == 0 || mir >= j_hi),
+                  "sga_loss_anchor_multi_bwd_symx_bf16x6: columns [%d,%d) / mirror start %d not on 32-column boundaries", j_lo, j_hi, mir);
+    const bool ordered = j_lo == 0 && j_hi == A && mir >= j_hi;
+    SGA_CHECK_ARG(ordered || mir <= j_lo || (j_lo >= a_lo && (mir < j_hi ? mir : j_hi) <= a_hi),
+                  "sga_loss_anchor_multi_bwd_symx_bf16x6: ordered columns [%d,%d) outside the block's square [%d,%d)", j_lo, mir, a_lo, a_hi);
+    SGA_CHECK_ARG(ordered || out_terms, "sga_loss_anchor_multi_bwd_symx_bf16x6: a symmetric launch returns its terms (out_terms == NULL)");
+    for (int m = 0; m < M; ++m)
+        SGA_CHECK_ARG(Zb[m] && M1[m] && (mir >= j_hi || (M2 && M2[m])), "sga_loss_anchor_multi_bwd_symx_bf16x6: null table or stash");
+    hipStream_t s = static_cast<hipStream_t>(stream);
+    if (int rc0 = zero_slots(gs, (M + 1) * 8, s, "sga_loss_anchor_multi_bwd_symx_bf16x6")) return rc0;
+    if (int rc1 = zero_slots(gamma, M, s, "sga_loss_anchor_multi_bwd_symx_bf16x6")) return rc1;
+    if (out_terms) { if (int rc2 = zero_slots(out_terms, (M + 1) + 2 * M, s, "sga_loss_anchor_multi_bwd_symx_bf16x6")) return rc2; }
+    if (A == 0 || a_hi <= a_lo || j_hi <= j_lo) return SGA_OK;
+    Anchor3Args k{};
+    AnchorMultiArgs& a = k.a;
+    a.M = M; a.A = A; a.i_lo = a_lo; a.i_hi = a_hi; a.beta = beta; a.sums = sums; a.alpha = alpha;
+    a.kc = LOG2E / tau_icl; a.ki = LOG2E / tau_ial; a.itc = 1.f / tau_icl; a.iti = 1.f / tau_ial;
+    a.coef = coef; a.gs = gs; a.gamma = gamma; a.out = out_terms;
+    a.j_lo = j_lo; a.j_hi = j_hi; a.mir = mir;
+    k.nbA = make_tlayout(A, J1, J2).nbA;
+    for (int m = 0; m < M; ++m) {
+        k.Zb[m] = static_cast<const unsigned char*>(Zb[m]);
+        a.M1[m] = M1[m]; a.M2[m] = M2 ? M2[m] : nullptr;
+    }
+    float* inv = reinterpret_cast<float*>(gs + (size_t)(1 + SGA_SLOTS) * (M + 1) * 8);
+    hipLaunchKernelGGL(inv_sums_kernel, dim3(1), dim3(64), 0, s, sums, inv, (M + 1) * 8);
+    a.inv = inv;
+    const size_t lds = (size_t)M * 2 * 2 * A3_NOP * 1024;
+    const int nib = (a_hi - a_lo + 31) / 32, ntile16 = 2 * ((j_hi + 31) / 32) - (j_lo >> 4);
+    int nsp = (3 * sga_num_cus() + nib - 1) / nib;
+    if (nsp > (ntile16 + A3_TW - 1) / A3_TW) nsp = (ntile16 + A3_TW - 1) / A3_TW;
+    if (nsp < 1) nsp = 1;
+    a.nsplit = nsp;
+    auto go = [&](auto kern) {
+        hipFuncSetAttribute(reinterpret_cast<const void*>(kern), hipFuncAttributeMaxDynamicSharedMemorySize, (int)lds);
+        hipLaunchKernelGGL(kern, dim3(nib * nsp), dim3(A3_THREADS), lds, s, k);
+    };
+    if (!ordered) { if (M == 2) go(anchor3_bwd_kernel<2, true, true>); else go(anchor3_bwd_kernel<3, true, true>); }
+    else if (out_terms) { if (M == 2) go(anchor3_bwd_kernel<2, true, false>); else go(anchor3_bwd_kernel<3, true, false>); }
+    else { if (M == 2) go(anchor3_bwd_kernel<2, false, false>); else go(anchor3_bwd_kernel<3, false, false>); }
+    if (out_terms) fold_slots(out_terms, (M + 1) + 2 * M, s);
+    fold_slots(gs, (M + 1) * 8, s);
+    fold_slots(gamma, M, s);
+    SGA_CHECK_LAUNCH("sga_loss_anchor_multi_bwd_symx_bf16x6");
+    return SGA_OK;
+}
diff --git a/sgaligner_amd/csrc/loss_anchor.hip b/sgaligner_amd/csrc/loss_anchor.hip
--- a/sgaligner_amd/csrc/loss_anchor.hip
+++ b/sgaligner_amd/csrc/loss_anchor.hip
@@ -2,6 +2,7 @@
 #include <type_traits>
 
 #include "loss_math.h"
+#include "aa_epilogue.h"
 
 extern "C" int sga_gemm(int transA, int transB, int M, int N, int K, const void* A, long lda, int a_is_f64, const float* B,
                         long ldb, float* C, long ldc, const float* bias, int accumulate, void* stream);
@@ -9,23 +10,6 @@
 namespace {
 
 constexpr int CT_THREADS = 256;
-struct AnchorMultiArgs {
-    int M, A, i_lo, i_hi, nsplit;
-    const float* Z[4];
-    const float* beta;
-    const double* sums;
-    const float* inv;
-    float alpha, kc, ki, itc, iti;
-    double* out;
-    const float* coef;
-    float* M1[4];
-    double* gs;
-    double* gamma;
-    int j_lo;
-    float* M2[4];
-    int j_hi, mir;
-};
-
 template <int M>
 __global__ __launch_bounds__(CT_THREADS, M <= 3 ? 2 : 1) void anchor_multi_kernel(AnchorMultiArgs a) {
     constexpr int DP = 104, NQ = 13, NT = M + 1;
@@ -135,18 +119,12 @@
     }
 }
 
-__global__ void inv_sums_kernel(const double* __restrict__ sums, float* __restrict__ inv, int n) {
-    const int i = blockIdx.x * blockDim.x + threadIdx.x;
-    if (i < n) inv[i] = (float)(1.0 / (sums[i] + 1e-9));
-}
-
 template <int M, bool TERMS = false, int RB = (M <= 3 ? 32 : 16), bool SYM = false>
 __global__ __launch_bounds__(CT_THREADS, 2) void anchor_multi_bwd16_kernel(AnchorMultiArgs a) {
     static_assert(!SYM || TERMS, "symmetric mode: one-pass build");
     constexpr int DP = 104, NT = M + 1, NSUB = RB / 16, TW = 4 / NSUB;
     extern __shared__ __attribute__((aligned(16))) float lds[];
     const float* __restrict__ inv_s = a.inv;
-    auto CF = [&](int e) { return a.coef[e]; };
     const int tid = threadIdx.x, lane = tid & 63, wave = tid >> 6, g = lane >> 4, l15 = lane & 15;
     const int A = a.A, ns = a.i_hi - a.i_lo;
     const int JH = SYM ? a.j_hi : A;
@@ -178,32 +156,7 @@
     for (int e = 0; e < (TERMS ? NT + 2 * M : 1); ++e) acc_out[e] = 0.f;
     int tiles_done = 0;
     const int slot = my_slot();
-    auto flush = [&]() {
-        if (TERMS) {
-#pragma unroll
-            for (int e = 0; e < NT + 2 * M; ++e) {
-                const float v = wave_sum(acc_out[TERMS ? e : 0]);
-                if (lane == 0 && v != 0.f) atomicAdd(a.out + (NT + 2 * M) * (1 + slot) + e, (double)v);
-                acc_out[TERMS ? e : 0] = 0.f;
-            }
-        }
-#pragma unroll
-        for (int k = 0; k < NT; ++k)
-#pragma unroll
-            for (int e = 0; e < 8; ++e) {
-                const float iv2 = inv_s[k * 8 + e];
-                const float v = -iv2 * iv2 * wave_sum(acc_gs[k][e]);
-                if (lane == 0 && v != 0.f) atomicAdd(a.gs + NT * 8 * (1 + slot) + k * 8 + e, (double)v);
-                acc_gs[k][e] = 0.f;
-            }
-#pragma unroll
-        for (int m = 0; m < M; ++m) {
-            const float v = wave_sum(acc_gam[m]);
-            if (lane == 0 && v != 0.f) atomicAdd(a.gamma + M * (1 + slot) + m, (double)v);
-            acc_gam[m] = 0.f;
-        }
-    };
-    const float* js = inv_s + M * 8;
+    auto flush = [&]() { aa_flush<M, TERMS>(a, inv_s, lane, slot, acc_gs, acc_gam, acc_out); };
 
     const int ntile = (JH + 15) / 16;
 #pragma unroll 1
@@ -256,172 +209,13 @@
             }
             __builtin_amdgcn_sched_barrier(0);
         }
-        const float cJ = CF(M);
-        auto epilogue = [&](auto masked_c) {
-        constexpr bool MASKED = decltype(masked_c)::value;
-#pragma unroll
-        for (int r = 0; r < 4; ++r) {
-            const int j = j0 + 4 * g + r;
-            const bool ok = !MASKED || (iv && (j < JH));
-            const float okf = (!MASKED || ok) ? 1.f : 0.f;
-            float xj = 0.f, yj = 0.f;
-#pragma unroll
-            for (int m = 0; m < M; ++m) { xj = fmaf(beta[m], P[m][r], xj); yj = fmaf(beta[m], Q[m][r], yj); }
-            float gJ, EA = 0.f, EB = 0.f;
-            {
-                const float dx = fexp2(xj * a.kc), dy = fexp2(yj * a.kc);
-                const GP Ax = g_parts(dx, js[0], js[2]), Bx = g_parts(dx, js[4], js[6]);
-                const float qAy = g_val(dy, js[0], js[2]), qBy = g_val(dy, js[4], js[6]);
-                const float denA = a.alpha * Ax.q + (1.f - a.alpha) * qBy;
-                const float wA = okf * (-cJ * a.alpha) * frcp(denA) * dx;
-                const float wB = okf * (-cJ * (1.f - a.alpha)) * frcp(a.alpha * qAy + (1.f - a.alpha) * Bx.q) * dx;
-                if (TERMS) acc_out[TERMS ? M : 0] = fmaf(okf, -flog(denA), acc_out[TERMS ? M : 0]);
-                gJ = fmaf(wA, Ax.dd, wB * Bx.dd) * a.itc;
-                acc_gs[M][0] = fmaf(wA, Ax.p, acc_gs[M][0]); acc_gs[M][2] = fmaf(wA, Ax.r, acc_gs[M][2]);
-                acc_gs[M][4] = fmaf(wB, Bx.p, acc_gs[M][4]); acc_gs[M][6] = fmaf(wB, Bx.r, acc_gs[M][6]);
-            }
-            const float dji = fexp2(xj * a.ki);
-            const GP MA = g_parts(dji, js[1], js[3]), MB = g_parts(dji, js[5], js[7]);
-            const float lqma = flog(MA.q), lqmb = flog(MB.q);
-            float gx[M];
-#pragma unroll
-            for (int m = 0; m < M; ++m) {
-                const float* is = inv_s + m * 8;
-                const float c = CF(m), ca = CF(NT + m), cb = CF(NT + M + m);
-                const float x = P[m][r], y = Q[m][r];
-                const float dx = fexp2(x * a.kc), dy = fexp2(y * a.kc);
-                const GP Ax = g_parts(dx, is[0], is[2]), Bx = g_parts(dx, is[4], is[6]);
-                const float qAy = g_val(dy, is[0], is[2]), qBy = g_val(dy, is[4], is[6]);
-                const float denA = a.alpha * Ax.q + (1.f - a.alpha) * qBy;
-                const float wA = okf * (-c * a.alpha) * frcp(denA) * dx;
-                const float wB = okf * (-c * (1.f - a.alpha)) * frcp(a.alpha * qAy + (1.f - a.alpha) * Bx.q) * dx;
-                if (TERMS) acc_out[TERMS ? m : 0] = fmaf(okf, -flog(denA), acc_out[TERMS ? m : 0]);
-                float gxm = fmaf(wA, Ax.dd, wB * Bx.dd) * a.itc;
-                acc_gs[m][0] = fmaf(wA, Ax.p, acc_gs[m][0]); acc_gs[m][2] = fmaf(wA, Ax.r, acc_gs[m][2]);
-                acc_gs[m][4] = fmaf(wB, Bx.p, acc_gs[m][4]); acc_gs[m][6] = fmaf(wB, Bx.r, acc_gs[m][6]);
-                const float dm = fexp2(x * a.ki);
-                const GP OA = g_parts(dm, is[1], is[3]), OB = g_parts(dm, is[5], is[7]);
-                const float xA = okf * __expf(OA.q), xB = okf * __expf(OB.q);
-                const float eA = ca * xA, eB = cb * xB;
-                if (TERMS) {
-                    acc_out[TERMS ? NT + m : 0] = fmaf(xA, OA.q - lqma, acc_out[TERMS ? NT + m : 0]);
-                    acc_out[TERMS ? NT + M + m : 0] = fmaf(xB, OB.q - lqmb, acc_out[TERMS ? NT + M + m : 0]);
-                }
-                const float tA = eA * (OA.q - lqma + 1.f) * dm, tB = eB * (OB.q - lqmb + 1.f) * dm;
-                gxm = fmaf(fmaf(tA, OA.dd, tB * OB.dd), a.iti, gxm);
-                acc_gs[m][1] = fmaf(tA, OA.p, acc_gs[m][1]); acc_gs[m][3] = fmaf(tA, OA.r, acc_gs[m][3]);
-                acc_gs[m][5] = fmaf(tB, OB.p, acc_gs[m][5]); acc_gs[m][7] = fmaf(tB, OB.r, acc_gs[m][7]);
-                EA += eA; EB += eB;
-                gx[m] = gxm;
-            }
-            {
-                const float uA = -EA * frcp(MA.q) * dji, uB = -EB * frcp(MB.q) * dji;
-                gJ = fmaf(fmaf(uA, MA.dd, uB * MB.dd), a.iti, gJ);
-                acc_gs[M][1] = fmaf(uA, MA.p, acc_gs[M][1]); acc_gs[M][3] = fmaf(uA, MA.r, acc_gs[M][3]);
-                acc_gs[M][5] = fmaf(uB, MB.p, acc_gs[M][5]); acc_gs[M][7] = fmaf(uB, MB.r, acc_gs[M][7]);
-            }
-#pragma unroll
-            for (int m = 0; m < M; ++m) {
-                acc_gam[m] = fmaf(gJ, P[m][r], acc_gam[m]);
-                if (ok) a.M1[m][(size_t)(j - a.j_lo) * ns + (my_i - a.i_lo)] = fmaf(beta[m], gJ, gx[m]);
-            }
-#pragma unroll
-            for (int k = 0; k < NT; ++k)
-#pragma unroll
-                for (int e = 0; e < 8; ++e) asm volatile("" : "+v"(acc_gs[k][e]));
-#pragma unroll
-            for (int m = 0; m < M; ++m) asm volatile("" : "+v"(acc_gam[m]));
-            if (TERMS) {
-#pragma unroll
-                for (int e = 0; e < NT + 2 * M; ++e) asm volatile("" : "+v"(acc_out[TERMS ? e : 0]));
-            }
-            __builtin_amdgcn_sched_barrier(0);
-        }
-        };
-        auto epilogue_sym = [&](auto) {
-#pragma unroll
-        for (int r = 0; r < 4; ++r) {
-            const int j = j0 + 4 * g + r;
-            const bool ok = iv && (j < JH);
-            const float okf = ok ? 1.f : 0.f;
-            float xj = 0.f, yj = 0.f;
-#pragma unroll
-            for (int m = 0; m < M; ++m) { xj = fmaf(beta[m], P[m][r], xj); yj = fmaf(beta[m], Q[m][r], yj); }
-            float gci[NT][2];
-#pragma unroll
-            for (int k = 0; k < NT; ++k) {
-                const float* is = inv_s + k * 8;
-                const float x = k < M ? P[k < M ? k : 0][r] : xj, y = k < M ? Q[k < M ? k : 0][r] : yj;
-                const float c = CF(k);
-                const float dx = fexp2(x * a.kc), dy = fexp2(y * a.kc);
-                const GP Ax = g_parts(dx, is[0], is[2]), Bx = g_parts(dx, is[4], is[6]);
-                const GP Ay = g_parts(dy, is[0], is[2]), By = g_parts(dy, is[4], is[6]);
-                const float den1 = a.alpha * Ax.q + (1.f - a.alpha) * By.q;
-                const float den2 = a.alpha * Ay.q + (1.f - a.alpha) * Bx.q;
-                const float r1 = okf * -c * frcp(den1), r2 = okf * -c * frcp(den2);
-                const float wAx = a.alpha * r1 * dx, wBx = (1.f - a.alpha) * r2 * dx;
-                const float wAy = a.alpha * r2 * dy, wBy = (1.f - a.alpha) * r1 * dy;
-                acc_out[TERMS ? k : 0] = fmaf(okf, -(flog(den1) + flog(den2)), acc_out[TERMS ? k : 0]);
-                gci[k][0] = fmaf(wAx, Ax.dd, wBx * Bx.dd) * a.itc;
-                gci[k][1] = fmaf(wAy, Ay.dd, wBy * By.dd) * a.itc;
-                acc_gs[k][0] = fmaf(wAx, Ax.p, fmaf(wAy, Ay.p, acc_gs[k][0])); acc_gs[k][2] = fmaf(wAx, Ax.r, fmaf(wAy, Ay.r, acc_gs[k][2]));
-                acc_gs[k][4] = fmaf(wBx, Bx.p, fmaf(wBy, By.p, acc_gs[k][4])); acc_gs[k][6] = fmaf(wBx, Bx.r, fmaf(wBy, By.r, acc_gs[k][6]));
-#pragma unroll
-                for (int e = 0; e < 8; e += 2) asm volatile("" : "+v"(acc_gs[k][e]));
-                asm volatile("" : "+v"(acc_out[TERMS ? k : 0]));
-                __builtin_amdgcn_sched_barrier(0);
-            }
-#pragma unroll
-            for (int dir = 0; dir < 2; ++dir) {
-                const float vj = dir ? yj : xj;
-                const float dji = fexp2(vj * a.ki);
-                const GP MA = g_parts(dji, js[1], js[3]), MB = g_parts(dji, js[5], js[7]);
-                const float lqma = flog(MA.q), lqmb = flog(MB.q);
-                float gx[M], EA = 0.f, EB = 0.f;
-#pragma unroll
-                for (int m = 0; m < M; ++m) {
-                    const float* is = inv_s + m * 8;
-                    const float ca = CF(NT + m), cb = CF(NT + M + m);
-                    const float v = dir ? Q[m][r] : P[m][r];
-                    const float dm = fexp2(v * a.ki);
-                    const GP OA = g_parts(dm, is[1], is[3]), OB = g_parts(dm, is[5], is[7]);
-                    const float xA = okf * __expf(OA.q), xB = okf * __expf(OB.q);
-                    const float eA = ca * xA, eB = cb * xB;
-                    acc_out[TERMS ? NT + m : 0] = fmaf(xA, OA.q - lqma, acc_out[TERMS ? NT + m : 0]);
-                    acc_out[TERMS ? NT + M + m : 0] = fmaf(xB, OB.q - lqmb, acc_out[TERMS ? NT + M + m : 0]);
-                    const float tA = eA * (OA.q - lqma + 1.f) * dm, tB = eB * (OB.q - lqmb + 1.f) * dm;
-                    gx[m] = fmaf(fmaf(tA, OA.dd, tB * OB.dd), a.iti, gci[m][dir]);
-                    acc_gs[m][1] = fmaf(tA, OA.p, acc_gs[m][1]); acc_gs[m][3] = fmaf(tA, OA.r, acc_gs[m][3]);
-                    acc_gs[m][5] = fmaf(tB, OB.p, acc_gs[m][5]); acc_gs[m][7] = fmaf(tB, OB.r, acc_gs[m][7]);
-                    EA += eA; EB += eB;
-                }
-                const float uA = -EA * frcp(MA.q) * dji, uB = -EB * frcp(MB.q) * dji;
-                const float gJ = fmaf(fmaf(uA, MA.dd, uB * MB.dd), a.iti, gci[M][dir]);
-                acc_gs[M][1] = fmaf(uA, MA.p, acc_gs[M][1]); acc_gs[M][3] = fmaf(uA, MA.r, acc_gs[M][3]);
-                acc_gs[M][5] = fmaf(uB, MB.p, acc_gs[M][5]); acc_gs[M][7] = fmaf(uB, MB.r, acc_gs[M][7]);
-                float* const* dst = dir ? a.M2 : a.M1;
-                const size_t off = (size_t)(j - (dir ? a.mir : a.j_lo)) * ns + (my_i - a.i_lo);
-#pragma unroll
-                for (int m = 0; m < M; ++m) {
-                    acc_gam[m] = fmaf(gJ, dir ? Q[m][r] : P[m][r], acc_gam[m]);
-                    if (ok) dst[m][off] = fmaf(beta[m], gJ, gx[m]);
-                }
-#pragma unroll
-                for (int k = 0; k < NT; ++k)
-#pragma unroll
-                    for (int e = 1; e < 8; e += 2) asm volatile("" : "+v"(acc_gs[k][e]));
-#pragma unroll
-                for (int m = 0; m < M; ++m) asm volatile("" : "+v"(acc_gam[m]));
-#pragma unroll
-                for (int e = NT; e < NT + 2 * M; ++e) asm volatile("" : "+v"(acc_out[TERMS ? e : 0]));
-                __builtin_amdgcn_sched_barrier(0);
-            }
-        }
-        };
+        const int jg = j0 + 4 * g;
         if constexpr (SYM) {
-            if (j0 >= a.mir) epilogue_sym(0); else epilogue(std::true_type{});
+            if (j0 >= a.mir) aa_epilogue_sym<M>(a, inv_s, beta, P, Q, acc_gs, acc_gam, acc_out, jg, JH, iv, my_i, ns);
+            else aa_epilogue<M, TERMS, true>(a, inv_s, beta, P, Q, acc_gs, acc_gam, acc_out, jg, JH, iv, my_i, ns);
         } else {
-            if (j0 + 16 <= A && i0 + RB <= a.i_hi) epilogue(std::false_type{}); else epilogue(std::true_type{});
+            if (j0 + 16 <= A && i0 + RB <= a.i_hi) aa_epilogue<M, TERMS, false>(a, inv_s, beta, P, Q, acc_gs, acc_gam, acc_out, jg, JH, iv, my_i, ns);
+            else aa_epilogue<M, TERMS, true>(a, inv_s, beta, P, Q, acc_gs, acc_gam, acc_out, jg, JH, iv, my_i, ns);
         }
         if ((++tiles_done & (SYM ? 15 : 31)) == 0) flush();
     }
diff --git a/sgaligner_amd/csrc/s3_layout.h b/sgaligner_amd/csrc/s3_layout.h
--- /dev/null
+++ b/sgaligner_amd/csrc/s3_layout.h
@@ -0,0 +1,35 @@
+#pragma once
+#include "loss_math.h"
+
+namespace {
+
+typedef __bf16 bf16x8 __attribute__((ext_vector_type(8)));
+typedef __bf16 bf16x2 __attribute__((ext_vector_type(2)));
+typedef float f32x2 __attribute__((ext_vector_type(2)));
+typedef unsigned int u32x4 __attribute__((ext_vector_type(4)));
+typedef unsigned int u32x2 __attribute__((ext_vector_type(2)));
+typedef short s16x4 __attribute__((ext_vector_type(4)));
+
+constexpr int S3_DP = 104;
+constexpr int S3_PLANE = 3 * 2 * 1024;
+constexpr int S3_TAIL = 3 * S3_PLANE;
+constexpr int S3_BLOCK = S3_TAIL + 2048;
+constexpr int S3_NCH = S3_BLOCK / 1024;
+constexpr int S3_ROWSLOTS = 3 * 12 + 4;
+
+__device__ __forceinline__ f32x4 mfma_b(u32x4 a, u32x4 b, f32x4 c) {
+    return __builtin_amdgcn_mfma_f32_16x16x32_bf16(__builtin_bit_cast(bf16x8, a), __builtin_bit_cast(bf16x8, b), c, 0, 0, 0);
+}
+__host__ __device__ constexpr int s3_slot(int g, int i) { return 16 * g + (i ^ (12 * (g & 1))); }
+
+struct TLayout { int nbA, nb1, nb2; };
+__host__ __device__ inline TLayout make_tlayout(int A, int J1, int J2) { return TLayout{(A + 31) / 32, (J1 + 31) / 32, (J2 + 31) / 32}; }
+
+__device__ __forceinline__ void s3_own_tails(const u32x4 th, const u32x4 tm, const u32x4 tl, const int g4, u32x4 (&otl)[2]) {
+    otl[0] = g4 == 1 ? tm : th;
+    otl[1] = g4 == 0 ? tl : (g4 == 2 ? tm : u32x4{0, 0, 0, 0});
+#pragma unroll
+    for (int t = 0; t < 2; ++t) otl[t][2] = (otl[t][2] >> 16) | (otl[t][2] << 16);
+}
+
+}
diff --git a/sgaligner_amd/csrc/sweep3.hip b/sgaligner_amd/csrc/sweep3.hip
--- a/sgaligner_amd/csrc/sweep3.hip
+++ b/sgaligner_amd/csrc/sweep3.hip
@@ -1,22 +1,9 @@
 #include <type_traits>
 
 #include "loss_math.h"
+#include "s3_layout.h"
 
 namespace {
-
-typedef __bf16 bf16x8 __attribute__((ext_vector_type(8)));
-typedef __bf16 bf16x2 __attribute__((ext_vector_type(2)));
-typedef float f32x2 __attribute__((ext_vector_type(2)));
-typedef unsigned int u32x4 __attribute__((ext_vector_type(4)));
-typedef unsigned int u32x2 __attribute__((ext_vector_type(2)));
-typedef short s16x4 __attribute__((ext_vector_type(4)));
-
-constexpr int S3_DP = 104;
-constexpr int S3_PLANE = 3 * 2 * 1024;
-constexpr int S3_TAIL = 3 * S3_PLANE;
-constexpr int S3_BLOCK = S3_TAIL + 2048;
-constexpr int S3_NCH = S3_BLOCK / 1024;
-constexpr int S3_ROWSLOTS = 3 * 12 + 4;
 
 __device__ __forceinline__ void split3_pair(float v0, float v1, unsigned& h, unsigned& m, unsigned& l) {
     const bf16x2 H = __builtin_convertvector(f32x2{v0, v1}, bf16x2);
@@ -43,9 +30,6 @@
     const bf16x2 Lo = __builtin_convertvector(f32x2{s0, s1}, bf16x2);
     h = hu; m = mu; l = __builtin_bit_cast(unsigned, Lo);
 }
-__device__ __forceinline__ f32x4 mfma_b(u32x4 a, u32x4 b, f32x4 c) {
-    return __builtin_amdgcn_mfma_f32_16x16x32_bf16(__builtin_bit_cast(bf16x8, a), __builtin_bit_cast(bf16x8, b), c, 0, 0, 0);
-}
 __device__ __forceinline__ u32x2 tr_read16(const unsigned char* p) {
     return __builtin_bit_cast(u32x2, __builtin_amdgcn_ds_read_tr16_b64_v4i16((__attribute__((address_space(3))) s16x4*)(p)));
 }
@@ -61,11 +45,6 @@
         sgb_seq<X + 1, END, NR, VALU_ALL>();
     }
 }
-__host__ __device__ constexpr int s3_slot(int g, int i) { return 16 * g + (i ^ (12 * (g & 1))); }
-
-struct TLayout { int nbA, nb1, nb2; };
-__host__ __device__ inline TLayout make_tlayout(int A, int J1, int J2) { return TLayout{(A + 31) / 32, (J1 + 31) / 32, (J2 + 31) / 32}; }
-
 constexpr int S3_STAT_BYTES = 2048;
 constexpr int S3_DREAL = 100;
 
@@ -277,11 +256,7 @@
 #pragma unroll
             for (int q = 0; q < 3; ++q) rescale(opl[m][0][q], opl[m][1][q], opl[m][2][q]);
             rescale(th, tm, tl);
-            otl[m][0] = g4 == 1 ? tm : th;
-            otl[m][1] = g4 == 0 ? tl : (g4 == 2 ? tm : u32x4{0, 0, 0, 0});
-#pragma unroll
-            for (int t = 0; t < 2; ++t)
-                otl[m][t][2] = (otl[m][t][2] >> 16) | (otl[m][t][2] << 16);
+            s3_own_tails(th, tm, tl, g4, otl[m]);
         }
     }
 #pragma unroll
diff --git a/sgaligner_amd/loss_ops.py b/sgaligner_amd/loss_ops.py
--- a/sgaligner_amd/loss_ops.py
+++ b/sgaligner_amd/loss_ops.py
@@ -445,6 +445,15 @@
         else:
             _call('sga_loss_stash_grad', _p(m1), b, self.s.A, 104, _p(dz), *job[:2])
 
+    def anchor(self, beta, sums, alpha, coef, m1, m2, gsc, gam2, job, sym, out):
+        lo, hi, jl, jh, mir = job
+        head = (_ptr_array(self.zs), self.M, _p(beta), self.s.A, _p(sums), alpha, TAU_ICL, TAU_IAL, _p(coef), _ptr_array(m1))
+        if sym:
+            _call('sga_loss_anchor_multi_bwd_symx', *head, _ptr_array(m2) if m2 is not None else (_ct.c_void_p * self.M)(), _p(gsc), _p(gam2),
+                  lo, hi, jl, jh, mir, _p(out))
+        else:
+            _call('sga_loss_anchor_multi_bwd', *head, _p(gsc), _p(gam2), lo, hi, _p(out))
+
     def scatter(self, k, dz, nrm, d, de):
         _call('sga_loss_scatter', _p(dz), _p(self.zs[k]), _p(nrm), _p(self.s.idx), self.s.R, d, 104, _p(de))
 
@@ -482,6 +491,15 @@
         if not _o.BF16X6_STASH:
             return super().stash(k, m1, m2, dz, job, sym)
         _call('sga_loss_stash_grad_symx_bf16x6', _p(m1), _p(m2), _p(self.planes[k]), *self.geom, _p(dz), *job)
+
+    def anchor(self, beta, sums, alpha, coef, m1, m2, gsc, gam2, job, sym, out):
+        lo, hi, jl, jh, mir = job
+        A = self.s.A
+        aligned = lo % 32 == 0 and jl % 32 == 0 and (mir % 32 == 0 or mir >= jh) and (hi % 32 == 0 or hi == A) and (jh % 32 == 0 or jh == A)
+        if not (_o.AA_PLANES and A >= _o.AA_PLANES_MIN_ANCHORS and self.M <= 3 and aligned):
+            return super().anchor(beta, sums, alpha, coef, m1, m2, gsc, gam2, job, sym, out)
+        _call('sga_loss_anchor_multi_bwd_symx_bf16x6', _ptr_array(self.planes), self.M, _p(beta), *self.geom, _p(sums), alpha, TAU_ICL, TAU_IAL, _p(coef),
+              _ptr_array(m1), _ptr_array(m2) if m2 is not None else None, _p(gsc), _p(gam2), lo, hi, jl, jh, mir, _p(out))
 
     def scatter(self, k, dz, nrm, d, de):
         _call('sga_loss_scatter_tangent', _p(dz), _p(self.zs[k]), _p(nrm), _p(self.s.idx), *self.geom, d, _p(self.planes[k]), _p(de))
@@ -505,17 +523,11 @@
     gam2 = torch.empty((slots, M), device=dev, dtype=torch.float64)
     fl = max(((jh - jl) + max(0, jh - mir)) * (hi - lo) for lo, hi, jl, jh, mir in jobs)
     buf = [torch.empty((fl,), device=dev, dtype=torch.float32) for _ in range(M)]
-    zarr = _ptr_array(tier.zs)
     for lo, hi, jl, jh, mir in jobs:
         n1 = (jh - jl) * (hi - lo)
         m1, m2 = [b[:n1] for b in buf], [b[n1:] for b in buf]
         has2 = mir < jh
-        if sym:
-            _call('sga_loss_anchor_multi_bwd_symx', zarr, M, _p(beta), A, _p(sums), alpha, TAU_ICL, TAU_IAL, _p(coef), _ptr_array(m1),
-                  _ptr_array(m2) if has2 else (_ct.c_void_p * M)(), _p(gsc), _p(gam2), lo, hi, jl, jh, mir, _p(out))
-        else:
-            _call('sga_loss_anchor_multi_bwd', zarr, M, _p(beta), A, _p(sums), alpha, TAU_ICL, TAU_IAL, _p(coef), _ptr_array(m1), _p(gsc), _p(gam2),
-                  lo, hi, _p(out))
+        tier.anchor(beta, sums, alpha, coef, m1, m2 if has2 else None, gsc, gam2, (lo, hi, jl, jh, mir), sym, out)
         if out is not None:
             terms += out[:n_terms]
         gs += gsc[0]
diff --git a/sgaligner_amd/ops.py b/sgaligner_amd/ops.py
--- a/sgaligner_amd/ops.py
+++ b/sgaligner_amd/ops.py
@@ -398,6 +398,8 @@
 FUSED_AA_ONEPASS = True
 AA_SYMMETRIC = True
 ONEPASS_MIN_ANCHORS = 256
+AA_PLANES = _os.environ.get('SGA_AA_PLANES', '1') != '0'
+AA_PLANES_MIN_ANCHORS = 1024
 WIDE_STASH = True
 KERNEL_EVENTS = None
 
```

Measured after the change: 1003, median of 6. +1.3%, better.
